# Hi-PACE/hipace

Measured on AMD Instinct MI355X. Metric: transverse slices/s at 1024^2 x 4ppc (explicit solver), higher is better.
Workload: dtype f64

## Files before the change

hipace_amd/_lib.py:

```python
import ctypes as C
import os
import subprocess


def hip_already_started():
    import sys
    if _LIB is not None:
        return True
    t = sys.modules.get("torch")
    try:
        return bool(t is not None and t.cuda.is_initialized())
    except Exception:
        return False


_LIB = None
_HWQ_PRESET = "GPU_MAX_HW_QUEUES" in os.environ
_HIP_STARTED_AT_IMPORT = hip_already_started()
_HERE = os.path.dirname(os.path.abspath(__file__))
CSRC = os.path.join(_HERE, "csrc")
SO = os.environ.get("HPS_LIB") or os.path.join(CSRC, "libhpslice.so")


class Slab(C.Structure):
# ... 74 lines not shown
                ("adaptive_no_predict_step", C.c_int), ("adaptive_no_phase_control", C.c_int), ("adaptive_phase_substeps", C.c_int),
                ("adaptive_density", C.c_double), ("max_time", C.c_double), ("beam_uz_std", C.c_double),
                ("ext_Ez_slope", C.c_double),
                ("beam_do_salame", C.c_int), ("salame_n_iter", C.c_int), ("salame_relative_tolerance", C.c_double),
                ("salame_no_advance", C.c_int), ("salame_Ez_target_slope", C.c_double)]


COMPS = ["N_jx_beam", "N_jy_beam", "chi", "Sy", "Sx", "ExmBy", "EypBx", "Ez", "Bx", "By", "Bz",
         "Psi", "jx_beam", "jy_beam", "jz_beam", "jx", "jy", "rhomjz", "P_jx_beam", "P_jy_beam",
         "Ion_rhomjz", "rho"]
CIDX = {n: i for i, n in enumerate(COMPS)}
COMPS_PC = ["N_jx", "N_jy", "ExmBy", "EypBx", "Ez", "Bx", "By", "Bz", "Psi", "jx", "jy", "jz", "rhomjz",
            "P_Bx", "P_By", "P_jx", "P_jy", "Ion_rhomjz", "It_Bx", "It_By", "PIt_Bx", "PIt_By", "rho"]
CIDX_PC = {n: i for i, n in enumerate(COMPS_PC)}
COMPS_SALAME = ["Ez_target", "Ez_no_salame", "Ez", "jx", "jy", "jz_beam", "Bx", "By", "Sy", "Sx", "Sy_back", "Sx_back"]
ID_VALID = 1 << 63

_SIGS = {
    "hps_last_error": (C.c_char_p, []),
    "hps_version": (C.c_char_p, []),
    "hps_deposit_current": (C.c_int, [Slab, Plasma, Geom, C.c_void_p, C.c_double, C.c_double, C.c_int, C.c_double,
                                      C.c_int, C.c_void_p, C.c_void_p]),
    "hps_explicit_deposit": (C.c_int, [Slab, Plasma, Geom, C.c_void_p, C.c_void_p, C.c_double, C.c_double, C.c_int,
                                       C.c_int, C.c_int, C.c_void_p]),
    "hps_advance_plasma": (C.c_int, [Slab, Plasma, Geom, C.c_void_p, C.c_double, C.c_double, C.c_int, C.c_int,
                                     C.c_int, C.c_int, C.c_void_p]),
    "hps_tiling_create": (C.c_int, [C.c_int, C.c_int, C.c_int, C.c_long, C.POINTER(C.c_void_p)]),
    "hps_reorder_particles": (C.c_int, [C.c_void_p, Plasma, Plasma, Geom, C.c_void_p]),
    "hps_tiling_info": (C.c_int, [C.c_void_p, C.POINTER(C.c_int), C.POINTER(C.c_void_p), C.POINTER(C.c_void_p)]),
    "hps_tiling_destroy": (C.c_int, [C.c_void_p]),
    "hps_deposit_current_tiled": (C.c_int, [Slab, Plasma, Geom, C.c_void_p, C.c_double, C.c_double, C.c_int, C.c_double,
                                            C.c_int, C.c_void_p, C.c_void_p, C.c_void_p, C.c_void_p]),
    "hps_explicit_deposit_tiled": (C.c_int, [Slab, Plasma, Geom, C.c_void_p, C.c_void_p, C.c_double, C.c_double, C.c_int,
                                             C.c_int, C.c_int, C.c_void_p, C.c_void_p, C.c_void_p]),
    "hps_advance_plasma_tiled": (C.c_int, [Slab, Plasma, Geom, C.c_void_p, C.c_double, C.c_double, C.c_int, C.c_int,
                                           C.c_int, C.c_int, C.c_void_p, C.c_void_p, C.c_void_p]),
    "hps_deposit_current_tiled_laser": (C.c_int, [Slab, Plasma, Geom, C.c_void_p, C.c_int, C.c_double, C.c_double, C.c_int,
                                                  C.c_double, C.c_int, C.c_void_p, C.c_void_p, C.c_void_p, C.c_void_p]),
    "hps_explicit_deposit_tiled_laser": (C.c_int, [Slab, Plasma, Geom, C.c_void_p, C.c_int, C.c_void_p, C.c_double, C.c_double,
                                                   C.c_int, C.c_int, C.c_int, C.c_void_p, C.c_void_p, C.c_void_p]),
    "hps_advance_plasma_tiled_laser": (C.c_int, [Slab, Plasma, Geom, C.c_void_p, C.c_int, C.c_double, C.c_double, C.c_int,
                                                 C.c_int, C.c_int, C.c_int, C.c_void_p, C.c_void_p, C.c_void_p]),
    "hps_tiling_set_validity": (C.c_int, [C.c_void_p, C.c_int, C.c_int]),
    "hps_particles_record": (C.c_int, [C.c_int]),
    "hps_particles_recorded": (C.c_int, [C.c_char_p, C.c_long, C.POINTER(C.c_long)]),
    "hps_poisson_create": (C.c_int, [C.c_int, C.c_int, C.c_double, C.c_double, C.POINTER(C.c_void_p)]),
    "hps_poisson_solve": (C.c_int, [C.c_void_p, C.c_void_p, Slab, C.c_int, C.c_void_p]),
    "hps_poisson_solve_batch": (C.c_int, [C.c_void_p, C.c_int, C.c_void_p, Slab, C.c_void_p, C.c_void_p]),
    "hps_poisson_info": (C.c_int, [C.c_void_p, C.POINTER(C.c_int), C.POINTER(C.c_int), C.POINTER(C.c_int)]),
    "hps_poisson_destroy": (C.c_int, [C.c_void_p]),
    "hps_mg_create": (C.c_int, [C.c_int, C.c_int, C.c_double, C.c_double, C.POINTER(C.c_void_p)]),
    "hps_mg_solve1": (C.c_int, [C.c_void_p, Slab, C.c_int, C.c_int, C.c_int, C.c_double, C.c_double, C.c_int,
                                C.POINTER(C.c_int), C.POINTER(C.c_double), C.c_void_p]),
    "hps_mg_solve1_fabs": (C.c_int, [C.c_void_p, Slab, Slab, Slab, C.c_double, C.c_double, C.c_int,
                                     C.POINTER(C.c_int), C.POINTER(C.c_double), C.c_void_p]),
    "hps_mg_info": (C.c_int, [C.c_void_p, C.POINTER(C.c_int), C.POINTER(C.c_int), C.POINTER(C.c_int), C.POINTER(C.c_int),
                              C.POINTER(C.c_long), C.POINTER(C.c_int), C.POINTER(C.c_int), C.POINTER(C.c_int), C.POINTER(C.c_int)]),
    "hps_mg_destroy": (C.c_int, [C.c_void_p]),
    "hps_mg2_create": (C.c_int, [C.c_int, C.c_int, C.c_double, C.c_double, C.POINTER(C.c_void_p)]),
    "hps_mg2_solve2": (C.c_int, [C.c_void_p, C.c_void_p, C.c_void_p, C.c_void_p, C.c_void_p, C.c_double, C.c_double, C.c_int,
                                 C.POINTER(C.c_int), C.POINTER(C.c_double), C.c_void_p]),
    "hps_mg2_info": (C.c_int, [C.c_void_p, C.POINTER(C.c_int), C.POINTER(C.c_int), C.POINTER(C.c_int), C.POINTER(C.c_int)]),
    "hps_mg2_destroy": (C.c_int, [C.c_void_p]),
    "hps_engine_laser_vcycles": (C.c_int, [C.c_void_p, C.POINTER(C.c_long)]),
    "hps_engine_create": (C.c_int, [C.POINTER(Deck), C.c_int, C.POINTER(C.c_void_p)]),
    "hps_engine_destroy": (C.c_int, [C.c_void_p]),
    "hps_engine_begin_step": (C.c_int, [C.c_void_p]),
    "hps_engine_solve_slice": (C.c_int, [C.c_void_p, C.c_int]),
    "hps_engine_solve_slice_begin": (C.c_int, [C.c_void_p, C.c_int]),
    "hps_engine_solve_slice_finish": (C.c_int, [C.c_void_p, C.c_int]),
    "hps_engine_slice_ready": (C.c_int, [C.c_void_p]),
    "hps_engine_run_step": (C.c_int, [C.c_void_p]),
    "hps_engine_sync": (C.c_int, [C.c_void_p]),
    "hps_engine_info": (C.c_int, [C.c_void_p, C.POINTER(C.c_int), C.POINTER(C.c_int), C.POINTER(C.c_long)]),
    "hps_engine_slab": (Slab, [C.c_void_p]),
    "hps_engine_plasma": (Plasma, [C.c_void_p]),
    "hps_engine_stream": (C.c_void_p, [C.c_void_p]),
    "hps_engine_ions": (Plasma, [C.c_void_p]),
    "hps_engine_ion_stats": (C.c_int, [C.c_void_p, C.POINTER(C.c_long), C.POINTER(C.c_long)]),
    "hps_engine_checksums": (C.c_int, [C.c_void_p, C.c_void_p]),
    "hps_beam_sort_by_box": (C.c_int, [C.c_void_p, C.c_long, C.c_double, C.c_double, C.c_int, C.c_void_p, C.c_void_p,
                                       C.c_void_p, C.c_void_p]),
    "hps_engine_stats": (C.c_int, [C.c_void_p, C.POINTER(C.c_long), C.POINTER(C.c_long)]),
    "hps_engine_set_insitu_plasma": (C.c_int, [C.c_void_p, C.c_double]),
    "hps_engine_set_insitu_beam": (C.c_int, [C.c_void_p, C.c_double]),
    "hps_engine_insitu_beam": (C.c_int, [C.c_void_p, C.c_void_p]),
    "hps_engine_insitu_plasma": (C.c_int, [C.c_void_p, C.c_void_p]),
    "hps_engine_set_insitu_fields": (C.c_int, [C.c_void_p, C.c_int]),
    "hps_engine_insitu_fields": (C.c_int, [C.c_void_p, C.c_void_p]),
    "hps_engine_set_field_diagnostic": (C.c_int, [C.c_void_p, C.c_int, C.c_void_p, C.c_void_p]),
    "hps_engine_field_diagnostic": (C.c_int, [C.c_void_p, C.c_void_p]),
    "hps_engine_set_field_diagnostic_box": (C.c_int, [C.c_void_p, C.c_int, C.c_void_p, C.c_void_p, C.c_int, C.c_void_p, C.c_void_p]),
    "hps_engine_field_diagnostic_geometry": (C.c_int, [C.c_void_p, C.c_void_p, C.c_void_p, C.c_void_p]),
    "hps_engine_record_event": (C.c_int, [C.c_void_p, C.c_int, C.POINTER(C.c_void_p)]),
    "hps_engine_wait_event": (C.c_int, [C.c_void_p, C.c_void_p]),
    "hps_stream_pool_shared_pairs": (C.c_int, [C.c_int]),
    "hps_engine_copy_async": (C.c_int, [C.c_void_p, C.c_void_p, C.c_void_p, C.c_long]),
    "hps_engine_set_profiling_stride": (C.c_int, [C.c_void_p, C.c_int]),
    "hps_engine_set_laser_import": (C.c_int, [C.c_void_p, C.c_int, C.c_int]),
    "hps_engine_set_step": (C.c_int, [C.c_void_p, C.c_int]),
    "hps_engine_set_time": (C.c_int, [C.c_void_p, C.c_double, C.c_double]),
    "hps_engine_beam_moments": (C.c_int, [C.c_void_p, C.c_void_p]),
    "hps_adaptive_create": (C.c_int, [C.c_void_p, C.POINTER(C.c_void_p)]),
    "hps_adaptive_set_density_profile": (C.c_int, [C.c_void_p, C.c_int, C.c_void_p, C.c_void_p, C.c_int, C.c_void_p, C.c_void_p]),
    "hps_adaptive_initial_dt": (C.c_int, [C.c_void_p, C.c_double, C.c_double, C.c_int, C.POINTER(C.c_double)]),
    "hps_adaptive_before_step": (C.c_int, [C.c_void_p, C.c_double, C.POINTER(C.c_double)]),
    "hps_adaptive_next_time": (C.c_int, [C.c_void_p, C.POINTER(C.c_double)]),
    "hps_adaptive_after_step": (C.c_int, [C.c_void_p, C.c_void_p, C.c_double, C.c_int, C.POINTER(C.c_double)]),
    "hps_adaptive_destroy": (C.c_int, [C.c_void_p]),
    "hps_engine_export_laser_slice": (C.c_int, [C.c_void_p, C.c_int, C.c_void_p]),
    "hps_engine_import_laser_slice": (C.c_int, [C.c_void_p, C.c_int, C.c_void_p]),
    "hps_engine_import_laser_from": (C.c_int, [C.c_void_p, C.c_int, C.c_void_p]),
    "hps_engine_laser_envelope": (C.c_int, [C.c_void_p, C.c_void_p]),
    "hps_engine_laser_info": (C.c_int, [C.c_void_p, C.POINTER(C.c_int), C.POINTER(C.c_double)]),
    "hps_engine_set_laser_grid": (C.c_int, [C.c_void_p, C.POINTER(C.c_int), C.POINTER(C.c_double), C.POINTER(C.c_double), C.c_int]),
    "hps_engine_laser_grid": (C.c_int, [C.c_void_p, C.POINTER(C.c_int), C.POINTER(C.c_int), C.POINTER(C.c_int), C.POINTER(C.c_int)]),
    "hps_engine_laser_chi": (C.c_int, [C.c_void_p, C.c_void_p]),
    "hps_engine_set_laser_pulses": (C.c_int, [C.c_void_p, C.c_int, C.POINTER(LaserPulse)]),
    "hps_engine_add_laser_samples": (C.c_int, [C.c_void_p, C.c_int, C.c_void_p, C.POINTER(C.c_long), C.POINTER(C.c_double),
                                               C.POINTER(C.c_double), C.c_double]),
    "hps_engine_set_insitu_laser": (C.c_int, [C.c_void_p, C.c_int]),
    "hps_engine_insitu_laser": (C.c_int, [C.c_void_p, C.c_void_p]),
    "hps_laser_interp_aabs": (C.c_int, [Slab, C.c_int, C.c_void_p, C.c_int, C.c_int, C.c_double, C.c_double, C.c_double, C.c_double,
                                        Geom, C.c_int, C.c_void_p]),
    "hps_laser_interp_chi": (C.c_int, [Slab, C.c_int, C.c_void_p, C.c_void_p, C.c_int, C.c_int, C.c_double, C.c_double, C.c_double,
                                       C.c_double, Geom, C.c_int, C.c_int, C.c_void_p]),
    "hps_deposit_current_laser": (C.c_int, [Slab, Plasma, Geom, C.c_void_p, C.c_int, C.c_double, C.c_double, C.c_int, C.c_double,
                                            C.c_int, C.c_void_p, C.c_void_p]),
    "hps_explicit_deposit_laser": (C.c_int, [Slab, Plasma, Geom, C.c_void_p, C.c_int, C.c_void_p, C.c_double, C.c_double, C.c_int,
                                             C.c_int, C.c_int, C.c_void_p]),
    "hps_advance_plasma_laser": (C.c_int, [Slab, Plasma, Geom, C.c_void_p, C.c_int, C.c_double, C.c_double, C.c_int, C.c_int,
                                           C.c_int, C.c_int, C.c_void_p]),
    "hps_engine_pc_stats": (C.c_int, [C.c_void_p, C.POINTER(C.c_long), C.POINTER(C.c_double)]),
    "hps_engine_pc_zero_b_slices": (C.c_int, [C.c_void_p, C.POINTER(C.c_long)]),
    "hps_engine_set_diagnostics": (C.c_int, [C.c_void_p, C.c_int]),
    "hps_engine_set_tiling": (C.c_int, [C.c_void_p, C.c_int, C.c_int]),
    "hps_engine_fallbacks": (C.c_int, [C.c_void_p, C.POINTER(C.c_long)]),
    "hps_engine_set_fusion": (C.c_int, [C.c_void_p, C.c_int]),
    "hps_engine_set_density_profile": (C.c_int, [C.c_void_p, C.c_int, C.c_void_p, C.c_void_p, C.c_int, C.c_void_p, C.c_void_p]),
    "hps_engine_set_plasma_init": (C.c_int, [C.c_void_p, C.POINTER(C.c_int), C.POINTER(C.c_int), C.c_double]),
    "hps_engine_set_fine_patch": (C.c_int, [C.c_void_p, C.c_void_p, C.c_int]),
    "hps_engine_set_plasma_momentum": (C.c_int, [C.c_void_p, C.c_int, C.POINTER(C.c_double), C.POINTER(C.c_double), C.c_ulonglong]),
    "hps_engine_set_plasma_symmetry": (C.c_int, [C.c_void_p, C.c_int, C.c_int]),
    "hps_engine_sorts": (C.c_int, [C.c_void_p, C.POINTER(C.c_long)]),
    "hps_engine_assume_initial_beam_support": (C.c_int, [C.c_void_p]),
    "hps_engine_beam_state": (C.c_int, [C.c_void_p, C.c_void_p, C.c_void_p]),
    "hps_engine_beam_capacity": (C.c_int, [C.c_void_p, C.POINTER(C.c_long)]),
    "hps_engine_set_beam_capacity": (C.c_int, [C.c_void_p, C.c_long]),
    "hps_engine_beam_message_rows": (C.c_int, [C.c_void_p, C.POINTER(C.c_int)]),
    "hps_engine_beam_spin": (C.c_int, [C.c_void_p, C.c_void_p]),
    "hps_engine_set_beam_import": (C.c_int, [C.c_void_p, C.c_int]),
    "hps_engine_export_beam_slice": (C.c_int, [C.c_void_p, C.c_int, C.c_void_p]),
    "hps_engine_import_beam_slice": (C.c_int, [C.c_void_p, C.c_int, C.c_void_p]),
    "hps_engine_set_profiling": (C.c_int, [C.c_void_p, C.c_int]),
    "hps_engine_phase_times": (C.c_int, [C.c_void_p, C.c_void_p, C.c_void_p]),
    "hps_engine_beam_info": (C.c_int, [C.c_void_p, C.POINTER(C.c_long), C.c_void_p]),
    "hps_engine_set_beam_particles": (C.c_int, [C.c_void_p, C.c_long, C.c_void_p, C.POINTER(C.c_long)]),
    "hps_engine_set_beam_storage": (C.c_int, [C.c_void_p, C.c_void_p]),
    "hps_engine_initial_beam": (C.c_int, [C.c_void_p, C.c_void_p]),
    "hps_ring_unique_id": (C.c_int, [C.c_char_p]),
    "hps_ring_init": (C.c_int, [C.c_int, C.c_int, C.c_int, C.c_char_p, C.c_char_p, C.POINTER(C.c_void_p)]),
    "hps_ring_send_slice": (C.c_int, [C.c_void_p, C.c_void_p, C.c_long, C.c_void_p, C.c_int, C.POINTER(C.c_void_p)]),
    "hps_ring_recv_slice": (C.c_int, [C.c_void_p, C.c_void_p, C.c_long, C.c_void_p, C.c_int, C.POINTER(C.c_void_p)]),
    "hps_ring_sendrecv_self": (C.c_int, [C.c_void_p, C.c_void_p, C.c_void_p, C.c_long, C.c_void_p, C.c_int, C.POINTER(C.c_void_p)]),
    "hps_ring_stream_wait": (C.c_int, [C.c_void_p, C.c_int, C.c_void_p]),
    "hps_ring_sync_sends": (C.c_int, [C.c_void_p]),
# ... 89 lines not shown
```

hipace_amd/api.py:

```python
import ctypes as C

import numpy as np
import torch

from . import _lib, decks as _decks, expr as _expr
from ._lib import CIDX, COMPS, ID_VALID, PL_REAL, check


def _stream():
    return C.c_void_p(torch.cuda.current_stream().cuda_stream)


def _iarr(vals):
    return (C.c_int * len(vals))(*[int(v) for v in vals])


class Geometry:

    def __init__(self, nx, ny, lo, hi, dz, bc=1, normalized=True, consts=(1., 1., 1., 1., 1.), ng=None):
        self.nx, self.ny = nx, ny
        g = _lib.Geom()
        g.dx = (hi[0] - lo[0]) / nx
        g.dy = (hi[1] - lo[1]) / ny
        g.dz = dz
# ... 1004 lines not shown
        if event is not None:
            check(_lib.lib().hps_engine_wait_event(self._h, C.c_void_p(event)))

    def copy_async(self, dst, src):
        assert dst.numel() == src.numel()
        check(_lib.lib().hps_engine_copy_async(self._h, C.c_void_p(dst.data_ptr()), C.c_void_p(src.data_ptr()),
                                               dst.numel() * 8))

    def phase_times(self):
        ms = (C.c_double * 8)()
        n = C.c_long()
        check(_lib.lib().hps_engine_phase_times(self._h, ms, C.byref(n)))
        names = ["deposit_current", "poisson", "explicit_deposit", "mg_solve1", "advance_plasma", "other", "sort", "empty_interval"]
        return {k: ms[i] for i, k in enumerate(names)}, n.value

    def checksums(self):
        out = (C.c_double * self.ncomp)()
        check(_lib.lib().hps_engine_checksums(self._h, out))
        names = self.comp_names()
        cs = {names[i]: out[i] for i in range(self.ncomp)}
        if "aabs" in cs:
            tot = C.c_double()
            check(_lib.lib().hps_engine_laser_info(self._h, None, C.byref(tot)))
            cs["laserEnvelope"] = tot.value
        return cs

    @property
    def has_laser(self):
        return bool(self.deck.get("laser_on", 0))

    def laser_message_doubles(self):
        nxl, nyl, _, _ = self.laser_grid()
        return 4 * nxl * nyl

    def set_step(self, step):
        check(_lib.lib().hps_engine_set_step(self._h, int(step)))

    def set_laser_import(self, on, step=0):
        check(_lib.lib().hps_engine_set_laser_import(self._h, int(on), int(step)))

    def export_laser_slice(self, islice, msg):
        check(_lib.lib().hps_engine_export_laser_slice(self._h, islice, C.c_void_p(msg.data_ptr())))

    def import_laser_slice(self, islice, msg):
        check(_lib.lib().hps_engine_import_laser_slice(self._h, islice, C.c_void_p(msg.data_ptr())))

    def import_laser_from(self, islice, src):
        check(_lib.lib().hps_engine_import_laser_from(self._h, islice, src._h))

    def laser_envelope(self):
        nxl, nyl, zlo, zhi = self.laser_grid()
        out = np.empty((zhi - zlo + 1, nyl, nxl), dtype=np.complex128)
        check(_lib.lib().hps_engine_laser_envelope(self._h, out.ctypes.data_as(C.c_void_p)))
        return out

    def comp_names(self):
        if self.deck.get("bxby_solver", 0):
            return list(_lib.COMPS_PC[:22]) + (["rho"] if self.deck.get("deposit_rho", 0) else [])
        return list(COMPS[:21]) + (["rho"] if self.deck.get("deposit_rho", 0) else []) + \
            (["aabs"] if self.deck.get("laser_on", 0) else []) + \
            (["Salame_" + n for n in _lib.COMPS_SALAME] if self.deck.get("beam_do_salame", 0) else [])

    def salame_stats(self):
        nz = self.deck["nz"]
        out = np.zeros((nz, 4), dtype=np.float64)
        check(_lib.lib().hps_engine_salame_stats(self._h, out.ctypes.data_as(C.c_void_p)))
        flags = out[:, 3].astype(np.int64)
        return {"W": out[:, 0].copy(), "W_total": out[:, 1].copy(), "iterations": out[:, 2].astype(np.int64),
                "converged": (flags & 1) != 0, "overloaded": (flags & 2) != 0, "ran": out[:, 2] > 0}

    def pc_stats(self):
        its, err = C.c_long(), C.c_double()
        check(_lib.lib().hps_engine_pc_stats(self._h, C.byref(its), C.byref(err)))
        return its.value, err.value

    def pc_zero_b_slices(self):
        n = C.c_long()
        check(_lib.lib().hps_engine_pc_zero_b_slices(self._h, C.byref(n)))
        return n.value

    def stats(self):
        vc, sl = C.c_long(), C.c_long()
        check(_lib.lib().hps_engine_stats(self._h, C.byref(vc), C.byref(sl)))
        return dict(vcycles=vc.value, slices=sl.value)

    def slab(self):
        self.sync()
        s = _lib.lib().hps_engine_slab(self._h)
        nx, ny, g = s.nx, s.ny, s.ng
        out = np.empty((s.ncomp, ny + 2 * g, nx + 2 * g), dtype=np.float64)
        check(_lib.lib().hps_memcpy_d2h(out.ctypes.data_as(C.c_void_p), C.c_void_p(s.p), out.nbytes))
        return out

    def ions(self):
        self.sync()
        p = _lib.lib().hps_engine_ions(self._h)
        n = p.n
        real = np.empty((11, n), dtype=np.float64)
        idc = np.empty(n, dtype=np.uint64)
        lev = np.empty(n, dtype=np.int32)
        if n:
            for k, name in enumerate(PL_REAL):
                check(_lib.lib().hps_memcpy_d2h(real[k].ctypes.data_as(C.c_void_p), C.c_void_p(getattr(p, name)), real[k].nbytes))
            check(_lib.lib().hps_memcpy_d2h(idc.ctypes.data_as(C.c_void_p), C.c_void_p(p.idcpu), idc.nbytes))
            check(_lib.lib().hps_memcpy_d2h(lev.ctypes.data_as(C.c_void_p), C.c_void_p(p.ion_lev), lev.nbytes))
        key = ((idc >> np.uint64(24)) & np.uint64((1 << 39) - 1)).astype(np.int64) - 1
        return real, ((idc >> np.uint64(63)) & np.uint64(1)).astype(np.int32), lev, key

    def ion_stats(self):
        a, b = C.c_long(), C.c_long()
        check(_lib.lib().hps_engine_ion_stats(self._h, C.byref(a), C.byref(b)))
        return a.value, b.value

    def particles(self):
        self.sync()
        p = _lib.lib().hps_engine_plasma(self._h)
        n = p.n
        real = np.empty((11, n), dtype=np.float64)
        idc = np.empty(n, dtype=np.uint64)
        if n:
            for k, name in enumerate(PL_REAL):
                check(_lib.lib().hps_memcpy_d2h(real[k].ctypes.data_as(C.c_void_p), C.c_void_p(getattr(p, name)), real[k].nbytes))
            check(_lib.lib().hps_memcpy_d2h(idc.ctypes.data_as(C.c_void_p), C.c_void_p(p.idcpu), idc.nbytes))
        return real, ((idc >> np.uint64(63)) & np.uint64(1)).astype(np.int32)
```

hipace_amd/csrc/engine.h:

```cpp
#ifndef HPS_ENGINE_H_
#define HPS_ENGINE_H_

#include "common.h"
#include "expr.h"
#include <algorithm>
#include <array>
#include <vector>
#include "tiling.h"
#include "mg_gate.h"
#include "particle_math.h"
#include "poisson_src.h"
#include "beam_deposit.h"
#include "slab_ops.h"

void mg_rider (void* mg_handle, int** dev_words, const int** host_words);
namespace hps {

constexpr int PC_MAX_SPEC = 64;

int mg_solve1_begin (void* mg_handle, hps_slab s, int sol_comp, int rhs_comp, int acf_comp, double tol_rel, double tol_abs,
                     int max_iters, hipStream_t st);
void mg_solve1_forget_hierarchy (void* mg_handle);
bool poisson_gateable (void* poisson_handle);
void poisson_set_gate (void* poisson_handle, const int* gate);
bool ring_is_ticket (const void* p);
int mg_solve1_prepare (void* mg_handle, hps_slab s, int sol_comp, int rhs_comp, int acf_comp, int max_iters, hipStream_t st);
int mg_solve1_prepare_with (void* mg_handle, hps_slab s, int sol_comp, int rhs_comp, int acf_comp, int max_iters, SlabView f, GradPsiSxSy ga,
                            hipStream_t st, bool* done);
const int* mg_gate_after_enqueued (void* mg_handle);
void mg_defer_post (void* mg_handle);
bool mg_take_deferred_post (void* mg_handle, MgPost* out);
bool mg_solve1_ready (void* mg_handle);
int mg_solve1_finish (void* mg_handle, int* iters_out, double* resnorm_out, int* extra, hipStream_t st);
}

namespace hps {

struct LaserState;

struct DensityProgram { const hps_expr_ins* ins; int n_ins; const double* consts; double z, min_density; };

struct ExprImage {
    ExprImage () = default;
    explicit ExprImage (int header_slots) : h_ins((size_t)header_slots, hps_expr_ins{0, 0}) {}
    int add (const hps_expr& checked);
    hps_expr_ins& slot (int q) { return h_ins[(size_t)q]; }
    int n_ins () const { return (int)h_ins.size(); }
    int upload ();
    const hps_expr_ins* ins () const { return d_ins.get(); }
    const double* consts () const { return d_consts.get(); }
private:
    std::vector<hps_expr_ins> h_ins; std::vector<double> h_consts;
    DevBuf<hps_expr_ins> d_ins; DevBuf<double> d_consts;
};

struct BeamSoA { double *x, *y, *z, *ux, *uy, *uz, *w; int* nsub;
                 double *sx, *sy, *sz; };

struct CollScratch {
    unsigned *cnt = nullptr, *off[2] = {nullptr, nullptr}, *perm[2] = {nullptr, nullptr};
    long cap[2] = {0, 0}; int ncells = 0; void* temp = nullptr; size_t temp_bytes = 0; unsigned long long* stats = nullptr;
    CollScratch () = default; CollScratch (const CollScratch&) = delete; CollScratch& operator= (const CollScratch&) = delete;
    ~CollScratch ();
};

struct Engine {
    hps_deck d{};
    hps_geom gm{};
    int g = 0, ncomp = 0;
    hipStream_t st = nullptr;
    bool st_pooled = false; int st_device = 0;
    hps_slab slab{};
    struct Ions { double* d_adk = nullptr; unsigned long long* d_cnt = nullptr; long long* h_cnt = nullptr; long long* h_cnt_dev = nullptr;
                  long long seq = 0; long n_ionized = 0; bool pending = false; int* d_tile_flag = nullptr;
                  double* d_fbound = nullptr;
                } ion;
    std::vector<double> prof_r, prof_t, prof_f_t; double* d_prof_r = nullptr; double prof_ft = 1.0;
    double hollow_core_radius = 0.0;
    bool fine_patch_set = false; int fine_T = 0; long fine_ncells = 0; int* d_fine_level = nullptr; int* d_fine_cells = nullptr;
    struct Thermal { double u_mean[3] = {0.0, 0.0, 0.0}, u_std[3] = {0.0, 0.0, 0.0}; unsigned long long seed = 0;
                     bool warm () const { for (int q = 0; q < 3; ++q) if (u_mean[q] != 0.0 || u_std[q] != 0.0) return true; return false; }
                   };
    bool do_symmetrize = false, prevent_centered = false;
    bool shifted (const int ppc[2], int dir) const { return prevent_centered && (dir == 0 ? d.nx : d.ny) % 2 == 1 && ppc[dir] % 2 == 1; }
    int set_plasma_momentum (int species, const double* u_mean, const double* u_std, unsigned long long seed);
    int set_plasma_symmetry (int symmetrize, int prevent_centered_particle);
    int alloc_sheets ();
    int set_plasma_init (const int* plasma_fine, const int* ion_fine, double hollow_core);
    int set_fine_patch (const unsigned char* mask_host, int transition_cells);
    bool fuse_push_deposit = false; int ahead_for = -2;
    long fallback_div = 256;
    bool gate_push = true;
    int step_index = -1;
    int next_step = -1;
    bool time_set = false; double next_t = 0.0, next_dt = 0.0, step_dt = 0.0;
    double step_time = 0.0;
    struct BeamExt { bool on = false; ExprImage image; int depth = 0; } bext;
    int set_beam_external_fields (const hps_expr* E3, const hps_expr* B3);
    struct DensityExpr { bool on = false; std::vector<std::vector<hps_expr_ins>> ins; std::vector<std::vector<double>> consts;
                         std::vector<double> z_pos; std::vector<int> off; int depth = 0; double min_density = 0.0; int cur = 0; };
    ExprImage dens_image; double dens_z = 0.0;
    int set_density_expr (int species, int n_progs, const hps_expr* progs, const double* z_pos, double min_density);
    void density_begin_step (double ct);
    DensityProgram density_program (int species) const;
    size_t density_lds (int species) const { const DensityExpr& D = sp[species].dens; return D.on ? expr_lds_bytes(D.depth, 256) : 0; }
    struct Species {
        int index = 0;
        hps_plasma pl{}, pl_alt{}; double *real = nullptr, *real_alt = nullptr; Tiling* tiling = nullptr;
        long cap = 0, n_init = 0;
        int ppc[2] = {0, 0}, fine_ppc[2] = {0, 0}; double density = 0.0, charge = 0.0, mass = 0.0;
        int init_level = 0, can_ionize = 0, keyed = 0;
// ... 34 lines not shown
    double* d_open_mom = nullptr;
    int open_boundary (int nbatch, unsigned no_monopole_mask);
    double* beam_data = nullptr; double* beam_init = nullptr; double* beam_cur = nullptr;
    long nbeam = 0; std::vector<long> beam_off;
    bool moving = false; int steps_begun = 0; int beam_rows = 7;
    BeamSoA bm{}, bm_scr{}; double* bm_store = nullptr; int* bm_nsub = nullptr; int* bm_nsub_scr = nullptr;
    long* d_B = nullptr; int* d_nfront = nullptr; std::vector<long> h_B;
    bool beam_import = false; long* d_Bimp = nullptr; long beam_cap = 0; int* d_beam_overflow = nullptr;
    long beam_bound (int p) const {
        if (p < 0 || p >= d.nz) return 0;
        if (beam_import) return std::max(nbeam, 1L);
        return h_B[p + 1] - h_B[0];
    }
    struct Box { int ilo, ihi, jlo, jhi; };
    Box beam_box{0, -1, 0, -1}, beam_box_init{0, -1, 0, -1}, full_box{0, -1, 0, -1};
    int* d_nqsa = nullptr;
    double* d_checksum = nullptr;
    bool diagnostics = false;
    bool profiling = false; bool prof_light = false; int prof_stride = 1; bool prof_now = false;
    std::vector<hipEvent_t> ev; size_t ev_used = 0;
    std::vector<hipEvent_t> hand_ev;
    void mark ();
    long total_vcycles = 0, slices_done = 0;
    int* d_pc_dist = nullptr;
    double pc_floor = 0.0;
    int* d_pc_go = nullptr; bool pc_speculate = false; int pc_spec_iters = 1, pc_enqueued = 0, pc_islice = -1; double pc_base_seq = 0.0, pc_last_err = 0.0;
    int solve_slice_pc_begin (int islice); int solve_slice_pc_finish (int islice); int pc_enqueue_iteration (int it); int pc_wait_slot (int slot, double seq);
    bool pc = false; double* d_pc = nullptr; double* d_pc_aux = nullptr; double* h_pc = nullptr; double* h_pc_dev = nullptr; double pc_seq = 0.0; long pc_iterations = 0; double pc_err_sum = 0.0; long pc_zero_b_slices = 0;
    double pc_tol = 4e-2, pc_mix = 0.05; int pc_max_iter = 30;
    int c_aabs = -1; double* d_laser_sum = nullptr;
    LaserState* laser = nullptr;
    struct LaserGrid { bool set = false; int nx = 0, ny = 0, zlo = 0, zhi = -1, order = 1;
                       double lo[3] = {0, 0, 0}, hi[3] = {0, 0, 0}, dx = 0.0, dy = 0.0, xoff = 0.0, yoff = 0.0; } lgrid;
    int set_laser_grid (const int* n_cell, const double* patch_lo, const double* patch_hi, int interp_order);
    struct LaserSamples { int geometry = 0; long extent[3] = {0, 0, 0}; double offset[3] = {0, 0, 0}, spacing[3] = {0, 0, 0}, unit = 1.0;
                          std::vector<double> data; };
    bool laser_pulses_set = false; std::vector<hps_laser_pulse> laser_pulses; std::vector<LaserSamples> laser_samples;
    bool insitu_laser = false;
    bool laser_has_slice (int islice) const { return !lgrid.set || (islice >= lgrid.zlo && islice <= lgrid.zhi); }
    hipStream_t st_laser = nullptr; hipEvent_t ev_lfork = nullptr, ev_ldone = nullptr;
    bool laser_async = true, laser_pending = false;
    hipStream_t st_aux = nullptr; hipEvent_t ev_aux[3] = {nullptr, nullptr, nullptr}; bool aux_on = false, aux_pending = false;
    hipStream_t laser_stream () const { return (laser_async && st_laser) ? st_laser : st; }
    int fork_laser ();
    int laser_done ();
    int join_laser ();
    std::vector<int> fd_comps; int fd_c[3] = {1, 1, 1}; double* d_fd = nullptr; int* d_fd_comps = nullptr;
    int fd_n[3] = {0, 0, 0}; double fd_h[3] = {0, 0, 0}, fd_pos0[3] = {0, 0, 0}, fd_lo[3] = {0, 0, 0}, fd_hi[3] = {0, 0, 0}; int fd_slice_dir = -1;
    size_t fd_cells () const { return (size_t)fd_n[0]*fd_n[1]*fd_n[2]; }
    int fill_field_diagnostic (int islice);
    double* d_insitu_bm = nullptr; double insitu_bm_radius = 0.0;
    void insitu_beam (int islice);
    double* d_insitu_pl = nullptr; double insitu_pl_radius = 0.0;
    double* d_insitu = nullptr;

    ~Engine ();
    int create (const hps_deck& deck, int device);
    int init_beam ();
    int install_beam (std::vector<double> (&h)[7]);
    int set_beam_particles (long n, const double* soa_host, long* n_outside);
    int set_beam_fixed_ppc (const hps_expr* density, double min_density, const double* u_std, const int* random_ppc, unsigned long long seed);
    int set_beam_fixed_weight (const hps_beam_fixed_weight* spec, const hps_expr* mean_x, const hps_expr* mean_y, unsigned long long seed,
                               long* n_left_out);
    int set_beam_fixed_weight_pdf (const hps_beam_fixed_weight_pdf* spec, const hps_expr* pdf, const hps_expr* progs, unsigned long long seed,
                                   long* n_left_out, double* uz_moments);
    int install_beam_device (double* blocks_dev, long n, const double box[4]);
    int begin_device_beam (long* n_left_out = nullptr);
    int finish_device_beam (DevBuf<double>& blocks, long n, long* n_left_out = nullptr);
    int drop_device_beam (int e, long* n_left_out);
    void release_beam ();
    void set_beam_box (double xlo, double xhi, double ylo, double yhi);
    int install_moving_beam (const std::vector<double> (*h)[7]);
    int begin_step ();
    int deposit_beam_slice (int islice, int cjx, int cjy, int cjz, const int* go = nullptr);
    void deposit_grid_current (int islice, int cjz);
    int solve_slice (int islice);
    int solve_slice_begin (int islice);
    int solve_slice_finish (int islice);
    int pending_slice = -1; bool pend_fuse = false, pend_gated = false, pend_gated_ion = false;
    bool gate_ion_push = true; IonArgs pend_ia{}; long pend_covered = 0;
    int push_with_ionization (int islice, const int comp[5], const int* go, bool first);
    bool lazy_shift = true, shift_pending = false;
    void flush_shift ();
    bool fuse_sources = true;
    int c_sal = -1; int sal_last_slice = -2; bool sal_overloaded = false; double sal_zeta_initial = 0.0;
    double* d_sal = nullptr; std::vector<double> sal_stats;
    bool salame_now () const { return c_sal >= 0 && step_index == 0; }
    int salame_module (int islice);
    int salame_solve_ez ();
    int run_step ();
    struct Collision { int a, b; double coulomb_log; unsigned long long seed; bool beam = false; };
    std::vector<Collision> coll; CollScratch coll_scratch; bool step_begun = false;
    int collide_slice (int islice);
};

int ion_create (Engine& E);
void ion_destroy (Engine& E);
unsigned event_flags (bool timing);
std::array<double**, 11> soa_arrays (hps_plasma& p);
int alloc_soa (hps_plasma& p, double*& real, long cap, bool alias);
void free_soa (hps_plasma& p, double*& real);
int init_plasma_fine (Engine& E, const Engine::Species& s, double radius_sq);
int init_plasma_warm (Engine& E, const Engine::Species& s, double radius_sq);
int laser_create (Engine& E);
void laser_destroy (Engine& E);
int laser_begin_step (Engine& E);
int laser_update_aabs (Engine& E, int islice, double* sum_abs);
int laser_advance_slice (Engine& E, int islice);
int laser_copy_envelope (Engine& E, double* out_host);
int laser_chi_initial (Engine& E);
int laser_copy_chi (Engine& E, double* out_host);
void laser_sizes (Engine& E, int* nx, int* ny, int* nz);
long laser_mg_vcycles (Engine& E);
int laser_set_import (Engine& E, int on, int step);
int laser_export_slice (Engine& E, int islice, double* msg_dev);
int laser_import_slice (Engine& E, int islice, const double* msg_dev);
int laser_import_from (Engine& E, int islice, Engine& src);
int laser_check_samples (Engine& E, const Engine::LaserSamples& S);
int laser_set_insitu (Engine& E, int on);
int laser_clear_insitu (Engine& E);
int laser_copy_insitu (Engine& E, double* out_host);
int expr_check_named (const char* fn, const char* what, const hps_expr* p, int n_vars, int* depth);
bool expr_is_zero (const hps_expr& p);
int beam_blocks_to_soa (Engine& E, const double* blocks, double* soa, long nb);
int beam_deposit_moving (Engine& E, int p, int cjx, int cjy, int cjz);
int beam_push_moving (Engine& E, int islice);
int beam_push_slice (Engine& E, int islice, int p, long bound);
int beam_moments_reset (Engine& E);
int beam_export_slice (Engine& E, int islice, double* msg_dev, long cap);
int beam_import_slice (Engine& E, int islice, const double* msg_dev, long cap);
int salame_get_w_enqueue (const hps_slab& slab, int cT, int cN, int cE, int cJ, double* scratch, hipStream_t st);
const double* salame_get_w_result (const double* scratch);

}
#endif
```

hipace_amd/csrc/engine.hip:

```cpp
#include "common.h"
#include "engine.h"

#include <cmath>
#include <cstdlib>
#include <cstring>
#include <limits>
#include <atomic>
#include <algorithm>
#include <map>
#include <mutex>
#include <new>

namespace {
std::mutex g_pool_mutex;
std::map<int, std::vector<hipStream_t>> g_stream_pool;
std::map<int, bool> g_pool_made;
}

namespace hps {

int deposit_current_tiled (const hps_slab& slab, const hps_plasma& pl, const hps_geom& g, const int comp[6], double charge,
                           double mass, int order, double max_qsa, int can_ionize, int* n_qsa, Tiling* T, int* n_fallback,
                           hipStream_t st, int aabs_comp = -1, const int* tile_flag = nullptr, TailWork tw = TailWork{},
                           const BeamPairWork* beam = nullptr, const int* go = nullptr, bool valid_by_w = false);
int explicit_deposit_tiled (const hps_slab& slab, const hps_plasma& pl, const hps_geom& g, const int cache[4], const int depos[2],
                            double charge, double mass, int order, int dtype, int can_ionize, Tiling* T, int* n_fallback,
                            hipStream_t st, int aabs_comp = -1, const int* tile_flag = nullptr, TailWork tw = TailWork{}, bool valid_by_w = false);
int advance_plasma_tiled (const hps_slab& slab, const hps_plasma& pl, const hps_geom& g, const int comp[5], double charge,
                          double mass, int order, int temp_slice, int n_subcycles, int can_ionize, Tiling* T,
                          int* n_fallback, hipStream_t st, int aabs_comp = -1, const IonArgs* ion = nullptr, const int* go = nullptr,
                          TailWork tw = TailWork{}, const MgPost* post = nullptr);
int advance_deposit_tiled (const hps_slab& slab, const hps_plasma& pl, const hps_geom& g, const int comp[5], const int dep_comp[6],
                           double charge, double mass, int order, int n_subcycles, double max_qsa, int* n_qsa, Tiling* T,
                           int* n_fallback, hipStream_t st);

static thread_local std::string g_err;
void set_error (const std::string& msg) { g_err = msg; }

struct CompList { int n; int c[12]; };


__global__ __launch_bounds__(256)
void k_zero_comps (double* p, long ns, long plane, int js, CompList full, CompList boxed, CellBox bb, CompList from_ion = CompList{0, {}}, int c_ion = -1)
{
    const long s = (long)blockIdx.x*blockDim.x + threadIdx.x;
    if (s >= plane) return;
    for (int k = 0; k < full.n; ++k) p[full.c[k]*ns + s] = 0.0;
    if (c_ion >= 0) { const double ion = p[c_ion*ns + s]; for (int k = 0; k < from_ion.n; ++k) p[from_ion.c[k]*ns + s] = ion; }
    const int j = (int)(s / js), i = (int)(s - (long)j*js);
    if (i >= bb.ilo && i <= bb.ihi && j >= bb.jlo && j <= bb.jhi)
        for (int k = 0; k < boxed.n; ++k) p[boxed.c[k]*ns + s] = 0.0;
}

__global__ __launch_bounds__(256)
void k_copy_comps (double* p, long ns, long plane, CompList dst, CompList src)
{
    const long s = (long)blockIdx.x*blockDim.x + threadIdx.x;
    if (s >= plane) return;
    double v[12];
    for (int k = 0; k < src.n; ++k) v[k] = p[src.c[k]*ns + s];
    for (int k = 0; k < dst.n; ++k) p[dst.c[k]*ns + s] = v[k];
}

__global__ __launch_bounds__(256)
void k_shift_slices (double* p, long ns, long plane, int js, CellBox bb)
{
    const long s = (long)blockIdx.x*blockDim.x + threadIdx.x;
    if (s >= plane) return;
    const int j = (int)(s / js), i = (int)(s - (long)j*js);
    double njx = 0.0, njy = 0.0;
    if (i >= bb.ilo && i <= bb.ihi && j >= bb.jlo && j <= bb.jhi) {
        const double tjx = p[HPS_C_JXB*ns + s], tjy = p[HPS_C_JYB*ns + s];
        njx = p[HPS_C_N_JXB*ns + s]; njy = p[HPS_C_N_JYB*ns + s];
        p[HPS_C_P_JXB*ns + s] = tjx; p[HPS_C_P_JYB*ns + s] = tjy;
        p[HPS_C_JXB*ns + s] = njx;   p[HPS_C_JYB*ns + s] = njy;
    }
    p[HPS_C_JX*ns + s] = njx; p[HPS_C_JY*ns + s] = njy;
}

__global__ __launch_bounds__(256)
void k_shift_zero (double* p, long ns, long plane, int js, CellBox bb, int c_rho, int c_ion = -1)
{
    const long s = (long)blockIdx.x*blockDim.x + threadIdx.x;
    if (s >= plane) return;
    const int j = (int)(s / js), i = (int)(s - (long)j*js);
    double njx = 0.0, njy = 0.0;
    if (i >= bb.ilo && i <= bb.ihi && j >= bb.jlo && j <= bb.jhi) {
        const double tjx = p[HPS_C_JXB*ns + s], tjy = p[HPS_C_JYB*ns + s];
        njx = p[HPS_C_N_JXB*ns + s]; njy = p[HPS_C_N_JYB*ns + s];
        p[HPS_C_P_JXB*ns + s] = tjx; p[HPS_C_P_JYB*ns + s] = tjy;
        p[HPS_C_JXB*ns + s] = njx;   p[HPS_C_JYB*ns + s] = njy;
        p[HPS_C_N_JXB*ns + s] = 0.0; p[HPS_C_N_JYB*ns + s] = 0.0; p[HPS_C_JZB*ns + s] = 0.0;
    }
    p[HPS_C_JX*ns + s] = njx; p[HPS_C_JY*ns + s] = njy;
    const double ion = c_ion >= 0 ? p[c_ion*ns + s] : 0.0;
    p[HPS_C_CHI*ns + s] = 0.0; p[HPS_C_RHOMJZ*ns + s] = ion;
    if (c_rho >= 0) p[c_rho*ns + s] = ion;
}

__global__ __launch_bounds__(256)
void k_add_ions_psi_rhs (SlabView f, int c_rhomjz, int c_ion, int c_rho, double inv_ep0, double* staging)
{
    const int i = blockIdx.x*blockDim.x + threadIdx.x - f.ng;
    const int j = blockIdx.y - f.ng;
    if (i >= f.nx + f.ng) return;
    const long o = f.off(i, j);
    const double ion = f.p[c_ion*f.ns + o];
    const double r = f.p[c_rhomjz*f.ns + o] + ion;
    f.p[c_rhomjz*f.ns + o] = r;
    if (c_rho >= 0) f.p[c_rho*f.ns + o] += ion;
    if (i >= 0 && i < f.nx && j >= 0 && j < f.ny) staging[(long)j*f.nx + i] = -inv_ep0*r;
}

__global__ __launch_bounds__(256)
void k_rhs_all (SlabView f, int c_rhomjz, int c_ion, int c_rho, int c_jx, int c_jy, double inv_ep0,
                double fez_x, double fez_y, double fbz_y, double fbz_x, double* staging, long plane)
{
    const int i = blockIdx.x*blockDim.x + threadIdx.x - f.ng;
    const int j = blockIdx.y - f.ng;
    if (i >= f.nx + f.ng) return;
    const long o = f.off(i, j);
    double r;
    if (c_ion >= 0) {
        const double ion = f.p[c_ion*f.ns + o];
        r = f.p[c_rhomjz*f.ns + o] + ion;
        f.p[c_rhomjz*f.ns + o] = r;
        if (c_rho >= 0) f.p[c_rho*f.ns + o] += ion;
    } else {
        if (!(i >= 0 && i < f.nx && j >= 0 && j < f.ny)) return;
        r = f.p[c_rhomjz*f.ns + o];
    }
    if (i >= 0 && i < f.nx && j >= 0 && j < f.ny) {
        const long so = (long)j*f.nx + i;
        const double* X = f.p + c_jx*f.ns + o;
        const double* Y = f.p + c_jy*f.ns + o;
        staging[so] = -inv_ep0*r;
        staging[plane + so] = fez_x*(X[1] - X[-1]) + fez_y*(Y[f.js] - Y[-f.js]);
        staging[2*plane + so] = fbz_y*(X[f.js] - X[-f.js]) + fbz_x*(Y[1] - Y[-1]);
    }
}

__global__ __launch_bounds__(256)
void k_rhs_lincomb (SlabView f, int cA, int dirA, double fa, int cB, int dirB, double fb, double* staging)
{
    const int i = blockIdx.x*blockDim.x + threadIdx.x;
    const int j = blockIdx.y;
    if (i >= f.nx) return;
    const long o = f.off(i, j);
    const long sa = dirA == 0 ? 1 : f.js, sb = dirB == 0 ? 1 : f.js;
    const double* A = f.p + cA*f.ns + o;
    const double* B = f.p + cB*f.ns + o;
    staging[(long)j*f.nx + i] = fa*(A[sa] - A[-sa]) + fb*(B[sb] - B[-sb]);
}

__global__ __launch_bounds__(256)
void k_grid_current (SlabView f, int cjz, double xlo, double ylo, double dx, double dy, double mx, double my, double sx, double sy,
                     double amp)
{
    const int i = blockIdx.x*blockDim.x + threadIdx.x;
    const int j = blockIdx.y;
    if (i >= f.nx) return;
    const double delta_x = (xlo + (i + 0.5)*dx - mx) / sx;
    const double delta_y = (ylo + (j + 0.5)*dy - my) / sy;
    f(i, j, cjz) += amp*exp(-0.5*(delta_x*delta_x + delta_y*delta_y));
}

__global__ __launch_bounds__(256)
void k_grad_psi (SlabView f, int cPsi, int cExmBy, int cEypBx, double hdx_inv, double hdy_inv)
{
    const int gg = f.ng - 1;
    const int i = blockIdx.x*blockDim.x + threadIdx.x - gg;
    const int j = blockIdx.y - gg;
    if (i >= f.nx + gg) return;
    const long o = f.off(i, j);
    const double* P = f.p + cPsi*f.ns + o;
    f.p[cExmBy*f.ns + o] = -(P[1] - P[-1])*hdx_inv;
    f.p[cEypBx*f.ns + o] = -(P[f.js] - P[-f.js])*hdy_inv;
}

__global__ __launch_bounds__(256)
// ... 409 lines not shown
        int lo = 0, hi = -1;
        if (std::sscanf(e.substr(pos, end - pos).c_str(), "%d-%d", &lo, &hi) == 2)
            for (int b = std::max(lo, 0); b <= std::min(hi, 255); ++b) mask[b >> 5] |= 1u << (b & 31);
        pos = end + 1;
    }
    return hipExtStreamCreateWithCUMask(s, 8, mask);
}

long Engine::sheet_slots (const Species& s) const
{
    if (!s.present()) return 0;
    const long cells = (long)d.nx*d.ny, nc = (long)s.ppc[0]*s.ppc[1];
    const long copies = do_symmetrize ? 4 : 1;
    if (!(fine_patch_set && s.fine_ppc[0] > 0)) return copies*nc*cells;
    return copies*(nc*cells + ((long)s.fine_ppc[0]*s.fine_ppc[1] - nc)*fine_ncells);
}

std::array<double**, 11> soa_arrays (hps_plasma& p)
{
    return {&p.x, &p.y, &p.w, &p.ux, &p.uy, &p.psi, &p.x_prev, &p.y_prev, &p.ux_half, &p.uy_half, &p.psi_half};
}
int alloc_soa (hps_plasma& p, double*& real, long cap, bool alias)
{
    HPS_HIP_CHECK(hipMalloc(&real, (size_t)cap*11*sizeof(double)));
    const auto arr = soa_arrays(p);
    for (int k = 0; k < 11; ++k) *arr[k] = real + (size_t)k*cap;
    if (alias) { p.x_prev = p.x; p.y_prev = p.y; }
    HPS_HIP_CHECK(hipMalloc(&p.idcpu, (size_t)cap*sizeof(uint64_t)));
    HPS_HIP_CHECK(hipMalloc(&p.ion_lev, (size_t)cap*sizeof(int32_t)));
    return HPS_OK;
}
void free_soa (hps_plasma& p, double*& real)
{
    (void)hipFree(real); (void)hipFree(p.idcpu); (void)hipFree(p.ion_lev);
    real = nullptr; p = hps_plasma{};
}
static hps_plasma tail_of (const hps_plasma& p, long first, long n)
{
    hps_plasma t = p;
    for (double** a : soa_arrays(t)) *a += first;
    t.idcpu += first; t.ion_lev += first; t.n = n;
    return t;
}

int Engine::alloc_sheets ()
{
    for (Species& s : sp) { free_soa(s.pl, s.real); s.n_init = s.cap = sheet_slots(s); }
    if (ions.present()) el.cap = el.n_init + ions.n_init*(long)(d.ion_Z - d.ion_init_level);
    for (Species& s : sp) {
        s.pl.n = s.n_init;
        if (s.cap > 0) { if (int e = alloc_soa(s.pl, s.real, s.cap, s.alias_prev())) return e; }
    }
    return HPS_OK;
}

int Engine::create (const hps_deck& deck, int device)
{
    d = deck;
    HPS_REQUIRE(d.nx >= 4 && d.ny >= 4 && d.nz >= 1, "hps_engine_create: bad grid");
    HPS_REQUIRE(d.order >= 0 && d.order <= 3, "hps_engine_create: depos_order must be 0..3");
    HPS_REQUIRE(d.n_subcycles >= 0, "hps_engine_create: plasma n_subcycles must be >= 1 (0 = default 1)");
    if (d.n_subcycles == 0) d.n_subcycles = 1;
    if (d.field_bc != 0 && d.field_bc != 1) { set_error("hps_engine_create: boundary.field must be 0 (Dirichlet) or 1 (Open)"); return HPS_ERR_UNSUPPORTED; }
    if (d.field_bc == 1) {
        const double radius = std::min(std::min(std::fabs(d.lo[0]), std::fabs(d.hi[0])), std::min(std::fabs(d.lo[1]), std::fabs(d.hi[1])));
        HPS_REQUIRE(radius > 0.0 && d.lo[0] < 0.0 && d.hi[0] > 0.0 && d.lo[1] < 0.0 && d.hi[1] > 0.0, "hps_engine_create: boundary.field = Open needs x = y = 0 inside the box");
        HPS_HIP_CHECK(hipMalloc(&d_open_mom, (size_t)4*256*2*19*sizeof(double)));
    }
    pc = (d.bxby_solver != 0);
    if (const char* v = std::getenv("HPS_GATED_PUSH")) gate_push = std::atoi(v) != 0;
    if (const char* v = std::getenv("HPS_AUX_STREAM")) aux_on = std::atoi(v) != 0;
    if (aux_on) {
        HPS_HIP_CHECK(hipStreamCreateWithFlags(&st_aux, hipStreamNonBlocking));
        for (hipEvent_t& ev : ev_aux) HPS_HIP_CHECK(hipEventCreateWithFlags(&ev, event_flags(false)));
    }
    if (const char* v = std::getenv("HPS_FOLD_TAIL")) fold_tail = std::atoi(v) != 0;
    if (const char* v = std::getenv("HPS_POST_IN_PUSH")) post_in_push = std::atoi(v) != 0;
    if (const char* v = std::getenv("HPS_FOLD_BEAM")) fold_beam = std::atoi(v) != 0;
    if (const char* v = std::getenv("HPS_FOLD_HIERARCHY")) fold_hierarchy = std::atoi(v) != 0;
    if (const char* v = std::getenv("HPS_VALID_BY_W")) valid_by_w = std::atoi(v) != 0;
    if (const char* v = std::getenv("HPS_GATED_ION_PUSH")) gate_ion_push = std::atoi(v) != 0;
    if (const char* v = std::getenv("HPS_LAZY_SHIFT")) lazy_shift = std::atoi(v) != 0;
    if (const char* v = std::getenv("HPS_FUSE_SOURCES")) fuse_sources = std::atoi(v) != 0;
    if (const char* v = std::getenv("HPS_SORT_FALLBACK_DIV")) { const long q = std::atol(v); if (q >= 1) fallback_div = q; }
    HPS_REQUIRE(!(d.beam_spin_tracking && d.dt == 0.0 && !d.dt_adaptive), "hps_engine_create: spin tracking needs a moving beam (hipace.dt != 0)");
    HPS_REQUIRE(!(d.dt_adaptive && d.laser_on), "hps_engine_create: hipace.dt = adaptive cannot be used with a laser (Hipace.cpp:408)");
    if (d.beam_do_salame) {
        if (pc) { set_error("hps_engine_create: beam_do_salame needs the explicit solver (Hipace.cpp:152), not the predictor-corrector"); return HPS_ERR_UNSUPPORTED; }
        if (d.beam_profile == 0 && !(std::isfinite(d.beam_zmin) && std::isfinite(d.beam_zmax))) {
            set_error("hps_engine_create: beam_do_salame with a gaussian beam profile needs finite beam_zmin and beam_zmax (BeamParticleContainer.cpp:149)"); return HPS_ERR_ARG; }
        if (d.ion_on) { set_error("hps_engine_create: beam_do_salame with the ionisable species (ion_on) is not supported"); return HPS_ERR_UNSUPPORTED; }
        if (d.laser_on) { set_error("hps_engine_create: beam_do_salame with a laser is not supported"); return HPS_ERR_UNSUPPORTED; }
        if (d.dt != 0.0 || d.dt_adaptive) { set_error("hps_engine_create: beam_do_salame needs a static beam (hipace.dt = 0)"); return HPS_ERR_UNSUPPORTED; }
        HPS_REQUIRE(d.salame_n_iter >= 0 && d.salame_relative_tolerance >= 0.0, "hps_engine_create: salame_n_iter and salame_relative_tolerance must not be negative");
        if (d.salame_n_iter == 0) d.salame_n_iter = 5;
        if (d.salame_relative_tolerance == 0.0) d.salame_relative_tolerance = 1.0e-4;
    }
    step_dt = d.dt;
    if (d.predcorr_tol > 0.0) pc_tol = d.predcorr_tol;
    if (d.predcorr_max_iter > 0) pc_max_iter = d.predcorr_max_iter;
    if (d.predcorr_mix > 0.0) pc_mix = d.predcorr_mix;
    HPS_HIP_CHECK(hipSetDevice(device));
    HPS_HIP_CHECK(create_engine_stream(&st, device, &st_pooled));
    st_device = device;
    if (const char* v = std::getenv("HPS_LASER_ASYNC")) laser_async = std::atoi(v) != 0;
    if (laser_async && d.laser_on && d.laser_solver >= 1 && d.dt != 0.0) {
        int lo = 0, hi = 0;
        (void)hipDeviceGetStreamPriorityRange(&lo, &hi);
        HPS_HIP_CHECK(hipStreamCreateWithPriority(&st_laser, hipStreamNonBlocking, lo));
        HPS_HIP_CHECK(hipEventCreateWithFlags(&ev_lfork, event_flags(false)));
        HPS_HIP_CHECK(hipEventCreateWithFlags(&ev_ldone, event_flags(false)));
    }
    g = (d.order + 1)/2 + 1;
    ncomp = pc ? (d.deposit_rho ? HPS_PC_RHO + 1 : HPS_PC_RHO) : (d.deposit_rho ? HPS_C_RHO + 1 : HPS_C_RHO);
    if (d.beam_radiation_reaction && !d.si_units && !(d.background_density_SI > 0.0)) {
        set_error("hps_engine_create: radiation reaction in normalised units needs background_density_SI"); return HPS_ERR_ARG; }
    if (d.laser_on) {
        if (pc) { set_error("hps_engine_create: the laser needs the explicit solver"); return HPS_ERR_UNSUPPORTED; }
        HPS_REQUIRE(d.laser_w0 > 0.0 && d.laser_L0 > 0.0 && d.laser_lambda0 > 0.0, "hps_engine_create: laser w0, L0, lambda0 must be positive");
        if (d.laser_solver < 0 || d.laser_solver > 2) { set_error("hps_engine_create: lasers.solver_type must be 0 (static), 1 (fft) or 2 (multigrid)"); return HPS_ERR_UNSUPPORTED; }
        c_aabs = ncomp++;
    }
    gm.dx = (d.hi[0] - d.lo[0])/d.nx; gm.dy = (d.hi[1] - d.lo[1])/d.ny; gm.dz = (d.hi[2] - d.lo[2])/d.nz;
    gm.xoff = 0.5*(d.lo[0] + d.hi[0] - gm.dx*(d.nx - 1));
    gm.yoff = 0.5*(d.lo[1] + d.hi[1] - gm.dy*(d.ny - 1));
    gm.c = gm.ep0 = gm.mu0 = gm.q_e = gm.m_e = 1.0;
    if (d.si_units) {
        gm.c = 299792458.0; gm.ep0 = 8.8541878128e-12; gm.mu0 = 1.25663706212e-06; gm.q_e = 1.602176634e-19; gm.m_e = 9.1093837015e-31;
    }
    gm.plo[0] = d.lo[0]; gm.plo[1] = d.lo[1]; gm.phi[0] = d.hi[0]; gm.phi[1] = d.hi[1];
    gm.bc = d.bc; gm.normalized = d.si_units ? 0 : 1;

    if (d.beam_do_salame) {
        c_sal = ncomp;
        HPS_HIP_CHECK(hipMalloc(&d_sal, (size_t)4*257*sizeof(double)));
        sal_stats.assign((size_t)4*d.nz, 0.0);
    }
    slab.nx = d.nx; slab.ny = d.ny; slab.ng = g; slab.ncomp = ncomp + (c_sal >= 0 ? (int)HPS_SAL_NCOMP : 0);
    slab.jstride = d.nx + 2*g; slab.nstride = slab.jstride*(d.ny + 2*g);
    HPS_HIP_CHECK(hipMalloc(&slab.p, (size_t)slab.nstride*slab.ncomp*sizeof(double)));
    HPS_HIP_CHECK(hipMemset(slab.p, 0, (size_t)slab.nstride*slab.ncomp*sizeof(double)));
    HPS_HIP_CHECK(hipMalloc(&staging, (size_t)3*d.nx*d.ny*sizeof(double)));

    if (d.ion_on) {
        HPS_REQUIRE(d.ion_ppc[0] >= 1 && d.ion_ppc[1] >= 1 && d.ion_density > 0.0 && d.ion_mass > 0.0 && d.ion_charge != 0.0,
                    "hps_engine_create: the ion species needs ppc, density, mass and charge");
        if (int e = ion_create(*this)) return e;
    }
    for (int k = 0; k < 2; ++k) { sp[k].index = k; sp[k].can_ionize = k; sp[k].keyed = k; sp[k].temp_push = pc || (k == 0 && c_sal >= 0); }
    std::copy(d.plasma_ppc, d.plasma_ppc + 2, el.ppc); el.density = d.plasma_density; el.charge = d.plasma_charge; el.mass = d.plasma_mass;
    if (d.ion_on) { std::copy(d.ion_ppc, d.ion_ppc + 2, ions.ppc); ions.density = d.ion_density; ions.charge = d.ion_charge; ions.mass = d.ion_mass; ions.init_level = d.ion_init_level; }
    if (int e = alloc_sheets()) return e;
    HPS_HIP_CHECK(hipMalloc(&d_laser_sum, sizeof(double)));
    HPS_HIP_CHECK(hipMemset(d_laser_sum, 0, sizeof(double)));
    HPS_HIP_CHECK(hipMalloc(&d_nqsa, sizeof(int)));
    HPS_HIP_CHECK(hipMemset(d_nqsa, 0, sizeof(int)));
    HPS_HIP_CHECK(hipMalloc(&d_checksum, HPS_PC_NCOMP_MAX*sizeof(double)));
    HPS_HIP_CHECK(hipMemset(d_checksum, 0, HPS_PC_NCOMP_MAX*sizeof(double)));
    if (int e = hps_poisson_create(d.nx, d.ny, gm.dx, gm.dy, &ps)) return e;
    if (int e = hps_mg_create(d.nx, d.ny, gm.dx, gm.dy, &mg)) return e;
    {   int* dw = nullptr; const int* hw = nullptr;
        mg_rider(mg, &dw, &hw);
        d_nfallback = dw; h_nfallback = hw; }
    if (pc) {
        HPS_HIP_CHECK(hipMalloc(&d_pc, 4*sizeof(double)));
        HPS_HIP_CHECK(hipMemset(d_pc, 0, 4*sizeof(double)));
        HPS_HIP_CHECK(hipMalloc(&d_pc_aux, 4*sizeof(double)));
        HPS_HIP_CHECK(hipMemset(d_pc_aux, 0, 4*sizeof(double)));
        HPS_HIP_CHECK(hipHostMalloc(&h_pc, 8*PC_MAX_SPEC*sizeof(double), hipHostMallocMapped));
        std::memset(h_pc, 0, 8*PC_MAX_SPEC*sizeof(double));
        HPS_HIP_CHECK(hipHostGetDevicePointer((void**)&h_pc_dev, h_pc, 0));
        HPS_HIP_CHECK(hipMalloc(&d_pc_go, (PC_MAX_SPEC + 1)*sizeof(int)));
        HPS_HIP_CHECK(hipMemset(d_pc_go, 0, (PC_MAX_SPEC + 1)*sizeof(int)));
        {   const char* v = std::getenv("HPS_PC_EXACT_ZERO");
            if (!(v && std::atoi(v) == 0)) d_pc_dist = d_pc_go + PC_MAX_SPEC; }
        {   double rel = 0.0;
            if (const char* v = std::getenv("HPS_PC_NOISE_FLOOR")) rel = std::atof(v);
            pc_floor = rel*gm.mu0*gm.c*std::fabs(d.plasma_charge*d.plasma_density)*(double)d.nx*d.ny*(d.nx*gm.dx); }
        {   const char* v = std::getenv("HPS_PC_SPECULATE");
            pc_speculate = !(v && std::atoi(v) == 0) && pc_max_iter <= PC_MAX_SPEC - 2 && poisson_gateable(ps)
                           && d.field_bc == 0; }
        d_nfallback = reinterpret_cast<int*>(d_pc + 2); h_nfallback = reinterpret_cast<const int*>(h_pc + 4);
    }
    if (c_aabs >= 0) { if (int e = laser_create(*this)) return e; }
    return init_beam();
}

int Engine::setup_tiling ()
{
    if (tile_size == 0 || el.cap == 0 || el.tiling) return HPS_OK;
    if (int e = tiling_create(d.nx, d.ny, tile_size, el.cap, &el.tiling)) return e;
    {   const char* v = std::getenv("HPS_VALID_BY_PSI");
        el.tiling->valid_by_psi = (v && std::atoi(v) != 0); }
    if (int e = alloc_soa(el.pl_alt, el.real_alt, el.cap, el.alias_prev())) return e;
    if (ions.present()) {
        int ion_ts = tile_size;
        if (const char* v = std::getenv("HPS_ION_TILE")) { const int t = std::atoi(v); if (t == 16 || t == 32) ion_ts = t; }
        if (int e = tiling_create(d.nx, d.ny, ion_ts, ions.cap, &ions.tiling)) return e;
        if (int e = alloc_soa(ions.pl_alt, ions.real_alt, ions.cap, ions.alias_prev())) return e;
        HPS_HIP_CHECK(hipMalloc(&ion.d_tile_flag, (size_t)ions.tiling->g.ntiles*sizeof(int)));
        {   const char* v = std::getenv("HPS_ION_TILE_SKIP");
            if (!(v && std::atoi(v) == 0)) HPS_HIP_CHECK(hipMalloc(&ion.d_fbound, (size_t)5*ions.tiling->g.ntiles*sizeof(double))); }
    }
    return HPS_OK;
}

int Engine::sort_sheet (Species& s)
{
    s.pl_alt.n = s.pl.n;
    if (int e = tiling_sort(s.tiling, s.pl, s.pl_alt, gm, st)) return e;
    std::swap(s.pl, s.pl_alt);
    std::swap(s.real, s.real_alt);
    return HPS_OK;
}

int Engine::resort ()
{
    if (int e = sort_sheet(el)) return e;
    since_sort = 0; ++n_sorts;
    fb_at_sort = h_nfallback ? *h_nfallback : 0;
    return HPS_OK;
}

int Engine::init_sheet (Species& s)
{
    const long n = s.pl.n;
    if (n == 0) return HPS_OK;
    const double radius_sq = d.plasma_radius > 0.0 ? d.plasma_radius*d.plasma_radius : std::numeric_limits<double>::infinity();
    if (warm_init(s)) return init_plasma_warm(*this, s, radius_sq);
    if (hollow_core_radius > 0.0 || (fine_patch_set && s.fine_ppc[0] > 0) || s.dens.on)
        return init_plasma_fine(*this, s, radius_sq);
    const int nppc = s.ppc[0]*s.ppc[1];
    hipLaunchKernelGGL(k_init_plasma, dim3(ceil_div(n, 256)), dim3(256), 0, st, s.pl, n, d.nx, d.ny, s.ppc[0], s.ppc[1], d.lo[0], d.lo[1],
                       gm.dx, gm.dy, s.density*(d.si_units ? gm.dx*gm.dy*gm.dz/nppc : 1.0/nppc),
                       s.init_level, s.keyed, d_prof_r, (int)prof_r.size(), prof_ft, radius_sq);
    return HPS_OK;
}

int Engine::begin_step ()
{
    HPS_REQUIRE(!(d.dt_adaptive && steps_begun == 0 && d.beam_profile < 0 && !host_beam),
                "hps_engine_begin_step: hipace.dt = adaptive needs a beam (beam_profile = -1 and no hps_engine_set_beam_particles: the sum of weights is 0)");
    HPS_REQUIRE(fine_patch_set == (el.fine_ppc[0] > 0 || ions.fine_ppc[0] > 0),
                "hps_engine_begin_step: both fine_ppc (hps_engine_set_plasma_init) and the fine patch (hps_engine_set_fine_patch) must be given to use the fine plasma patch");
    HPS_REQUIRE(!(laser && laser_pulses_set && laser_pulses.empty() && laser_samples.empty() && !step_begun),
                "hps_engine_begin_step: hps_engine_set_laser_pulses with n = 0 needs at least one hps_engine_add_laser_samples");
    if (laser && !step_begun) { for (const LaserSamples& S : laser_samples) { if (int e = laser_check_samples(*this, S)) return e; } }
    if (int e = setup_tiling()) return e;
    el.keyed = coll.empty() ? 0 : 1;
    step_begun = true;
    if (moving && steps_begun > 0) {
        int ov = 0;
        HPS_HIP_CHECK(hipMemcpyAsync(&ov, d_beam_overflow, sizeof(int), hipMemcpyDeviceToHost, st));
        HPS_HIP_CHECK(hipStreamSynchronize(st));
        HPS_REQUIRE(ov == 0, "moving beam: a slice outgrew the hand-off capacity (twice the fullest injected slice) in the previous step");
    }
    if (moving && beam_import) {
        HPS_HIP_CHECK(hipMemsetAsync(d_B, 0, (size_t)(d.nz + 1)*sizeof(long), st));
        HPS_HIP_CHECK(hipMemsetAsync(d_Bimp, 0, (size_t)(d.nz + 1)*sizeof(long), st));
        HPS_HIP_CHECK(hipMemsetAsync(d_nfront, 0, (size_t)(d.nz + 2)*sizeof(int), st));
        ++steps_begun;
    } else if (moving) {
        if (steps_begun > 0) {
            hipLaunchKernelGGL(k_beam_new_step, dim3(ceil_div(std::max(nbeam, 1L), 256)), dim3(256), 0, st, bm_nsub, nbeam);
            HPS_HIP_CHECK(hipMemsetAsync(d_nfront, 0, (size_t)(d.nz + 2)*sizeof(int), st));
        }
        HPS_HIP_CHECK(hipMemcpyAsync(h_B.data(), d_B, (size_t)(d.nz + 1)*sizeof(long), hipMemcpyDeviceToHost, st));
        HPS_HIP_CHECK(hipStreamSynchronize(st));
        ++steps_begun;
    }
    shift_pending = false;
    HPS_HIP_CHECK(hipMemsetAsync(slab.p, 0, (size_t)slab.nstride*slab.ncomp*sizeof(double), st));
    if (d_pc_dist) HPS_HIP_CHECK(hipMemsetAsync(d_pc_dist, (d.grid_current_on || d.ion_on || d.plasma_no_neutralize || el.thermal.warm() || ions.thermal.warm()) ? 1 : 0, sizeof(int), st));
    HPS_HIP_CHECK(hipMemsetAsync(d_checksum, 0, HPS_PC_NCOMP_MAX*sizeof(double), st));
    HPS_HIP_CHECK(hipMemsetAsync(d_laser_sum, 0, sizeof(double), st));
    if (int e = join_laser()) return e;
    if (laser) { if (int e = laser_begin_step(*this)) return e; }
    if (d_insitu_pl) HPS_HIP_CHECK(hipMemsetAsync(d_insitu_pl, 0, (size_t)15*d.nz*sizeof(double), st));
    if (d_insitu_bm) HPS_HIP_CHECK(hipMemsetAsync(d_insitu_bm, 0, (size_t)23*d.nz*sizeof(double), st));
    if (d_insitu) HPS_HIP_CHECK(hipMemsetAsync(d_insitu, 0, (size_t)10*d.nz*sizeof(double), st));
    if (insitu_laser && laser) { if (int e = laser_clear_insitu(*this)) return e; }
    if (d_fd) HPS_HIP_CHECK(hipMemsetAsync(d_fd, 0, fd_comps.size()*fd_cells()*sizeof(double), st));
    step_index = (next_step >= 0) ? next_step : step_index + 1;
    next_step = -1;
    ahead_for = -2;
    if (salame_now()) { sal_last_slice = -2; sal_overloaded = false; std::fill(sal_stats.begin(), sal_stats.end(), 0.0); }
    if (d_mom) { if (int e = beam_moments_reset(*this)) return e; }
    if (time_set) {
        step_dt = next_dt; step_time = next_t;
        prof_ft = table_value(prof_t.data(), prof_f_t.data(), (int)prof_t.size(), gm.c*next_t);
        density_begin_step(gm.c*next_t);
        time_set = false;
    } else {
        step_dt = d.dt; step_time = d.dt*step_index;
        prof_ft = table_value(prof_t.data(), prof_f_t.data(), (int)prof_t.size(), gm.c*d.dt*step_index);
        density_begin_step(gm.c*d.dt*step_index);
    }
    if (laser && lgrid.set) { if (int e = laser_chi_initial(*this)) return e; }
    if (int e = ionize_collect()) return e;
    el.pl.n = el.n_init;
    if (int e = init_sheet(el)) return e;
    if (el.tiling) { if (int e = resort()) return e; }
    if (el.pl.n > 0 && !d.plasma_no_neutralize) {
        const int comp[6] = {-1, -1, -1, -1, -1, pc ? (int)HPS_PC_ION_RHOMJZ : (int)HPS_C_ION_RHOMJZ};
        if (el.tiling) {
            if (int e = deposit_current_tiled(slab, el.pl, gm, comp, -el.charge, el.mass, d.order, d.max_qsa, 0, d_nqsa, el.tiling, d_nfallback, st)) return e;
        } else {
            if (int e = hps_deposit_current(slab, el.pl, gm, comp, -el.charge, el.mass, d.order, d.max_qsa, 0, d_nqsa, st)) return e;
        }
    }
    if (ions.present()) {
        if (int e = init_sheet(ions)) return e;
        if (ions.tiling) {
            if (int e = sort_sheet(ions)) return e;
            HPS_HIP_CHECK(hipMemsetAsync(ion.d_tile_flag, ions.init_level > 0 ? 0x01 : 0, (size_t)ions.tiling->g.ntiles*sizeof(int), st));
        }
        const unsigned long long c0[4] = {(unsigned long long)el.n_init, 0ULL, 0ULL, (unsigned long long)ion.n_ionized};
        HPS_HIP_CHECK(hipMemcpyAsync(ion.d_cnt, c0, sizeof(c0), hipMemcpyHostToDevice, st));
        HPS_HIP_CHECK(hipStreamSynchronize(st));
    }
    HPS_HIP_CHECK(hipGetLastError());
    return HPS_OK;
}

void Engine::deposit_grid_current (int islice, int cjz)
{
    if (!d.grid_current_on) return;
    const double delta_z = (d.lo[2] + islice*gm.dz - d.grid_current_mean[2]) / d.grid_current_std[2];
    hipLaunchKernelGGL(k_grid_current, dim3(ceil_div(d.nx, 256), d.ny), dim3(256), 0, st, SlabView(slab), cjz, d.lo[0], d.lo[1], gm.dx,
                       gm.dy, d.grid_current_mean[0], d.grid_current_mean[1], d.grid_current_std[0], d.grid_current_std[1],
                       d.grid_current_peak*std::exp(-0.5*(delta_z*delta_z)));
}

int Engine::deposit_beam_slice (int islice, int cjx, int cjy, int cjz, const int* go)
{
    if (nbeam == 0 || islice < 0 || islice >= d.nz) return HPS_OK;
    if (moving) return beam_deposit_moving(*this, d.nz - 1 - islice, cjx, cjy, cjz);
    const long first0 = beam_off[d.nz - 1 - islice], count = beam_off[d.nz - islice] - first0;
    if (count <= 0) return HPS_OK;
    double* blk = beam_cur + 7*first0;
    const BeamView beam{blk, blk + count, blk + 2*count, blk + 3*count, blk + 4*count, blk + 5*count, blk + 6*count};
    const long first = 0;
    const double q_invvol = d.beam_charge*(d.si_units ? 1.0/(gm.dx*gm.dy*gm.dz) : 1.0);
    const double csq_inv = 1.0/(gm.c*gm.c);
    const dim3 grid(ceil_div(count, 256)), block(256);
    SlabView f(slab);
    switch (d.order) {
        case 0: hipLaunchKernelGGL(k_beam_deposit<0>, grid, block, 0, st, f, beam, first, count, cjx, cjy, cjz, q_invvol, csq_inv, 1.0/gm.dx, 1.0/gm.dy, gm.xoff, gm.yoff, go, d_pc_dist); break;
        case 1: hipLaunchKernelGGL(k_beam_deposit<1>, grid, block, 0, st, f, beam, first, count, cjx, cjy, cjz, q_invvol, csq_inv, 1.0/gm.dx, 1.0/gm.dy, gm.xoff, gm.yoff, go, d_pc_dist); break;
        case 2: hipLaunchKernelGGL(k_beam_deposit<2>, grid, block, 0, st, f, beam, first, count, cjx, cjy, cjz, q_invvol, csq_inv, 1.0/gm.dx, 1.0/gm.dy, gm.xoff, gm.yoff, go, d_pc_dist); break;
        default: hipLaunchKernelGGL(k_beam_deposit<3>, grid, block, 0, st, f, beam, first, count, cjx, cjy, cjz, q_invvol, csq_inv, 1.0/gm.dx, 1.0/gm.dy, gm.xoff, gm.yoff, go, d_pc_dist); break;
    }
    return HPS_OK;
}
// ... 566 lines not shown
        e = hps_poisson_solve_batch(ps, 2, staging, slab, comps, st);
        poisson_set_gate(ps, nullptr);
        if (e) return e; }
    pc_seq += 1.0;
    hipLaunchKernelGGL(k_rel_b_error, dim3(128), b256, 0, st, f, HPS_PC_BX, HPS_PC_IT_BX, d_pc, (volatile double*)h_pc_dev, pc_seq,
                       go, pc_tol, it, pc_max_iter, pc_floor);
    hipLaunchKernelGGL(k_pc_mix, gplane, b256, 0, st, slab.p, slab.nstride, plane, d_pc, d_pc_aux, it, pc_mix, (const int*)go, (const int*)d_pc_dist);
    pc_enqueued = it;
    return HPS_OK;
}

int Engine::pc_wait_slot (int slot, double seq)
{
    volatile double* hp = h_pc + 8*slot;
    auto there = [&] () { return hp[1] == seq && hp[3] == seq && hp[5] == seq; };
    long spins = 0;
    while (!there()) {
        if ((++spins & 0xfffff) == 0 && hipStreamQuery(st) != hipErrorNotReady) {
            if (there()) break;
            HPS_HIP_CHECK(hipStreamSynchronize(st));
            if (!there()) { set_error("predictor-corrector: the error read-back never arrived"); return HPS_ERR_HIP; }
        }
    }
    __atomic_thread_fence(__ATOMIC_ACQUIRE);
    return HPS_OK;
}

int Engine::solve_slice_pc_finish (int islice)
{
    SlabView f(slab);
    const long plane = slab.nstride;
    const dim3 b256(256);
    const dim3 gplane(ceil_div(plane, 256));
    const int comp_push[5] = {HPS_PC_PSI, HPS_PC_EZ, HPS_PC_BX, HPS_PC_BY, HPS_PC_BZ};
    int e;
    double err = pc_last_err;
    if (pc_speculate && el.tiling && !moving && !ions.present()) {
        int it = 0;
        err = 1.0;
        while (err > pc_tol && it < pc_max_iter) {
            ++it; ++pc_iterations;
            if (it > pc_enqueued) { if ((e = pc_enqueue_iteration(it))) return e; }
            if ((e = pc_wait_slot(it, pc_base_seq + it))) return e;
            const volatile double* hp = h_pc + 8*it;
            err = hp[0] > 0.0 ? hp[2]/hp[0] : 0.0;
            if (!(hp[0] > 0.0) && it == 1) ++pc_zero_b_slices;
        }
        pc_spec_iters = it;
        pc_seq = pc_base_seq + std::max(it, pc_enqueued);
    }
    pc_err_sum += err;
    mark();
    if (diagnostics)
        hipLaunchKernelGGL(k_checksum, dim3(64, ncomp), b256, 0, st, f, ncomp, d_checksum);
    if ((e = fill_field_diagnostic(islice))) return e;
    mark();
    if (ions.present()) {
        if (ions.tiling) {
            if ((e = ion_field_bounds())) return e;
            const IonArgs ia = ion_args(islice);
            if ((e = advance_plasma_tiled(slab, ions.pl, gm, comp_push, ions.charge, ions.mass, d.order, 0, d.n_subcycles, 1, ions.tiling, d_nfallback, st, -1, &ia))) return e;
        } else {
            if ((e = ionize_slice(islice))) return e;
            if ((e = species_advance(ions, comp_push, 0))) return e;
        }
        if ((e = ionize_collect())) return e;
    }
    if ((e = species_advance(el, comp_push, 0))) return e;
    insitu_beam(islice);
    if (moving && nbeam > 0) { if ((e = beam_push_moving(*this, islice))) return e; }
    if (!coll.empty()) { if ((e = collide_slice(islice))) return e; }
    mark();
    {   CompList dst{6, {HPS_PC_PIT_BX, HPS_PC_PIT_BY, HPS_PC_P_BX, HPS_PC_P_BY, HPS_PC_P_JX, HPS_PC_P_JY}};
        CompList src{6, {HPS_PC_P_BX, HPS_PC_P_BY, HPS_PC_BX, HPS_PC_BY, HPS_PC_JX, HPS_PC_JY}};
        hipLaunchKernelGGL(k_copy_comps, gplane, b256, 0, st, slab.p, slab.nstride, plane, dst, src); }
    mark();
    HPS_HIP_CHECK(hipGetLastError());
    ++slices_done;
    return HPS_OK;
}

void Engine::flush_shift ()
{
    if (!shift_pending) return;
    shift_pending = false;
    const CellBox bb{beam_box.ilo, beam_box.ihi, beam_box.jlo, beam_box.jhi};
    hipLaunchKernelGGL(k_shift_slices, dim3(ceil_div(slab.nstride, 256)), dim3(256), 0, st, slab.p, slab.nstride, slab.nstride, (int)slab.jstride, bb);
}

int Engine::solve_slice (int islice)
{
    if (int e = solve_slice_begin(islice)) return e;
    return solve_slice_finish(islice);
}

int Engine::solve_slice_begin (int islice)
{
    HPS_REQUIRE(pending_slice == -1, "hps_engine_solve_slice_begin: the previous slice has not been finished");
    if (pc) { if (int e = solve_slice_pc_begin(islice)) return e; pending_slice = islice; return HPS_OK; }
    SlabView f(slab);
    const long plane = slab.nstride;
    const dim3 b256(256);
    const dim3 gplane(ceil_div(plane, 256));
    const dim3 gvalid(ceil_div(d.nx, 256), d.ny);
    int e;

    prof_now = profiling && (slices_done % prof_stride == 0);
    mg_solve1_forget_hierarchy(mg);
    if ((e = join_laser())) return e;
    mark();
    if (d_insitu_pl && el.pl.n > 0)
        hipLaunchKernelGGL(k_insitu_plasma, dim3(256), b256, 0, st, el.pl, 1.0/gm.c, insitu_pl_radius*insitu_pl_radius, d_insitu_pl, d.nz, islice);
    const CellBox bb{beam_box.ilo, beam_box.ihi, beam_box.jlo, beam_box.jhi};
    const bool ahead = (ahead_for == islice);
    ahead_for = -2;
    bool zeroed = false;
    if (shift_pending) {
        shift_pending = false;
        if (!ahead) { hipLaunchKernelGGL(k_shift_zero, gplane, b256, 0, st, slab.p, slab.nstride, plane, (int)slab.jstride, bb, d.deposit_rho ? (int)HPS_C_RHO : -1, (int)HPS_C_ION_RHOMJZ); zeroed = true; }
        else hipLaunchKernelGGL(k_shift_slices, gplane, b256, 0, st, slab.p, slab.nstride, plane, (int)slab.jstride, bb);
    }
    if (!ahead && !zeroed)
    {   CompList z{0, {}}, zb{0, {}};
        for (int c : {HPS_C_CHI, HPS_C_RHOMJZ}) z.c[z.n++] = c;
        if (d.deposit_rho) z.c[z.n++] = HPS_C_RHO;
        for (int c : {HPS_C_JZB, HPS_C_N_JXB, HPS_C_N_JYB}) zb.c[zb.n++] = c;
        CompList fi{0, {}};
        fi.c[fi.n++] = HPS_C_RHOMJZ; if (d.deposit_rho) fi.c[fi.n++] = HPS_C_RHO;
        hipLaunchKernelGGL(k_zero_comps, gplane, b256, 0, st, slab.p, slab.nstride, plane, (int)slab.jstride, z, zb, bb, fi, (int)HPS_C_ION_RHOMJZ); }
    if (c_aabs >= 0) {
        if ((e = laser_update_aabs(*this, islice, diagnostics ? d_laser_sum : nullptr))) return e;
    }
    const bool sal = salame_now();
    const bool aux = aux_on && st_aux && !pc && !ahead && !prof_now && !sal;
    if (aux) { HPS_HIP_CHECK(hipEventRecord(ev_aux[0], st)); HPS_HIP_CHECK(hipStreamWaitEvent(st_aux, ev_aux[0], 0)); }

    mark();
    if (el.tiling && (since_sort >= sort_period || (since_sort >= 2 && *h_nfallback - fb_at_sort > el.pl.n/fallback_div) ||
                      (since_sort >= 1 && el.pl.n - el.tiling->sorted_n > std::max(el.pl.n/32, 16384L)))) { if ((e = resort())) return e; }
    ++since_sort;
    mark();
    const bool pair = !moving && nbeam > 0 && !sal;
    BeamPairWork bw;
    if (pair) {
        const long fA = beam_off[d.nz - 1 - islice], cA = beam_off[d.nz - islice] - fA;
        const long fB = islice >= 1 ? beam_off[d.nz - islice] : 0, cB = islice >= 1 ? beam_off[d.nz - islice + 1] - fB : 0;
        double* pa = beam_cur + 7*fA; double* pb = beam_cur + 7*fB;
        bw.a = BeamView{pa, pa + cA, pa + 2*cA, pa + 3*cA, pa + 4*cA, pa + 5*cA, pa + 6*cA};
        bw.b = BeamView{pb, pb + cB, pb + 2*cB, pb + 3*cB, pb + 4*cB, pb + 5*cB, pb + 6*cB};
        bw.ca = cA; bw.cb = cB; bw.nba = (int)ceil_div(cA, 256); bw.nwg = bw.nba + (int)ceil_div(cB, 256);
        bw.cjz = HPS_C_JZB; bw.cjxn = HPS_C_N_JXB; bw.cjyn = HPS_C_N_JYB;
        bw.q_invvol = d.beam_charge*(d.si_units ? 1.0/(gm.dx*gm.dy*gm.dz) : 1.0); bw.csq_inv = 1.0/(gm.c*gm.c);
    }
    const bool beam_folded = pair && fold_beam && bw.nwg > 0 && !ahead && el.pl.n > 0 && el.tiling && el.tiling->sorted_n > 0;
    if (!ahead)
    {   const int comp[6] = {HPS_C_JX, HPS_C_JY, -1, d.deposit_rho ? HPS_C_RHO : -1, HPS_C_CHI, HPS_C_RHOMJZ};
        if ((e = species_deposit(el, comp, beam_folded ? &bw : nullptr))) return e;
        if ((e = species_deposit(ions, comp))) return e; }
    mark();
    if (pair) {
        if (!beam_folded && bw.nwg > 0) {
            hipStream_t sb = (aux && !d.grid_current_on) ? st_aux : st;
#define HPS_PAIR(O) hipLaunchKernelGGL(k_beam_deposit_pair<O>, dim3(bw.nwg), b256, 0, sb, f, bw, 1.0/gm.dx, 1.0/gm.dy, gm.xoff, gm.yoff)
            switch (d.order) { case 0: HPS_PAIR(0); break; case 1: HPS_PAIR(1); break; case 2: HPS_PAIR(2); break; default: HPS_PAIR(3); break; }
#undef HPS_PAIR
        }
    } else if ((e = deposit_beam_slice(islice, -1, -1, HPS_C_JZB))) return e;
    deposit_grid_current(islice, HPS_C_JZB);
    if (aux) {
        HPS_HIP_CHECK(hipEventRecord(ev_aux[1], st)); HPS_HIP_CHECK(hipStreamWaitEvent(st_aux, ev_aux[1], 0));
        if ((e = mg_solve1_prepare(mg, slab, HPS_C_BX, HPS_C_SY, HPS_C_CHI, 200, st_aux))) return e;
        HPS_HIP_CHECK(hipEventRecord(ev_aux[2], st_aux));
        aux_pending = true;
    }

    {   const double fa = 1.0/(gm.ep0*gm.c);
        const double fez_x = fa*0.5*(1.0/gm.dx), fez_y = fa*0.5*(1.0/gm.dy), fbz_y = gm.mu0*0.5*(1.0/gm.dy), fbz_x = -gm.mu0*0.5*(1.0/gm.dx);
        const int comps[3] = {HPS_C_PSI, HPS_C_EZ, HPS_C_BZ};
        if (fuse_sources && poisson_sources_fusable(ps) && d.field_bc == 0) {
            const long js = slab.jstride;
            const double* R = slab.p + (long)HPS_C_RHOMJZ*slab.nstride + g + (long)g*js;
            const double* X = slab.p + (long)HPS_C_JX*slab.nstride + g + (long)g*js;
            const double* Y = slab.p + (long)HPS_C_JY*slab.nstride + g + (long)g*js;
            const PoissonSrc spec[3] = {
                {1, {R, nullptr}, {nullptr, nullptr}, {-1.0/gm.ep0, 0.0}},
                {2, {X + 1, Y + js}, {X - 1, Y - js}, {fez_x, fez_y}},
                {2, {X + js, Y + 1}, {X - js, Y - 1}, {fbz_y, fbz_x}}};
            if ((e = poisson_solve_batch_src(ps, 3, spec, js, slab, comps, st))) return e;
        } else {
            hipLaunchKernelGGL(k_rhs_all, dim3(ceil_div(slab.jstride, 256), d.ny + 2*g), b256, 0, st, f, HPS_C_RHOMJZ,
                               -1 , d.deposit_rho ? HPS_C_RHO : -1, HPS_C_JX, HPS_C_JY, 1.0/gm.ep0,
                               fez_x, fez_y, fbz_y, fbz_x, staging, (long)d.nx*d.ny);
            if ((e = open_boundary(3, 0x6u))) return e;
            if ((e = hps_poisson_solve_batch(ps, 3, staging, slab, comps, st))) return e;
        } }
    const bool laser_now = c_aabs >= 0 && d.laser_solver >= 1 && d.dt != 0.0 && laser_has_slice(islice);
    const bool laser_split = laser_now && laser_stream() != st;
    if (laser_now && !laser_split) { if ((e = laser_advance_slice(*this, islice))) return e; }
    if (laser_split) { if ((e = fork_laser())) return e; }
    if (laser_split && d.laser_solver == 1) { if ((e = laser_advance_slice(*this, islice)) || (e = laser_done())) return e; }
    if (aux_pending) { HPS_HIP_CHECK(hipStreamWaitEvent(st, ev_aux[2], 0)); aux_pending = false; }
    if (pair || nbeam == 0) {
        const GradPsiSxSy ga{HPS_C_PSI, HPS_C_EXMBY, HPS_C_EYPBX, 0.5*(1.0/gm.dx), 0.5*(1.0/gm.dy), HPS_C_SX, HPS_C_SY, HPS_C_JZB, HPS_C_N_JXB, HPS_C_N_JYB,
                             HPS_C_P_JXB, HPS_C_P_JYB, gm.mu0, 2.0*gm.dx, 2.0*gm.dy, 2.0*gm.dz, bb};
        bool with_hierarchy = false;
        if (fold_hierarchy && !pc && !aux) {
            if ((e = mg_solve1_prepare_with(mg, slab, HPS_C_BX, HPS_C_SY, HPS_C_CHI, 200, f, ga, st, &with_hierarchy))) return e;
        }
        if (!with_hierarchy)
            hipLaunchKernelGGL(k_gradpsi_sxsy, dim3(ceil_div(slab.jstride, 256), d.ny + 2*g), b256, 0, st, f, ga);
        mark();
    } else {
        hipLaunchKernelGGL(k_grad_psi, dim3(ceil_div(d.nx + 2*(g - 1), 256), d.ny + 2*(g - 1)), b256, 0, st, f, HPS_C_PSI,
                           HPS_C_EXMBY, HPS_C_EYPBX, 0.5*(1.0/gm.dx), 0.5*(1.0/gm.dy));
        mark();
        if (!sal) { if ((e = deposit_beam_slice(islice - 1, HPS_C_N_JXB, HPS_C_N_JYB, -1))) return e; }
        hipLaunchKernelGGL(k_sxsy_beam, dim3(ceil_div(slab.jstride, 256), d.ny + 2*g), b256, 0, st, f, HPS_C_SX, HPS_C_SY, HPS_C_JZB, HPS_C_N_JXB, HPS_C_N_JYB,
                           HPS_C_P_JXB, HPS_C_P_JYB, gm.mu0, 2.0*gm.dx, 2.0*gm.dy, 2.0*gm.dz, bb);
    }
    mark();
    {   const int cache[4] = {HPS_C_BZ, HPS_C_EZ, HPS_C_EXMBY, HPS_C_EYPBX};
        const int depos[2] = {HPS_C_SY, HPS_C_SX};
        for (const Species& s : sp) { if ((e = species_explicit(s, cache, depos))) return e; } }

    mark();
    const bool fuse = fuse_push_deposit && coll.empty() && el.tiling && islice > 0 && !moving && c_aabs < 0 && !ions.present() && el.pl.n > 0 && el.tiling->sorted_n == el.pl.n && !sal;
    const bool gated = gate_push && el.tiling && !fuse && !ions.present() && el.pl.n > 0 && el.tiling->sorted_n == el.pl.n && !diagnostics && !d_fd && !d_insitu && !sal;
    const bool gated_ion = gate_push && gate_ion_push && el.tiling && !fuse && ions.present() && ions.tiling && el.pl.n > 0 && el.tiling->sorted_n > 0 && fold_tail
                           && !diagnostics && !d_fd && !d_insitu && !sal;
    const int comp_push[5] = {HPS_C_PSI, HPS_C_EZ, HPS_C_BX, HPS_C_BY, HPS_C_BZ};
    {
        if (gated && post_in_push) mg_defer_post(mg);
        if ((e = mg_solve1_begin(mg, slab, HPS_C_BX, HPS_C_SY, HPS_C_CHI, d.mg_tol_rel, d.mg_tol_abs, 200, st))) return e;
        if (gated_ion) {
            mark();
            mark();
            if ((e = push_with_ionization(islice, comp_push, mg_gate_after_enqueued(mg), true))) return e;
        }
        if (gated) {
            mark();
            mark();
            MgPost mp{};
            const bool posting = mg_take_deferred_post(mg, &mp);
            if ((e = advance_plasma_tiled(slab, el.pl, gm, comp_push, el.charge, el.mass, d.order, 0, d.n_subcycles, 0, el.tiling, d_nfallback, st, c_aabs, nullptr,
                                          posting ? nullptr : mg_gate_after_enqueued(mg), TailWork{}, posting ? &mp : nullptr))) return e;
        }
        if (laser_split && d.laser_solver == 2) { if ((e = laser_advance_slice(*this, islice)) || (e = laser_done())) return e; }
        pending_slice = islice; pend_fuse = fuse; pend_gated = gated; pend_gated_ion = gated_ion;
        HPS_HIP_CHECK(hipGetLastError());
        return HPS_OK;
    }
}

int Engine::push_with_ionization (int islice, const int comp[5], const int* go, bool first)
{
    int e;
    if ((e = ion_field_bounds())) return e;
    if (first) pend_ia = ion_args(islice);
    if ((e = advance_plasma_tiled(slab, ions.pl, gm, comp, ions.charge, ions.mass, d.order, 0, d.n_subcycles, 1, ions.tiling, d_nfallback, st, c_aabs, &pend_ia, go))) return e;
    TailWork tw = fold_tail_of(el, 256, &pend_covered);
    if (tw.nwg) tw.live_n = ion.d_cnt;
    return advance_plasma_tiled(slab, el.pl, gm, comp, el.charge, el.mass, d.order, 0, d.n_subcycles, 0, el.tiling, d_nfallback, st, c_aabs, nullptr, go, tw);
}

int Engine::solve_slice_finish (int islice)
{
    HPS_REQUIRE(pending_slice == islice, "hps_engine_solve_slice_finish: not the slice that hps_engine_solve_slice_begin started");
    pending_slice = -1;
    if (pc) return solve_slice_pc_finish(islice);
    SlabView f(slab);
    const long plane = slab.nstride;
    const dim3 b256(256);
    const dim3 gplane(ceil_div(plane, 256));
    const CellBox bb{beam_box.ilo, beam_box.ihi, beam_box.jlo, beam_box.jhi};
    const bool fuse = pend_fuse, gated = pend_gated, gated_ion = pend_gated_ion;
    const int comp_push[5] = {HPS_C_PSI, HPS_C_EZ, HPS_C_BX, HPS_C_BY, HPS_C_BZ};
    int e;
    {   int iters = 0, extra = 0;
        if ((e = mg_solve1_finish(mg, &iters, nullptr, &extra, st))) return e;
        total_vcycles += iters;
        if (gated && extra) { if ((e = species_advance(el, comp_push, 0))) return e; }
        if (gated_ion) {
            if (extra) { if ((e = push_with_ionization(islice, comp_push, nullptr, false))) return e; }
            if ((e = ionize_collect())) return e;
            if (el.pl.n > pend_covered) { if ((e = hps_advance_plasma_laser(slab, tail_of(el.pl, pend_covered, el.pl.n - pend_covered), gm, comp_push, c_aabs, el.charge, el.mass, d.order, 0, d.n_subcycles, 0, st))) return e; }
        } }

    if (salame_now() && !moving && nbeam > 0 && beam_off[d.nz - islice] - beam_off[d.nz - 1 - islice] > 0) {
        if ((e = salame_module(islice))) return e;
    }

    if (!gated && !gated_ion) {
    mark();
    if (diagnostics)
        hipLaunchKernelGGL(k_checksum, dim3(64, ncomp), b256, 0, st, f, ncomp, d_checksum);
    if ((e = fill_field_diagnostic(islice))) return e;
    if (d_insitu)
        hipLaunchKernelGGL(k_insitu_fields, dim3(64), b256, 0, st, f, gm.c, gm.dx*gm.dy*gm.dz, d_insitu, d.nz, islice);

    mark();
    {   const int* comp = comp_push;
        bool body_done = false; long body_covered = 0;
        if (ions.present()) {
            if (ions.tiling) {
                if ((e = ion_field_bounds())) return e;
                const IonArgs ia = ion_args(islice);
                if ((e = advance_plasma_tiled(slab, ions.pl, gm, comp, ions.charge, ions.mass, d.order, 0, d.n_subcycles, 1, ions.tiling, d_nfallback, st, c_aabs, &ia))) return e;
            } else {
                if ((e = ionize_slice(islice))) return e;
                if ((e = species_advance(ions, comp, 0))) return e;
            }
            if (el.tiling && el.tiling->sorted_n > 0 && !fuse) {
                TailWork tw = fold_tail_of(el, 256, &body_covered);
                if (tw.nwg) tw.live_n = ion.d_cnt;
                if ((e = advance_plasma_tiled(slab, el.pl, gm, comp, el.charge, el.mass, d.order, 0, d.n_subcycles, 0, el.tiling, d_nfallback, st, c_aabs, nullptr, nullptr, tw))) return e;
                body_done = true;
            }
            if ((e = ionize_collect())) return e;
        }
        if (fuse) {
            hipLaunchKernelGGL(k_shift_zero, gplane, b256, 0, st, slab.p, slab.nstride, plane, (int)slab.jstride, bb, d.deposit_rho ? (int)HPS_C_RHO : -1, (int)HPS_C_ION_RHOMJZ);
            const int dep[6] = {HPS_C_JX, HPS_C_JY, -1, d.deposit_rho ? HPS_C_RHO : -1, HPS_C_CHI, HPS_C_RHOMJZ};
            if ((e = advance_deposit_tiled(slab, el.pl, gm, comp, dep, el.charge, el.mass, d.order, d.n_subcycles, d.max_qsa, d_nqsa, el.tiling, d_nfallback, st))) return e;
            ahead_for = islice - 1;
        } else if (body_done) {
            if (el.pl.n > body_covered) { if ((e = hps_advance_plasma_laser(slab, tail_of(el.pl, body_covered, el.pl.n - body_covered), gm, comp, c_aabs, el.charge, el.mass, d.order, 0, d.n_subcycles, 0, st))) return e; }
        } else {
            if ((e = species_advance(el, comp, 0))) return e;
        } }
    }

    insitu_beam(islice);
    if (moving && nbeam > 0) { if ((e = beam_push_moving(*this, islice))) return e; }
    if (!coll.empty()) { if ((e = collide_slice(islice))) return e; }
    mark();
    if (ahead_for != islice - 1) {
        if (lazy_shift && islice > 0 && !salame_now()) shift_pending = true;
        else hipLaunchKernelGGL(k_shift_slices, gplane, b256, 0, st, slab.p, slab.nstride, plane, (int)slab.jstride, bb);
    }
    mark();
    HPS_HIP_CHECK(hipGetLastError());
    ++slices_done;
    return HPS_OK;
}


int Engine::salame_solve_ez ()
{
    const double fa = 1.0/(gm.ep0*gm.c);
    hipLaunchKernelGGL(k_rhs_lincomb, dim3(ceil_div(d.nx, 256), d.ny), dim3(256), 0, st, SlabView(slab), c_sal + HPS_SAL_JX, 0,
                       fa*0.5*(1.0/gm.dx), c_sal + HPS_SAL_JY, 1, fa*0.5*(1.0/gm.dy), staging);
    if (int e = open_boundary(1, 0x1u)) return e;
    return hps_poisson_solve(ps, staging, slab, c_sal + HPS_SAL_EZ, st);
}

int Engine::salame_module (int islice)
{
    SlabView f(slab);
    const long plane = slab.nstride;
    const dim3 b256(256), gplane(ceil_div(plane, 256)), gvalid(ceil_div(d.nx, 256), d.ny);
    const CellBox bb{beam_box.ilo, beam_box.ihi, beam_box.jlo, beam_box.jhi}, none{0, -1, 0, -1};
    const int S = c_sal;
    const int comp_push[5] = {HPS_C_PSI, HPS_C_EZ, HPS_C_BX, HPS_C_BY, HPS_C_BZ};
    const int dep_jxjy[6] = {S + HPS_SAL_JX, S + HPS_SAL_JY, -1, -1, -1, -1};
    auto zero = [&] (std::initializer_list<int> cs) {
        CompList z{0, {}}; for (int c : cs) z.c[z.n++] = c;
        hipLaunchKernelGGL(k_zero_comps, gplane, b256, 0, st, slab.p, slab.nstride, plane, (int)slab.jstride, z, CompList{0, {}}, none);
    };
    auto copy = [&] (std::initializer_list<int> dst, std::initializer_list<int> src) {
        CompList a{0, {}}, b{0, {}}; for (int c : dst) a.c[a.n++] = c; for (int c : src) b.c[b.n++] = c;
        hipLaunchKernelGGL(k_copy_comps, gplane, b256, 0, st, slab.p, slab.nstride, plane, a, b);
    };
    auto solve_bxby = [&] (int cB, int cS) -> int {
        int iters = 0;
        if (int e = hps_mg_solve1(mg, slab, cB, cS, HPS_C_CHI, d.mg_tol_rel, d.mg_tol_abs, 200, &iters, nullptr, st)) return e;
        total_vcycles += iters;
        return HPS_OK;
    };
    int e;

    if (islice + 1 != sal_last_slice) {
        copy({S + HPS_SAL_EZ_TARGET}, {HPS_C_EZ});
        sal_overloaded = false;
        sal_zeta_initial = islice*gm.dz + d.lo[2] + 0.5*gm.dz;
    }
    sal_last_slice = islice;

    zero({HPS_C_SY, HPS_C_SX});
    {   const int cache[4] = {HPS_C_BZ, HPS_C_EZ, HPS_C_EXMBY, HPS_C_EYPBX};
        const int depos[2] = {HPS_C_SY, HPS_C_SX};
        if ((e = species_explicit(el, cache, depos))) return e; }
    copy({S + HPS_SAL_SY_BACK, S + HPS_SAL_SX_BACK}, {HPS_C_SY, HPS_C_SX});

    const long first0 = beam_off[d.nz - 1 - islice], count = beam_off[d.nz - islice] - first0;
    double W = 1.0, W_total = 0.0;
    int iter = 0, used = 0; bool converged = false, undetermined = false;
    for (; iter < d.salame_n_iter; ++iter) {
        if ((e = species_advance(el, comp_push, 1))) return e;
        copy({S + HPS_SAL_JX, S + HPS_SAL_JY}, {HPS_C_N_JXB, HPS_C_N_JYB});
        if ((e = species_deposit(el, dep_jxjy))) return e;
        zero({S + HPS_SAL_EZ, S + HPS_SAL_JZB, S + HPS_SAL_SY, S + HPS_SAL_SX, S + HPS_SAL_BX, S + HPS_SAL_BY});
        if ((e = salame_solve_ez())) return e;
        copy({S + HPS_SAL_EZ_NO_SALAME}, {S + HPS_SAL_EZ});

        if ((e = deposit_beam_slice(islice, -1, -1, S + HPS_SAL_JZB))) return e;
        if ((e = hps_salame_sxsy_from_jz(slab, gm, S + HPS_SAL_JZB, S + HPS_SAL_SY, S + HPS_SAL_SX, st))) return e;
        if ((e = solve_bxby(S + HPS_SAL_BX, S + HPS_SAL_SY))) return e;
        zero({S + HPS_SAL_EZ, S + HPS_SAL_JX, S + HPS_SAL_JY});
        if (!d.salame_no_advance) {
            if (el.pl.n > 0) { if ((e = hps_salame_only_advance(slab, el.pl, gm, S + HPS_SAL_BX, S + HPS_SAL_BY, el.charge, el.mass, d.order, 0, st))) return e; }
            if ((e = species_deposit(el, dep_jxjy))) return e;
        } else {
            if ((e = hps_salame_jxjy_from_bxby(slab, gm, S + HPS_SAL_BX, S + HPS_SAL_BY, HPS_C_CHI, S + HPS_SAL_JX, S + HPS_SAL_JY, st))) return e;
        }
        if ((e = salame_solve_ez())) return e;

        zero({S + HPS_SAL_JZB});
        if ((e = deposit_beam_slice(islice, -1, -1, S + HPS_SAL_JZB))) return e;
        double s4[4];
        if ((e = salame_get_w_enqueue(slab, S + HPS_SAL_EZ_TARGET, S + HPS_SAL_EZ_NO_SALAME, S + HPS_SAL_EZ, S + HPS_SAL_JZB, d_sal, st))) return e;
        HPS_HIP_CHECK(hipMemcpyAsync(s4, salame_get_w_result(d_sal), sizeof(s4), hipMemcpyDeviceToHost, st));
// ... 16 lines not shown

        {   CompList zb{0, {}}; zb.c[zb.n++] = HPS_C_JZB;
            hipLaunchKernelGGL(k_zero_comps, gplane, b256, 0, st, slab.p, slab.nstride, plane, (int)slab.jstride, CompList{0, {}}, zb, bb); }
        if ((e = deposit_beam_slice(islice, -1, -1, HPS_C_JZB))) return e;
        deposit_grid_current(islice, HPS_C_JZB);
        hipLaunchKernelGGL(k_sxsy_beam, dim3(ceil_div(slab.jstride, 256), d.ny + 2*g), b256, 0, st, f, HPS_C_SX, HPS_C_SY, HPS_C_JZB, HPS_C_N_JXB, HPS_C_N_JYB,
                           HPS_C_P_JXB, HPS_C_P_JYB, gm.mu0, 2.0*gm.dx, 2.0*gm.dy, 2.0*gm.dz, bb, S + HPS_SAL_SX_BACK, S + HPS_SAL_SY_BACK);
        if ((e = solve_bxby(HPS_C_BX, HPS_C_SY))) return e;
        if (last) break;
    }
    double* o = sal_stats.data() + (size_t)4*islice;
    o[0] = W; o[1] = W_total; o[2] = (double)used; o[3] = (converged ? 1.0 : 0.0) + (sal_overloaded ? 2.0 : 0.0);
    HPS_HIP_CHECK(hipGetLastError());
    return HPS_OK;
}

int Engine::run_step ()
{
    if (int e = begin_step()) return e;
    for (int isl = d.nz - 1; isl >= 0; --isl)
        if (int e = solve_slice(isl)) return e;
    return HPS_OK;
}

}

using namespace hps;

extern "C" const char* hps_last_error (void) { return g_err.c_str(); }
extern "C" const char* hps_version (void) { return "hpslice 0.1 (gfx950)"; }

extern "C" int hps_engine_create (const hps_deck* deck, int device, void** handle)
{
    HPS_REQUIRE(deck && handle, "hps_engine_create: null argument");
    Engine* E = new Engine;
    if (int e = E->create(*deck, device)) { delete E; return e; }
    *handle = E;
    return HPS_OK;
}
extern "C" int hps_engine_destroy (void* h) { delete static_cast<Engine*>(h); return HPS_OK; }
extern "C" int hps_engine_begin_step (void* h) { return static_cast<Engine*>(h)->begin_step(); }
extern "C" int hps_engine_solve_slice (void* h, int islice) { return static_cast<Engine*>(h)->solve_slice(islice); }
extern "C" int hps_engine_solve_slice_begin (void* h, int islice) { return static_cast<Engine*>(h)->solve_slice_begin(islice); }
extern "C" int hps_engine_slice_ready (void* h)
{
    Engine* E = static_cast<Engine*>(h);
    if (E->pc) {
        if (!(E->pc_speculate && E->el.tiling && !E->moving && !E->ions.present()) || E->pc_islice < 0 || E->pc_enqueued <= 0) return 1;
        for (int it = 1; it <= E->pc_enqueued; ++it) {
            const volatile double* hp = E->h_pc + 8*it;
            const double seq = E->pc_base_seq + it;
            if (!(hp[1] == seq && hp[3] == seq && hp[5] == seq)) return 0;
            const double err = hp[0] > 0.0 ? hp[2]/hp[0] : 0.0;
            if (!(err > E->pc_tol) || it >= E->pc_max_iter) return 1;
        }
        return 1;
    }
    if (E->pending_slice < 0) return 1;
    return mg_solve1_ready(E->mg) ? 1 : 0;
}
extern "C" int hps_engine_solve_slice_finish (void* h, int islice) { return static_cast<Engine*>(h)->solve_slice_finish(islice); }
extern "C" int hps_engine_run_step (void* h) { return static_cast<Engine*>(h)->run_step(); }
extern "C" int hps_engine_sync (void* h)
{
    Engine* E = static_cast<Engine*>(h);
    E->flush_shift();
    if (int e = E->join_laser()) return e;
    HPS_HIP_CHECK(hipStreamSynchronize(E->st));
    if (E->moving && E->d_beam_overflow) {
        int ov = 0;
        HPS_HIP_CHECK(hipMemcpy(&ov, E->d_beam_overflow, sizeof(int), hipMemcpyDeviceToHost));
        HPS_REQUIRE(ov == 0, "moving beam: a slice outgrew the hand-off capacity (twice the fullest injected slice): particles were lost");
    }
    return HPS_OK;
}
extern "C" int hps_engine_info (void* h, int* ncomp, int* ng, long* np)
{
    Engine* E = static_cast<Engine*>(h);
    if (ncomp) *ncomp = E->ncomp;
    if (ng) *ng = E->g;
    if (np) *np = E->el.pl.n;
    return HPS_OK;
}
extern "C" hps_slab hps_engine_slab (void* h) { Engine* E = static_cast<Engine*>(h); E->flush_shift(); return E->slab; }
extern "C" hps_plasma hps_engine_plasma (void* h) { return static_cast<Engine*>(h)->el.pl; }
extern "C" int hps_engine_tiling (void* h, void** tiling)
{
    HPS_REQUIRE(h && tiling, "hps_engine_tiling: null argument");
    *tiling = static_cast<Engine*>(h)->el.tiling;
    return HPS_OK;
}
extern "C" hps_plasma hps_engine_ions (void* h)
{
    Engine* E = static_cast<Engine*>(h);
    (void)hipStreamSynchronize(E->st);
    return E->ions.pl;
}
extern "C" int hps_engine_ion_stats (void* h, long* n_ionized, long* n_product)
{
    Engine* E = static_cast<Engine*>(h);
    HPS_HIP_CHECK(hipStreamSynchronize(E->st));
    if (int e = E->ionize_collect()) return e;
    if (n_ionized) *n_ionized = E->ion.n_ionized;
    if (n_product) *n_product = E->el.pl.n;
    return HPS_OK;
}
extern "C" hps_stream hps_engine_stream (void* h) { return static_cast<Engine*>(h)->st; }
extern "C" int hps_engine_checksums (void* h, double* out)
{
    Engine* E = static_cast<Engine*>(h);
    HPS_HIP_CHECK(hipStreamSynchronize(E->st));
    HPS_HIP_CHECK(hipMemcpy(out, E->d_checksum, E->ncomp*sizeof(double), hipMemcpyDeviceToHost));
    return HPS_OK;
}
extern "C" int hps_engine_stats (void* h, long* vc, long* sl)
{
    Engine* E = static_cast<Engine*>(h);
    if (vc) *vc = E->total_vcycles;
    if (sl) *sl = E->slices_done;
    return HPS_OK;
}
extern "C" int hps_engine_set_insitu_plasma (void* h, double radius)
{
    Engine* E = static_cast<Engine*>(h);
    HPS_HIP_CHECK(hipStreamSynchronize(E->st));
    (void)hipFree(E->d_insitu_pl); E->d_insitu_pl = nullptr; E->insitu_pl_radius = radius;
    if (!(radius > 0.0)) return HPS_OK;
    HPS_HIP_CHECK(hipMalloc(&E->d_insitu_pl, (size_t)15*E->d.nz*sizeof(double)));
    HPS_HIP_CHECK(hipMemset(E->d_insitu_pl, 0, (size_t)15*E->d.nz*sizeof(double)));
    return HPS_OK;
}
extern "C" int hps_engine_set_insitu_beam (void* h, double radius)
{
    Engine* E = static_cast<Engine*>(h);
    HPS_HIP_CHECK(hipStreamSynchronize(E->st));
    (void)hipFree(E->d_insitu_bm); E->d_insitu_bm = nullptr; E->insitu_bm_radius = radius;
    if (!(radius > 0.0)) return HPS_OK;
    HPS_HIP_CHECK(hipMalloc(&E->d_insitu_bm, (size_t)23*E->d.nz*sizeof(double)));
    HPS_HIP_CHECK(hipMemset(E->d_insitu_bm, 0, (size_t)23*E->d.nz*sizeof(double)));
    return HPS_OK;
}
extern "C" int hps_engine_insitu_beam (void* h, double* out)
{
    Engine* E = static_cast<Engine*>(h);
    HPS_REQUIRE(E->d_insitu_bm && out, "hps_engine_insitu_beam: not switched on");
    HPS_HIP_CHECK(hipStreamSynchronize(E->st));
    const int nz = E->d.nz;
    HPS_HIP_CHECK(hipMemcpy(out, E->d_insitu_bm, (size_t)23*nz*sizeof(double), hipMemcpyDeviceToHost));
    for (int k = 0; k < nz; ++k) {
        const double sw = out[k], inv = sw <= 0.0 ? 0.0 : 1.0/sw;
        for (int q = 1; q <= 21; ++q) out[(size_t)q*nz + k] *= inv;
    }
    return HPS_OK;
}
extern "C" int hps_engine_insitu_plasma (void* h, double* out)
{
    Engine* E = static_cast<Engine*>(h);
    HPS_REQUIRE(E->d_insitu_pl && out, "hps_engine_insitu_plasma: not switched on");
    HPS_HIP_CHECK(hipStreamSynchronize(E->st));
    const int nz = E->d.nz;
    HPS_HIP_CHECK(hipMemcpy(out, E->d_insitu_pl, (size_t)15*nz*sizeof(double), hipMemcpyDeviceToHost));
    for (int k = 0; k < nz; ++k) {
        const double sw = out[k], inv = sw <= 0.0 ? 0.0 : 1.0/sw;
        for (int q = 1; q <= 12; ++q) out[(size_t)q*nz + k] *= inv;
    }
    return HPS_OK;
}
// ... 549 lines not shown
```

hipace_amd/csrc/multigrid.hip:

```cpp
#include "common.h"
#include <type_traits>
#include "mg_gate.h"
#include "slab_ops.h"

#include <vector>
#include <algorithm>
#include <cmath>
#include <cstring>

namespace hps {

struct FView {
    double* p; long js, ns; int oi, oj;
    __device__ __forceinline__ double& operator() (int i, int j, int n) const {
        const unsigned o = (unsigned)((i + oi) + (j + oj)*(int)js + n*(int)ns)*8u;
        return *reinterpret_cast<double*>(reinterpret_cast<char*>(p) + o);
    }
};

struct LevBox { int lox, loy, hix, hiy;
                int vlx, vly, vhx, vhy; };

enum { SRC_ZERO = 0, SRC_DIRECT = 1, SRC_PROLONG = 2 };

// ... 838 lines not shown
    if (!last) {
        double q0[4];
        blk_residual(B, i, j, cc_box(nx, ny), a, fx, fy, q0);
        if (B.act) {
            const int pn = d.nx[l+1] + 2, psn = pn*(d.ny[l+1] + 2);
            base[d.off[l+1] + psn + ((j >> 1) + 1)*pn + (i >> 1) + 1] = 0.25*(q0[0] + q0[1] + q0[2] + q0[3]);
        }
        lvl_sync<WAVE>();
    }
}

template <bool WAVE>
__device__ __forceinline__ void low_up_s (lds_double* base, const Low2& d, int l, int t, double fx, double fy)
{
    const int nx = d.nx[l], ny = d.ny[l];
    Blk B; int i, j;
    blk_geometry(B, base + d.off[l], nx, ny, t, fx, fy, i, j);
    const int ps = B.pitch*(ny + 2);
    const lds_double* r = B.c0 + ps;
    const lds_double* cf = base + d.coff[l] + (B.c0 - (base + d.off[l]));
    const int ok[4] = {0, 1, B.pitch, B.pitch + 1};
    const int pn = d.nx[l+1] + 2;
    const lds_double* kc = base + d.off[l+1] + ((j >> 1) + 1)*pn + (i >> 1) + 1;
    const double k0 = B.act ? kc[0] : 0.0;
#pragma unroll
    for (int k = 0; k < 4; ++k) {
        const int o = B.ok[k] ? ok[k] : 0;
        B.r0[k] = r[o]; B.ci[k] = cf[ps + o];
        const double c0 = B.c0[o];
        B.v0[k] = B.ok[k] ? c0 + k0 : 0.0;
        if (B.ok[k]) B.c0[o] = B.v0[k];
    }
    lvl_sync<WAVE>();
    blk_sweep<0, WAVE>(B); blk_sweep<1, WAVE>(B); blk_sweep<0, WAVE>(B); blk_sweep<1, WAVE>(B);
}

__device__ __forceinline__ void tiny_down_s (lds_double* base, const Low2& d, int l, int t, double fx, double fy)
{
    const int nx = d.nx[l], ny = d.ny[l], pitch = nx + 2, ps = pitch*(ny + 2);
    const int i = t & 7, j = t >> 3;
    const bool ok = (i < nx) && (j < ny);
    const int o = ok ? (j + 1)*pitch + i + 1 : pitch + 1;
    lds_double* c0 = base + d.off[l] + o;
    const lds_double* cf = base + d.coff[l] + o;
    const double r0 = c0[ps], a = cf[0], ci = cf[ps];
    const double fxm = wall_mult<true>(i, 0, nx - 1, fx), fym = wall_mult<true>(j, 0, ny - 1, fy);
    if (ok && (((i + j) & 1) == 0)) c0[0] = r0*ci;
    lvl_sync<true>();
    for (int s = 1; s < 4; ++s) {
        if (ok && (((i + j + s) & 1) == 0)) c0[0] = (r0 - offdiag_m((const lds_double*)c0, pitch, fxm, fym))*ci;
        lvl_sync<true>();
    }
    const LevBox b = cc_box(nx, ny);
    const double u0 = residual_at<false>((const lds_double*)c0, pitch, i, j, b, r0, a, fx, fy);
    const double q0 = ok ? u0 : 0.0;
    const double b0 = __shfl_down(q0, 1), g0 = __shfl_down(q0, 8), e0 = __shfl_down(q0, 9);
    if (ok && !(i & 1) && !(j & 1)) {
        const int pn = d.nx[l+1] + 2, psn = pn*(d.ny[l+1] + 2);
        base[d.off[l+1] + psn + ((j >> 1) + 1)*pn + (i >> 1) + 1] = 0.25*(q0 + b0 + g0 + e0);
    }
    lvl_sync<true>();
}

__device__ __forceinline__ void tiny_up_s (lds_double* base, const Low2& d, int l, int t, double fx, double fy)
{
    const int nx = d.nx[l], ny = d.ny[l], pitch = nx + 2, ps = pitch*(ny + 2);
    const int i = t & 7, j = t >> 3;
    const bool ok = (i < nx) && (j < ny);
    const int o = ok ? (j + 1)*pitch + i + 1 : pitch + 1;
    lds_double* c0 = base + d.off[l] + o;
    const double r0 = c0[ps], ci = base[d.coff[l] + ps + o];
    const double fxm = wall_mult<true>(i, 0, nx - 1, fx), fym = wall_mult<true>(j, 0, ny - 1, fy);
    if (ok) {
        const int pn = d.nx[l+1] + 2;
        c0[0] = c0[0] + base[d.off[l+1] + ((j >> 1) + 1)*pn + (i >> 1) + 1];
    }
    lvl_sync<true>();
    for (int s = 0; s < 4; ++s) {
        if (ok && (((i + j + s) & 1) == 0)) c0[0] = (r0 - offdiag_m((const lds_double*)c0, pitch, fxm, fym))*ci;
        lvl_sync<true>();
    }
}

__global__ __launch_bounds__(1024)
void k_lower_v3 (const Low2* __restrict__ dp, const double* __restrict__ acf_g, const double* __restrict__ cinv_g,
                 const double* __restrict__ res_g, double* __restrict__ cor_g, double* __restrict__ coef_g, int nxA, int nyA, int ctot,
                 double facx0, double facy0, int nsweeps_bottom, StopRule sr)
{
    extern __shared__ __attribute__((aligned(16))) double lds_raw[];
    lds_double* base = (lds_double*)lds_raw;
    const int t = threadIdx.x;
    const Low2& d = *dp;
    const int nl = d.nl;
    const int cellsA = nxA*nyA;
    res_g += (long)blockIdx.x*cellsA; cor_g += (long)blockIdx.x*cellsA;
    const LevBox bA = cc_box(nxA, nyA);
    Blk A; int iA, jA;
    blk_geometry(A, base, nxA, nyA, t, facx0, facy0, iA, jA);
    double aA[4], rA[4];
#pragma unroll
    for (int k = 0; k < 4; ++k) {
        const int i = iA + (k & 1), j = jA + (k >> 1);
        const int g = min(i, nxA - 1) + min(j, nyA - 1)*nxA;
        const double v0 = res_g[g], v2 = acf_g[g], v3 = cinv_g[g];
        rA[k] = A.ok[k] ? v0 : 0.0; aA[k] = A.ok[k] ? v2 : 0.0; A.ci[k] = A.ok[k] ? v3 : 0.0;
        A.r0[k] = rA[k];
    }
    const bool derive = (sr.k <= 0);
    constexpr int NIMG = 4;
    double img[NIMG];
#pragma unroll
    for (int m = 0; m < NIMG; ++m) { const int q = min(t + 1024*m, ctot - 1); img[m] = derive ? 0.0 : coef_g[q]; }
    const bool active = vcycle_active(sr);
#pragma unroll
    for (int k = 0; k < 4; ++k) { HPS_KEEP(rA[k]); HPS_KEEP(aA[k]); HPS_KEEP(A.ci[k]); }
#pragma unroll
    for (int m = 0; m < NIMG; ++m) HPS_KEEP(img[m]);
    if (!active) return;
    MG_STAMP(8);
    for (int l = 0; l < nl; ++l) {
        const int n1 = (d.nx[l] + 2)*(d.ny[l] + 2);
        lds_double* c = base + d.off[l];
        for (int s = t; s < n1; s += 1024) c[s] = 0.0;
    }
    if (!derive) {
#pragma unroll
        for (int m = 0; m < NIMG; ++m) if (t + 1024*m < ctot) base[d.cbase + t + 1024*m] = img[m];
        for (int q = t + 1024*NIMG; q < ctot; q += 1024) base[d.cbase + q] = coef_g[q];
    }
    __syncthreads();
    if (derive) {
        if (nl > 1 && A.act) {
            const int p1 = d.nx[1] + 2;
            base[d.coff[1] + ((jA >> 1) + 1)*p1 + (iA >> 1) + 1] = 0.25*(aA[0] + aA[1] + aA[2] + aA[3]);
        }
        __syncthreads();
        for (int l = 1; l < nl; ++l) {
            const double fx = lvl_fac(facx0, l), fy = lvl_fac(facy0, l);
            const int nx = d.nx[l], ny = d.ny[l];
            Blk B; int i, j;
            blk_geometry(B, base + d.coff[l], nx, ny, t, fx, fy, i, j);
            const int ps = B.pitch*(ny + 2);
            lds_double* acf = B.c0;
            const int ok[4] = {0, 1, B.pitch, B.pitch + 1};
            if (B.act) {
                double a[4];
#pragma unroll
                for (int k = 0; k < 4; ++k) a[k] = B.ok[k] ? acf[ok[k]] : 0.0;
                if (l + 1 < nl) {
                    const int pn = d.nx[l+1] + 2;
                    base[d.coff[l+1] + ((j >> 1) + 1)*pn + (i >> 1) + 1] = 0.25*(a[0] + a[1] + a[2] + a[3]);
                }
#pragma unroll
                for (int k = 0; k < 4; ++k)
                    if (B.ok[k]) acf[ps + ok[k]] = 1.0/diag_c0<true>(i + (k & 1), j + (k >> 1), cc_box(nx, ny), a[k], fx, fy);
            }
            __syncthreads();
        }
        if (blockIdx.x == 0) for (int q = t; q < ctot; q += 1024) coef_g[q] = base[d.cbase + q];
    }
    MG_STAMP(9);
    const bool bottomA = (nl == 1);
    blk_down_sweeps<false>(A, bottomA ? nsweeps_bottom : 4);
    if (!bottomA) {
        double q0[4];
        blk_residual(A, iA, jA, bA, aA, facx0, facy0, q0);
        if (A.act) {
            const int p1 = d.nx[1] + 2, ps1 = p1*(d.ny[1] + 2);
            base[d.off[1] + ps1 + ((jA >> 1) + 1)*p1 + (iA >> 1) + 1] = 0.25*(q0[0] + q0[1] + q0[2] + q0[3]);
        }
        __syncthreads();
// ... 156 lines not shown
            if (i >= 1 && i <= o.vhx[l] && j >= 1 && j <= o.vhy[l]) {
                const double* f = cur + (2*lj)*w + 2*li;
                v = (1./16.)*(f[0] + 2.*f[1] + f[2]
                            + 2.*f[w] + 4.*f[w + 1] + 2.*f[w + 2]
                            + f[2*w] + 2.*f[2*w + 1] + f[2*w + 2]);
                if (i >= ox && j >= oy) out(i, j, 0) = v;
            }
            if (l < np) nxt[e] = v;
        }
        __syncthreads();
        cur = nxt; w = wl;
    }
}
static size_t nodal_pyramid_lds (int np)
{
    size_t n = 0;
    for (int l = 0; l < np; ++l) { const int s = np - l; const size_t w = (size_t)NPYR_NB*(1 << s) + (1 << s) - 1; n += w*w; }
    return n*sizeof(double);
}

__global__ void k_level_cinv (const double* __restrict__ acf, double* __restrict__ cinv, int nx, int ny, double fx, double fy)
{
    const int i = blockIdx.x*blockDim.x + threadIdx.x, j = blockIdx.y;
    if (i < nx && j < ny) cinv[i + (long)j*nx] = 1.0/diag_c0<true>(i, j, cc_box(nx, ny), acf[i + (long)j*nx], fx, fy);
}

__global__ void k_copy2 (LevBox b, FView dst, FView src)
{
    const int i = b.vlx + blockIdx.x*blockDim.x + threadIdx.x;
    const int j = b.vly + blockIdx.y;
    if (i > b.vhx || j > b.vhy) return;
    dst(i, j, 0) = src(i, j, 0); dst(i, j, 1) = src(i, j, 1);
}

template <bool CC>
__global__ __launch_bounds__(256)
void k_bottom_sweep (LevBox b, FView cor, FView rhs, FView acf, double facx, double facy, int is, StopRule sr)
{
    if (!vcycle_active(sr)) return;
    const int i = b.vlx + blockIdx.x*blockDim.x + threadIdx.x;
    const int j = b.vly + blockIdx.y;
    if (i > b.vhx || j > b.vhy) return;
    if (is < 0) { cor(i, j, 0) = 0.0; cor(i, j, 1) = 0.0; return; }
    if ((i + j + is) & 1) return;
    const double ci = 1.0/diag_c0<CC>(i, j, b, acf(i, j, 0), facx, facy);
    for (int n = 0; n < 2; ++n) {
        const double w = (i > b.lox) ? cor(i-1, j, n) : 0.0, e = (i < b.hix) ? cor(i+1, j, n) : 0.0;
        const double s = (j > b.loy) ? cor(i, j-1, n) : 0.0, no = (j < b.hiy) ? cor(i, j+1, n) : 0.0;
        double lx = facx*(w + e), ly = facy*(s + no);
        if (CC) {
            lx = (i == b.lox) ? facx*(4./3.)*e : ((i == b.hix) ? facx*(4./3.)*w : lx);
            ly = (j == b.loy) ? facy*(4./3.)*no : ((j == b.hiy) ? facy*(4./3.)*s : ly);
        }
        cor(i, j, n) = (rhs(i, j, n) - (lx + ly))*ci;
    }
}

struct MGLevelDev { LevBox b; long cells; double *acf, *res, *cor, *rescor; };

constexpr long LOWV_MAX_CELLS = 34*34;
constexpr long SMALL_TILE_CELLS = 300L*300L;

constexpr int MG_GO_WORD = 8;
struct SolveRun { int enq, nspec, nzeroed, max_iters; double tol_rel, tol_abs; bool cc; };

struct Multigrid {
    bool cc; int nx, ny; double dx, dy;
    bool hierarchy_ready = false;
    bool nodal_pull1 = false;
    std::vector<MGLevelDev> L;
    int lowv_begin = 1;
    LowLev* d_low = nullptr; size_t low_lds = 0;
    bool bottom = false;
    unsigned long long *d_buf = nullptr, *h_buf = nullptr;
    unsigned long long* h_buf_dev = nullptr;
    long dbg_trips = 0, dbg_solves = 0, dbg_hist[8] = {0,0,0,0,0,0,0,0};
    unsigned long long* h_seq = nullptr; unsigned long long* h_seq_dev = nullptr; unsigned long long seq = 0;
    unsigned long long* d_norms = nullptr;
    unsigned long long* h_norms = nullptr;
    int last_iters = 1;
    SolveRun run{};
    bool defer_post = false; bool deferred_valid = false; MgPost deferred{};
    bool use_low3 = false; Low2 low3{}; Low2* d_low3 = nullptr; size_t low3_lds = 0;
    double* cinvA = nullptr;
    double* coef_img = nullptr;
    double* tmp0 = nullptr;
    bool cor_in_tmp = false;
    FView sol, rhs, acf0;

    ~Multigrid () {
        for (auto& l : L) { (void)hipFree(l.acf); (void)hipFree(l.res); (void)hipFree(l.cor); (void)hipFree(l.rescor); }
        if (getenv("HPS_MG_DEBUG")) fprintf(stderr, "mg: solves %ld trips %ld hist %ld %ld %ld %ld %ld %ld\n", dbg_solves, dbg_trips, dbg_hist[0], dbg_hist[1], dbg_hist[2], dbg_hist[3], dbg_hist[4], dbg_hist[5]);
        (void)hipFree(d_buf); (void)hipFree(d_low); (void)hipFree(tmp0); (void)hipFree(d_low3); (void)hipFree(cinvA); (void)hipFree(coef_img);
        if (h_buf) (void)hipHostFree(h_buf);
    }
    FView lv (int il, double* p) const {
        const MGLevelDev& l = L[il];
        const long nxb = l.b.hix - l.b.lox + 1;
        return FView{p, nxb, l.cells, -l.b.lox, -l.b.loy};
    }
    int nlev () const { return (int)L.size(); }
    bool pulls (int il) const {
        return !cc && ((il >= 2 && ((il < lowv_begin && L[il].cells <= SMALL_TILE_CELLS) ||
                                    (il == lowv_begin && !use_low3 && !bottom))) ||
                       (il == 1 && nodal_pull1));
    }
};

static size_t device_max_lds ()
{
    static const size_t lim = [] {
        int dev = 0, a = 0, b = 0;
        if (hipGetDevice(&dev) != hipSuccess) return (size_t)0;
        if (hipDeviceGetAttribute(&a, hipDeviceAttributeMaxSharedMemoryPerBlock, dev) != hipSuccess) a = 0;
        if (hipDeviceGetAttribute(&b, hipDeviceAttributeSharedMemPerBlockOptin, dev) != hipSuccess) b = 0;
        return (size_t)std::max(a, b);
    }();
    return lim;
}

int mg_create (int nx, int ny, double dx, double dy, Multigrid** out)
{
    if (nx % 2 != ny % 2) { set_error("hps_mg_create: nx and ny must have the same parity"); return HPS_ERR_ARG; }
    HPS_REQUIRE((long)(nx + 16)*(ny + 16) < (1L << 27), "hps_mg_create: the kernels address a two-component plane pair by 32-bit byte offsets (at most 2^27 cells per plane)");
    Multigrid* M = new Multigrid;
    M->cc = (nx % 2 == 0); M->nx = nx; M->ny = ny; M->dx = dx; M->dy = dy;
    int hx = M->cc ? nx - 1 : nx + 1, hy = M->cc ? ny - 1 : ny + 1;
    for (int il = 0; il < 31; ++il) {
        MGLevelDev l{};
        l.b.lox = 0; l.b.loy = 0; l.b.hix = hx; l.b.hiy = hy;
        if (M->cc) { l.b.vlx = 0; l.b.vly = 0; l.b.vhx = hx; l.b.vhy = hy; }
        else       { l.b.vlx = 1; l.b.vly = 1; l.b.vhx = hx - 1; l.b.vhy = hy - 1; }
        l.cells = (long)(hx + 1)*(hy + 1);
        HPS_HIP_CHECK(hipMalloc(&l.acf, l.cells*sizeof(double)));
        HPS_HIP_CHECK(hipMalloc(&l.res, 2*l.cells*sizeof(double)));
        HPS_HIP_CHECK(hipMalloc(&l.cor, 2*l.cells*sizeof(double)));
        HPS_HIP_CHECK(hipMalloc(&l.rescor, 2*l.cells*sizeof(double)));
        HPS_HIP_CHECK(hipMemset(l.acf, 0, l.cells*sizeof(double)));
        HPS_HIP_CHECK(hipMemset(l.res, 0, 2*l.cells*sizeof(double)));
        HPS_HIP_CHECK(hipMemset(l.cor, 0, 2*l.cells*sizeof(double)));
        HPS_HIP_CHECK(hipMemset(l.rescor, 0, 2*l.cells*sizeof(double)));
        M->L.push_back(l);
        bool ok;
        const int nxl = hx + 1, nyl = hy + 1;
        if (M->cc) { ok = nxl >= 4 && nyl >= 4 && nxl % 2 == 0 && nyl % 2 == 0; if (ok) { hx = nxl/2 - 1; hy = nyl/2 - 1; } }
        else       { ok = nxl >= 8 && nyl >= 8 && hx % 2 == 0 && hy % 2 == 0;   if (ok) { hx /= 2; hy /= 2; } }
        if (!ok) break;
    }
    if (M->nlev() < 2) { delete M; set_error("hps_mg_create: grid too small to coarsen"); return HPS_ERR_ARG; }
    if (!M->cc)
        HPS_HIP_CHECK(hipFuncSetAttribute((const void*)k_nodal_acf_pyramid<5>, hipFuncAttributeMaxDynamicSharedMemorySize, (int)nodal_pyramid_lds(NPYR_MAX)));
    const int nl = M->nlev();
    M->lowv_begin = nl - 1;
    for (int il = nl - 1; il >= 1; --il) if (M->L[il].cells <= LOWV_MAX_CELLS) M->lowv_begin = il;
    if (M->cc) {
        for (int il = 1; il < nl; ++il) {
            const LevBox& b = M->L[il].b;
            const bool fits = (b.hix + 1 <= 64) && (b.hiy + 1 <= 64) && (nl - il <= LOW2_MAXLEV)
                           && (il + 1 >= nl || (M->L[il+1].b.hix + 1 <= 32 && M->L[il+1].b.hiy + 1 <= 32));
            if (!fits) continue;
            M->use_low3 = true; M->lowv_begin = il;
            Low2& e = M->low3;
            e.nl = nl - il;
            int off3 = 0;
            for (int k = 0; k < e.nl; ++k) {
                const LevBox& bk = M->L[il + k].b;
                e.nx[k] = bk.hix + 1; e.ny[k] = bk.hiy + 1; e.off[k] = off3;
                off3 += (k == 0 ? 1 : 2)*(e.nx[k] + 2)*(e.ny[k] + 2);
            }
            e.cbase = off3; e.coff[0] = off3;
            for (int k = 1; k < e.nl; ++k) { e.coff[k] = off3; off3 += 2*(e.nx[k] + 2)*(e.ny[k] + 2); }
            e.ctot = std::max(off3 - e.cbase, 1);
            e.total = off3;
            HPS_HIP_CHECK(hipMalloc(&M->coef_img, (size_t)e.ctot*sizeof(double)));
            HPS_HIP_CHECK(hipMemset(M->coef_img, 0, (size_t)e.ctot*sizeof(double)));
            M->low3_lds = (size_t)off3*sizeof(double);
            if (M->low3_lds > 64*1024)
                HPS_HIP_CHECK(hipFuncSetAttribute((const void*)k_lower_v3, hipFuncAttributeMaxDynamicSharedMemorySize, (int)M->low3_lds));
            HPS_HIP_CHECK(hipMalloc(&M->d_low3, sizeof(Low2)));
            HPS_HIP_CHECK(hipMemcpy(M->d_low3, &e, sizeof(Low2), hipMemcpyHostToDevice));
            HPS_HIP_CHECK(hipMalloc(&M->cinvA, (size_t)e.nx[0]*e.ny[0]*sizeof(double)));
            break;
        }
    }
    if (!M->use_low3) {
        long cells = 0;
        for (int il = M->lowv_begin; il < nl; ++il) cells += M->L[il].cells;
        M->low_lds = (size_t)(8*cells)*sizeof(double);
        hipFuncAttributes fa{};
        HPS_HIP_CHECK(hipFuncGetAttributes(&fa, M->cc ? (const void*)k_lower_v<true> : (const void*)k_lower_v<false>));
        if (M->low_lds + fa.sharedSizeBytes > device_max_lds()) { M->bottom = true; M->lowv_begin = nl - 1; M->low_lds = 0; }
    }
    M->nodal_pull1 = !M->cc && M->lowv_begin > 1;
    if (!M->use_low3 && !M->bottom) {
        std::vector<LowLev> low;
        int off = 0;
        for (int il = M->lowv_begin; il < nl; ++il) {
            const MGLevelDev& l = M->L[il];
            low.push_back(LowLev{l.b, l.b.hix - l.b.lox + 1, (int)l.cells, off});
            off += 8*(int)l.cells;
        }
        if (M->low_lds > 64*1024) {
            HPS_HIP_CHECK(hipFuncSetAttribute((const void*)k_lower_v<true>, hipFuncAttributeMaxDynamicSharedMemorySize, (int)M->low_lds));
            HPS_HIP_CHECK(hipFuncSetAttribute((const void*)k_lower_v<false>, hipFuncAttributeMaxDynamicSharedMemorySize, (int)M->low_lds));
        }
        HPS_HIP_CHECK(hipMalloc(&M->d_low, low.size()*sizeof(LowLev)));
        HPS_HIP_CHECK(hipMemcpy(M->d_low, low.data(), low.size()*sizeof(LowLev), hipMemcpyHostToDevice));
    }
    HPS_HIP_CHECK(hipMalloc(&M->d_buf, (3 + MG_MAX_VCYCLES)*MG_NSUB*sizeof(unsigned long long)));
    HPS_HIP_CHECK(hipHostMalloc(&M->h_buf, ((3 + MG_MAX_VCYCLES)*MG_NSUB + 8)*sizeof(unsigned long long), hipHostMallocMapped));
    HPS_HIP_CHECK(hipHostGetDevicePointer((void**)&M->h_buf_dev, M->h_buf, 0));
    M->h_seq = M->h_buf + (3 + MG_MAX_VCYCLES)*MG_NSUB; M->h_seq_dev = M->h_buf_dev + (3 + MG_MAX_VCYCLES)*MG_NSUB;
    *M->h_seq = 0ULL;
    HPS_HIP_CHECK(hipMemset(M->d_buf, 0, (3 + MG_MAX_VCYCLES)*MG_NSUB*sizeof(unsigned long long)));
    memset(M->h_buf, 0, (3 + MG_MAX_VCYCLES)*MG_NSUB*sizeof(unsigned long long));
    M->d_norms = M->d_buf + MG_NSUB; M->h_norms = M->h_buf + MG_NSUB;
    HPS_HIP_CHECK(hipMalloc(&M->tmp0, 2*M->L[0].cells*sizeof(double)));
    HPS_HIP_CHECK(hipMemset(M->tmp0, 0, 2*M->L[0].cells*sizeof(double)));
    *out = M;
    return HPS_OK;
}

template <class TS, bool CC, int SRC, bool DO_RES, int NSW = 4, bool RPULL = false>
static void launch_smooth_ts (Multigrid* M, int il, FView phi_out, FView phi_out2, FView rhs, FView acf, FView phi_in, FView crse,
                              FView res_out, FView cres_out, unsigned long long* resnorm, unsigned long long* rhsnorm,
                              const StopRule& sr, hipStream_t st)
{
    const LevBox& b = M->L[il].b;
    constexpr int E = DO_RES ? NSW : NSW - 1;
    constexpr int FX = TS::TX - 2*E, FY = TS::TY - 2*E;
    const int ntx = ceil_div(b.vhx - b.vlx + 1, FX), nty = ceil_div(b.vhy - b.vly + 1, FY);
    const double fac = (double)(1 << il);
    const double ldx = M->dx*fac, ldy = M->dy*fac;
    const double facx = 1.0/(ldx*ldx), facy = 1.0/(ldy*ldy);
    constexpr bool FUSE = CC && DO_RES;
    hipLaunchKernelGGL((k_smooth<TS, CC, SRC, DO_RES, FUSE, NSW, RPULL>), dim3(ntx*nty), dim3(TS::NT), 0, st, b, phi_out, phi_out2, rhs, acf,
                       phi_in, crse, res_out, cres_out, facx, facy, ntx, resnorm, rhsnorm, sr);
}

template <bool CC, int SRC, bool DO_RES>
static void launch_smooth (Multigrid* M, int il, FView phi_out, FView phi_out2, FView rhs, FView acf, FView phi_in, FView crse,
                           FView res_out, FView cres_out, unsigned long long* resnorm, unsigned long long* rhsnorm,
                           const StopRule& sr, hipStream_t st)
{
    if (M->L[il].cells <= SMALL_TILE_CELLS)
        launch_smooth_ts<TileSmall, CC, SRC, DO_RES>(M, il, phi_out, phi_out2, rhs, acf, phi_in, crse, res_out, cres_out, resnorm, rhsnorm, sr, st);
    else
        launch_smooth_ts<TileBig, CC, SRC, DO_RES>(M, il, phi_out, phi_out2, rhs, acf, phi_in, crse, res_out, cres_out, resnorm, rhsnorm, sr, st);
}

template <bool CC>
static void restrict_residual_if_nodal (Multigrid* M, int il, const StopRule& sr, hipStream_t st)
{
    if (CC) return;
    const LevBox& cb = M->L[il+1].b;
    hipLaunchKernelGGL(k_restrict<CC>, dim3(ceil_div(cb.vhx - cb.vlx + 1, 64), cb.vhy - cb.vly + 1), dim3(64), 0, st,
                       cb, M->lv(il+1, M->L[il+1].res), M->lv(il, M->L[il].rescor), 2, sr);
}

template <bool CC>
static void vcycle (Multigrid* M, int k, double tol_rel, double tol_abs, hipStream_t st)
{
    const int nl = M->nlev();
    const int lb = M->lowv_begin;
    const FView none{};
    const StopRule sr{M->d_norms, k, tol_rel, tol_abs};
    for (int il = 1; il < lb; ++il) {
        if (!M->pulls(il))
            launch_smooth<CC, SRC_ZERO, true>(M, il, M->lv(il, M->L[il].cor), none, M->lv(il, M->L[il].res), M->lv(il, M->L[il].acf), none,
                                              none, M->lv(il, M->L[il].rescor), M->lv(il+1, M->L[il+1].res), nullptr, nullptr, sr, st);
        else if constexpr (!CC) {
            if (M->L[il].cells > SMALL_TILE_CELLS)
                launch_smooth_ts<TileMid, CC, SRC_ZERO, true, 4, true>(M, il, M->lv(il, M->L[il].cor), none, M->lv(il, M->L[il].res), M->lv(il, M->L[il].acf), none,
                                                                       M->lv(il-1, M->L[il-1].rescor), M->lv(il, M->L[il].rescor), M->lv(il+1, M->L[il+1].res), nullptr, nullptr, sr, st);
            else
                launch_smooth_ts<TileSmall, CC, SRC_ZERO, true, 4, true>(M, il, M->lv(il, M->L[il].cor), none, M->lv(il, M->L[il].res), M->lv(il, M->L[il].acf), none,
                                                                         M->lv(il-1, M->L[il-1].rescor), M->lv(il, M->L[il].rescor), M->lv(il+1, M->L[il+1].res), nullptr, nullptr, sr, st);
        }
        if (!M->pulls(il + 1)) restrict_residual_if_nodal<CC>(M, il, sr, st);
    }
    {
        const double fac = (double)(1 << lb);
        const double ldx = M->dx*fac, ldy = M->dy*fac;
        const LevBox& bb = M->L[nl-1].b;
        const int nsweeps = std::max(16, (std::max(bb.hix - bb.lox + 1, bb.hiy - bb.loy + 1) + 1)/2*2);
        if (M->bottom) {
            const FView cor = M->lv(lb, M->L[lb].cor), rhs = M->lv(lb, M->L[lb].res), acf = M->lv(lb, M->L[lb].acf);
            const dim3 grid(ceil_div(bb.vhx - bb.vlx + 1, 64), bb.vhy - bb.vly + 1);
            for (int is = -1; is < nsweeps; ++is)
                hipLaunchKernelGGL(k_bottom_sweep<CC>, grid, dim3(64), 0, st, bb, cor, rhs, acf, 1.0/(ldx*ldx), 1.0/(ldy*ldy), is, sr);
        } else if (M->use_low3)
            hipLaunchKernelGGL(k_lower_v3, dim3(2), dim3(1024), M->low3_lds, st, M->d_low3, M->L[lb].acf, M->cinvA, M->L[lb].res, M->L[lb].cor,
                               M->coef_img, M->low3.nx[0], M->low3.ny[0], M->low3.ctot, 1.0/(ldx*ldx), 1.0/(ldy*ldy), nsweeps, sr);
        else
            hipLaunchKernelGGL(k_lower_v<CC>, dim3(CC ? 1 : 2), dim3(1024), M->low_lds, st, M->d_low, nl - lb, M->L[lb].acf, M->L[lb].res,
                               M->L[lb].cor, 1.0/(ldx*ldx), 1.0/(ldy*ldy), nsweeps, sr, M->pulls(lb) ? M->lv(lb-1, M->L[lb-1].rescor) : FView{});
    }
    for (int il = lb - 1; il >= 1; --il) {
        double* crse = (il + 1 == lb) ? M->L[il+1].cor : M->L[il+1].rescor;
        launch_smooth<CC, SRC_PROLONG, false>(M, il, M->lv(il, M->L[il].rescor), none, M->lv(il, M->L[il].res), M->lv(il, M->L[il].acf),
                                              M->lv(il, M->L[il].cor), M->lv(il+1, crse), none, none, nullptr, nullptr, sr, st);
    }
    {
        double* crse = (1 == lb) ? M->L[1].cor : M->L[1].rescor;
        double* in = M->cor_in_tmp ? M->tmp0 : M->L[0].cor;
        double* out = M->cor_in_tmp ? M->L[0].cor : M->tmp0;
        launch_smooth_ts<typename HugeTileOf<CC>::type, CC, SRC_PROLONG, true, 8>(M, 0, M->lv(0, out), M->sol, M->rhs, M->acf0, M->lv(0, in), M->lv(1, crse),
                                                             M->lv(0, M->L[0].rescor), M->lv(1, M->L[1].res), M->d_norms + (2 + k)*MG_NSUB,
                                                             nullptr, sr, st);
        M->cor_in_tmp = !M->cor_in_tmp;
    }
    if (!M->nodal_pull1) restrict_residual_if_nodal<CC>(M, 0, sr, st);
}

__global__ __launch_bounds__(256)
void k_post_norms (const unsigned long long* __restrict__ src, volatile unsigned long long* dst, int nwords,
                   volatile unsigned long long* seq_slot, unsigned long long seq, int* go_word, StopRule after)
{
    {   const bool act = vcycle_active(after);
        if (threadIdx.x == 0) *go_word = act ? 0 : 1; }
    for (int w = threadIdx.x; w < nwords; w += blockDim.x) dst[w] = src[w];
    HPS_HOST_STORES_ACKNOWLEDGED();
    __syncthreads();
    if (threadIdx.x == 0) { *seq_slot = seq; }
}

template <bool CC>
static void enqueue_cycles (Multigrid* M, hipStream_t st)
{
    SolveRun& r = M->run;
    for (int v = 0; v < r.nspec && r.enq < r.max_iters; ++v, ++r.enq) {
        if (r.enq >= r.nzeroed) {
            const int more = std::min(r.max_iters - r.nzeroed, 64);
            (void)hipMemsetAsync(M->d_norms + (2 + r.nzeroed)*MG_NSUB, 0, more*MG_NSUB*sizeof(unsigned long long), st);
            r.nzeroed += more;
        }
        vcycle<CC>(M, r.enq, r.tol_rel, r.tol_abs, st);
    }
    ++M->seq; ++M->dbg_trips;
    if (M->defer_post) {
        M->defer_post = false; M->deferred_valid = true;
        M->deferred = MgPost{M->d_buf, (volatile unsigned long long*)M->h_buf_dev, (3 + r.enq)*MG_NSUB, (volatile unsigned long long*)M->h_seq_dev, M->seq,
                             StopRule{M->d_norms, r.enq, r.tol_rel, r.tol_abs}};
        return;
    }
    hipLaunchKernelGGL(k_post_norms, dim3(1), dim3(256), 0, st, M->d_buf, (volatile unsigned long long*)M->h_buf_dev,
                       (3 + r.enq)*MG_NSUB, (volatile unsigned long long*)M->h_seq_dev, M->seq,
                       reinterpret_cast<int*>(M->d_buf) + MG_GO_WORD, StopRule{M->d_norms, r.enq, r.tol_rel, r.tol_abs});
}

struct GuestPass { bool on = false; SlabView f{hps_slab{}}; GradPsiSxSy ga{}; };

template <bool CC>
static int solve1_hierarchy (Multigrid* M, int max_iters, hipStream_t st, const GuestPass* guest = nullptr)
{
    const int lb = M->lowv_begin;
    max_iters = std::min(max_iters, MG_MAX_VCYCLES);
    const StopRule always{nullptr, -1, 0.0, 0.0};
    int nspec = std::min(std::max(M->last_iters, 1), std::max(max_iters, 1));
    int nzeroed = std::min(max_iters, nspec + 8);
    const int nzero_words = (2 + nzeroed)*MG_NSUB;
    int first = 1;
    if (CC) {
        PyrOut po{};
        const int np = std::min(lb, 5);
        for (int il = 1; il <= np; ++il) { po.p[il-1] = M->L[il].acf; po.nx[il-1] = M->L[il].b.hix + 1; po.ny[il-1] = M->L[il].b.hiy + 1; }
        const double lfac = (double)(1 << lb), lfx = 1.0/(M->dx*lfac*M->dx*lfac), lfy = 1.0/(M->dy*lfac*M->dy*lfac);
        if (M->use_low3 && lb <= np) { po.cinv = M->cinvA; po.cinv_l = lb - 1; po.cfx = lfx; po.cfy = lfy; }
        if (guest) {
            const int gx = ceil_div(M->nx, 32), gy = ceil_div(M->ny, 32);
            const SlabView& f = guest->f;
            const int nbx = ceil_div(f.js, 256), rows = f.ny + 2*f.ng;
            hipLaunchKernelGGL(k_hierarchy_gradpsi, dim3(gx*gy + nbx*rows), dim3(256), 0, st, M->acf0, M->nx, M->ny, po, np, M->d_norms, nzero_words,
                               gx, gy, f, guest->ga, nbx);
        } else
        hipLaunchKernelGGL(k_acf_pyramid, dim3(ceil_div(M->nx, 32), ceil_div(M->ny, 32)), dim3(256), 0, st, M->acf0, M->nx, M->ny, po, np,
                           M->d_norms, nzero_words);
// ... 67 lines not shown
        {   volatile unsigned long long* hs = M->h_seq;
            long spins = 0;
            while (*hs != M->seq) {
                if ((++spins & 0xfffff) == 0 && hipStreamQuery(st) != hipErrorNotReady) {
                    if (*hs == M->seq) break;
                    HPS_HIP_CHECK(hipStreamSynchronize(st));
                    if (*hs != M->seq) { set_error("hps_mg_solve1: the norm read-back never arrived"); return HPS_ERR_HIP; }
                }
            }
            __atomic_thread_fence(__ATOMIC_ACQUIRE); }
        const double res0 = slot_value(0), rhs0 = slot_value(1);
        const double max_norm = (rhs0 >= res0) ? rhs0 : res0;
        const double target = std::max(r.tol_abs, std::max(r.tol_rel, 1.e-16)*max_norm);
        last_norm = res0; iters = 0;
        converged = (res0 <= target); diverged = false;
        for (int k = 0; k < r.enq && !converged && !diverged; ++k) {
            last_norm = slot_value(2 + k); ++iters;
            if (last_norm <= target) converged = true;
            else if (!(last_norm <= 1.e20*max_norm)) diverged = true;
        }
        if (first_trip) {
            const double prev = (r.enq == 0) ? res0 : slot_value(2 + r.enq - 1);
            const bool gate_active = prev > target && prev <= 1.e20*max_norm;
            if (gate_active != !(converged || diverged)) { set_error("hps_mg_solve1: host and device stopping rules disagree"); return HPS_ERR_HIP; }
            if (extra) *extra = gate_active ? 1 : 0;
            first_trip = false;
        }
        if (converged || diverged) break;
        if (r.enq >= r.max_iters) { set_error("hps_mg_solve1: not converged after max_iters V-cycles"); status = HPS_ERR_MG_MAXITER; break; }
        r.nspec = 1;
        enqueue_cycles<CC>(M, st);
    }
    if (diverged) { set_error("hps_mg_solve1: diverging"); status = HPS_ERR_MG_DIVERGED; }
    M->last_iters = std::max(1, iters); ++M->dbg_solves; ++M->dbg_hist[std::min(iters, 7)];
    if (iters == 0) {
        const LevBox& b0 = M->L[0].b;
        hipLaunchKernelGGL(k_copy2, dim3(ceil_div(b0.vhx - b0.vlx + 1, 64), b0.vhy - b0.vly + 1), dim3(64), 0, st,
                           b0, M->sol, M->lv(0, M->L[0].cor));
    }
    HPS_HIP_CHECK(hipGetLastError());
    if (iters_out) *iters_out = iters;
    if (resnorm_out) *resnorm_out = last_norm;
    return status;
}

static void set_views (Multigrid* M, const hps_slab& s, int sol_comp, int rhs_comp, int acf_comp)
{
    const int sh = M->cc ? 0 : 1;
    const int o = s.ng - sh;
    M->sol  = FView{s.p + (long)sol_comp*s.nstride, s.jstride, s.nstride, o, o};
    M->rhs  = FView{s.p + (long)rhs_comp*s.nstride, s.jstride, s.nstride, o, o};
    M->acf0 = FView{s.p + (long)acf_comp*s.nstride, s.jstride, s.nstride, o, o};
}

int mg_solve1_begin (void* handle, hps_slab s, int sol_comp, int rhs_comp, int acf_comp, double tol_rel, double tol_abs,
                     int max_iters, hipStream_t st)
{
    Multigrid* M = static_cast<Multigrid*>(handle);
    HPS_REQUIRE(s.nstride < (1L << 27) && s.ng <= 8, "mg_solve1_begin: planes of at most 2^27 doubles and at most 8 guard cells (32-bit byte offsets in the kernels)");
    set_views(M, s, sol_comp, rhs_comp, acf_comp);
    return M->cc ? solve1_begin<true>(M, tol_rel, tol_abs, max_iters, st) : solve1_begin<false>(M, tol_rel, tol_abs, max_iters, st);
}
int mg_solve1_prepare (void* handle, hps_slab s, int sol_comp, int rhs_comp, int acf_comp, int max_iters, hipStream_t st)
{
    Multigrid* M = static_cast<Multigrid*>(handle);
    set_views(M, s, sol_comp, rhs_comp, acf_comp);
    if (int e = M->cc ? solve1_hierarchy<true>(M, max_iters, st) : solve1_hierarchy<false>(M, max_iters, st)) return e;
    M->hierarchy_ready = true;
    return HPS_OK;
}
int mg_solve1_prepare_with (void* handle, hps_slab s, int sol_comp, int rhs_comp, int acf_comp, int max_iters, SlabView f, GradPsiSxSy ga,
                            hipStream_t st, bool* done)
{
    Multigrid* M = static_cast<Multigrid*>(handle);
    *done = false;
    if (!M->cc) return HPS_OK;
    set_views(M, s, sol_comp, rhs_comp, acf_comp);
    GuestPass g; g.on = true; g.f = f; g.ga = ga;
    if (int e = solve1_hierarchy<true>(M, max_iters, st, &g)) return e;
    M->hierarchy_ready = true;
    *done = true;
    return HPS_OK;
}
void mg_solve1_forget_hierarchy (void* handle) { if (handle) static_cast<Multigrid*>(handle)->hierarchy_ready = false; }
void mg_defer_post (void* handle) { Multigrid* M = static_cast<Multigrid*>(handle); M->defer_post = true; M->deferred_valid = false; }
bool mg_take_deferred_post (void* handle, MgPost* out)
{
    Multigrid* M = static_cast<Multigrid*>(handle);
    M->defer_post = false;
    if (!M->deferred_valid) return false;
    M->deferred_valid = false; *out = M->deferred;
    return true;
}
const int* mg_gate_after_enqueued (void* handle)
{
    return reinterpret_cast<const int*>(static_cast<Multigrid*>(handle)->d_buf) + MG_GO_WORD;
}
bool mg_solve1_ready (void* handle)
{
    Multigrid* M = static_cast<Multigrid*>(handle);
    return *(volatile unsigned long long*)M->h_seq == M->seq;
}
int mg_solve1_finish (void* handle, int* iters_out, double* resnorm_out, int* extra, hipStream_t st)
{
    Multigrid* M = static_cast<Multigrid*>(handle);
    return M->cc ? solve1_finish<true>(M, iters_out, resnorm_out, extra, st) : solve1_finish<false>(M, iters_out, resnorm_out, extra, st);
}

int mg_solve1 (Multigrid* M, hps_slab s, int sol_comp, int rhs_comp, int acf_comp, double tol_rel, double tol_abs,
               int max_iters, int* iters_out, double* resnorm_out, hipStream_t st)
{
    if (int e = mg_solve1_begin(M, s, sol_comp, rhs_comp, acf_comp, tol_rel, tol_abs, max_iters, st)) return e;
    return mg_solve1_finish(M, iters_out, resnorm_out, nullptr, st);
}

}

using namespace hps;

extern "C" int hps_mg_create (int nx, int ny, double dx, double dy, void** handle)
{
    HPS_REQUIRE(nx >= 2 && ny >= 2 && handle, "hps_mg_create: bad size");
    Multigrid* M = nullptr;
    if (int e = mg_create(nx, ny, dx, dy, &M)) return e;
    *handle = M;
    return HPS_OK;
}

extern "C" int hps_mg_info (void* handle, int* cc, int* nlev, int* lowv_begin, int* lowv_kind, long* lowv_lds, int* tiles,
                            int* nodal_pull1, int* pyr_levels, int* pyr_restricts)
{
    HPS_REQUIRE(handle, "hps_mg_info: null handle");
    const Multigrid* M = static_cast<const Multigrid*>(handle);
    const int lb = M->lowv_begin;
    if (cc) *cc = M->cc;
    if (nlev) *nlev = M->nlev();
    if (lowv_begin) *lowv_begin = lb;
    if (lowv_kind) *lowv_kind = M->bottom ? HPS_MG_LOWV_BOTTOM : M->use_low3 ? HPS_MG_LOWV_V3 : M->cc ? HPS_MG_LOWV_CC : HPS_MG_LOWV_NODAL;
    if (lowv_lds) *lowv_lds = (long)(M->use_low3 ? M->low3_lds : M->low_lds);
    if (tiles) {
        for (int il = 0; il < HPS_MG_MAXLEV; ++il) {
            int t = -1;
            if (il < lb) {
                const bool small = M->L[il].cells <= SMALL_TILE_CELLS;
                t = M->pulls(il) ? (small ? HPS_MG_TILE_SMALL_PULL : HPS_MG_TILE_MID_PULL) : (small ? HPS_MG_TILE_SMALL : HPS_MG_TILE_BIG);
            }
            tiles[il] = t;
        }
    }
    if (nodal_pull1) *nodal_pull1 = M->nodal_pull1;
    if (pyr_levels) *pyr_levels = std::min(lb, M->cc ? 5 : NPYR_MAX);
    if (pyr_restricts) *pyr_restricts = lb - std::min(lb, M->cc ? 5 : NPYR_MAX);
    return HPS_OK;
}

extern "C" int hps_mg_solve1 (void* handle, hps_slab slab, int sol_comp, int rhs_comp, int acoef_comp, double tol_rel,
                              double tol_abs, int max_iters, int* iters_host, double* resnorm_host, hps_stream stream)
{
    HPS_REQUIRE(handle && slab.p, "hps_mg_solve1: null argument");
    Multigrid* M = static_cast<Multigrid*>(handle);
    HPS_REQUIRE(slab.nx == M->nx && slab.ny == M->ny, "hps_mg_solve1: slab size does not match the solver");
    HPS_REQUIRE(sol_comp >= 0 && sol_comp + 1 < slab.ncomp && rhs_comp >= 0 && rhs_comp + 1 < slab.ncomp &&
                acoef_comp >= 0 && acoef_comp < slab.ncomp, "hps_mg_solve1: bad component");
    HPS_REQUIRE(M->cc || slab.ng >= 1, "hps_mg_solve1: node-centred solve needs >= 1 guard cell");
    HPS_REQUIRE(slab.nstride < (1L << 27) && slab.ng <= 8, "hps_mg_solve1: planes of at most 2^27 doubles and at most 8 guard cells (32-bit byte offsets in the kernels)");
    return mg_solve1(M, slab, sol_comp, rhs_comp, acoef_comp, tol_rel, tol_abs, max_iters, iters_host, resnorm_host,
                     (hipStream_t)stream);
}

extern "C" int hps_mg_solve1_fabs (void* handle, hps_slab sol2, hps_slab rhs2, hps_slab acoef1, double tol_rel, double tol_abs,
                                   int max_iters, int* iters_host, double* resnorm_host, hps_stream stream)
{
    HPS_REQUIRE(handle && sol2.p && rhs2.p && acoef1.p, "hps_mg_solve1_fabs: null argument");
    Multigrid* M = static_cast<Multigrid*>(handle);
// ... 46 lines not shown
```

hipace_amd/csrc/slab_ops.h:

```cpp
#ifndef HPS_SLAB_OPS_H_
#define HPS_SLAB_OPS_H_

#include "common.h"

namespace hps {

struct CellBox { int ilo, ihi, jlo, jhi; };

struct GradPsiSxSy { int cPsi, cExmBy, cEypBx; double hdx_inv, hdy_inv; int cSx, cSy, cJzb, cNx, cNy, cPx, cPy;
                     double mu0, dx2, dy2, dz2; CellBox bb; };

__device__ __forceinline__ void gradpsi_sxsy_cell (const SlabView& f, const GradPsiSxSy& a, int i, int j)
{
    if (i >= f.nx + f.ng) return;
    const long o = f.off(i, j);
    const int gg = f.ng - 1;
    if (i >= -gg && i < f.nx + gg && j >= -gg && j < f.ny + gg) {
        const double* P = f.p + a.cPsi*f.ns + o;
        f.p[a.cExmBy*f.ns + o] = -(P[1] - P[-1])*a.hdx_inv;
        f.p[a.cEypBx*f.ns + o] = -(P[f.js] - P[-f.js])*a.hdy_inv;
    }
    const int ia = i + f.ng, ja = j + f.ng;
    if (i < 0 || i >= f.nx || j < 0 || j >= f.ny || ia < a.bb.ilo || ia > a.bb.ihi || ja < a.bb.jlo || ja > a.bb.jhi) {
        f.p[a.cSy*f.ns + o] = 0.0; f.p[a.cSx*f.ns + o] = 0.0; return;
    }
    const double* J = f.p + a.cJzb*f.ns + o;
    const double dx_jzb = (J[1] - J[-1])/a.dx2;
    const double dy_jzb = (J[f.js] - J[-f.js])/a.dy2;
    const double dz_jxb = (f.p[a.cPx*f.ns + o] - f.p[a.cNx*f.ns + o])/a.dz2;
    const double dz_jyb = (f.p[a.cPy*f.ns + o] - f.p[a.cNy*f.ns + o])/a.dz2;
    f.p[a.cSy*f.ns + o] =  a.mu0*(-dy_jzb + dz_jyb);
    f.p[a.cSx*f.ns + o] = -a.mu0*(-dx_jzb + dz_jxb);
}

}
#endif
```

include/hpslice.h:

```cpp
#ifndef HPSLICE_H_
#define HPSLICE_H_

#include <stdint.h>

#ifdef __cplusplus
extern "C" {
#endif

typedef void* hps_stream;

enum { HPS_OK = 0, HPS_ERR_ARG = 1, HPS_ERR_HIP = 2, HPS_ERR_FFT = 3, HPS_ERR_MG_DIVERGED = 4,
       HPS_ERR_MG_MAXITER = 5, HPS_ERR_COMM = 6, HPS_ERR_UNSUPPORTED = 7 };

enum { HPS_BC_REFLECTING = 0, HPS_BC_PERIODIC = 1, HPS_BC_ABSORBING = 2 };

typedef struct {
    double* p;
    int nx, ny, ng, ncomp;
    long jstride, nstride;
} hps_slab;

typedef struct {
    double *x, *y, *w, *ux, *uy, *psi, *x_prev, *y_prev, *ux_half, *uy_half, *psi_half;
    uint64_t* idcpu;
// ... 94 lines not shown
int hps_mg_solve1_fabs (void* handle, hps_slab sol2, hps_slab rhs2, hps_slab acoef1, double tol_rel, double tol_abs,
                        int max_iters, int* iters_host, double* resnorm_host, hps_stream stream);
enum { HPS_MG_LOWV_V3 = 0, HPS_MG_LOWV_CC = 1, HPS_MG_LOWV_NODAL = 2, HPS_MG_LOWV_BOTTOM = 3 };
enum { HPS_MG_TILE_SMALL = 0, HPS_MG_TILE_BIG = 1, HPS_MG_TILE_SMALL_PULL = 2, HPS_MG_TILE_MID_PULL = 3 };
enum { HPS_MG_MAXLEV = 31 };
int hps_mg_info (void* handle, int* cc, int* nlev, int* lowv_begin, int* lowv_kind, long* lowv_lds, int* tiles,
                 int* nodal_pull1, int* pyr_levels, int* pyr_restricts);
int hps_mg_destroy (void* handle);

int hps_mg2_create (int nx, int ny, double dx, double dy, void** handle);
int hps_mg2_solve2 (void* handle, double* sol2_dev, const double* rhs2_dev, const double* acoef_real_dev,
                    const double* acoef_imag_dev, double tol_rel, double tol_abs, int max_iters, int* iters_host,
                    double* resnorm_host, hps_stream stream);
enum { HPS_MG2_BOTTOM_LOWER_V = 0, HPS_MG2_BOTTOM_SINGLE_BLOCK = 1, HPS_MG2_BOTTOM_PER_SWEEP = 2 };
enum { HPS_MG2_TILE_SINGLE_BLOCK = 0, HPS_MG2_TILE_SMALL = 1, HPS_MG2_TILE_BIG = 2 };
int hps_mg2_info (void* handle, int* nlev, int* low_top, int* bottom, int* tiles);
int hps_mg2_destroy (void* handle);


#define HPS_MAX_ION_LEVELS 56
typedef struct {
    int nx, ny, nz; double lo[3], hi[3];
    int order; int deriv_type;
    int plasma_ppc[2]; double plasma_density; double plasma_radius;
    double plasma_charge, plasma_mass; double max_qsa; int n_subcycles;
    int beam_profile;
    double beam_zmin, beam_zmax, beam_radius, beam_density;
    double beam_umean[3], beam_pos_mean[3], beam_pos_std[3]; int beam_ppc[3]; double beam_charge;
    int bc; double mg_tol_rel, mg_tol_abs; int deposit_rho; int n_steps;
    double dt; int beam_n_subcycles; double beam_mass; double ext_E_slope[2];
    int bxby_solver; double predcorr_tol; int predcorr_max_iter; double predcorr_mix; int field_bc;
    int laser_on; double laser_a0, laser_w0, laser_L0, laser_lambda0, laser_pos[3];
    double laser_zfoc; int laser_solver; int laser_use_phase;
    int si_units;
    int grid_current_on; double grid_current_peak, grid_current_mean[3], grid_current_std[3];
    double laser_mg_tol_rel, laser_mg_tol_abs;
    int beam_radiation_reaction; double background_density_SI; int beam_no_z_push;
    int plasma_no_neutralize;
    int ion_on; int ion_ppc[2]; double ion_density, ion_mass, ion_charge; int ion_init_level, ion_Z;
    double ion_energies[HPS_MAX_ION_LEVELS]; unsigned long long ion_seed;
    int beam_spin_tracking; double beam_initial_spin[3]; double beam_spin_anom;
    int dt_adaptive; double nt_per_betatron, dt_max, adaptive_threshold_uz, adaptive_phase_tolerance;
    int adaptive_no_predict_step, adaptive_no_phase_control, adaptive_phase_substeps;
    double adaptive_density, max_time, beam_uz_std;
    double ext_Ez_slope;
    int beam_do_salame; int salame_n_iter; double salame_relative_tolerance; int salame_no_advance;
    double salame_Ez_target_slope;
} hps_deck;

enum { HPS_SAL_EZ_TARGET = 0, HPS_SAL_EZ_NO_SALAME, HPS_SAL_EZ, HPS_SAL_JX, HPS_SAL_JY, HPS_SAL_JZB, HPS_SAL_BX, HPS_SAL_BY,
       HPS_SAL_SY, HPS_SAL_SX, HPS_SAL_SY_BACK, HPS_SAL_SX_BACK, HPS_SAL_NCOMP };

enum { HPS_C_N_JXB = 0, HPS_C_N_JYB, HPS_C_CHI, HPS_C_SY, HPS_C_SX, HPS_C_EXMBY, HPS_C_EYPBX,
       HPS_C_EZ, HPS_C_BX, HPS_C_BY, HPS_C_BZ, HPS_C_PSI, HPS_C_JXB, HPS_C_JYB, HPS_C_JZB,
       HPS_C_JX, HPS_C_JY, HPS_C_RHOMJZ, HPS_C_P_JXB, HPS_C_P_JYB, HPS_C_ION_RHOMJZ, HPS_C_RHO,
       HPS_NCOMP_MAX };

enum { HPS_PC_N_JX = 0, HPS_PC_N_JY, HPS_PC_EXMBY, HPS_PC_EYPBX, HPS_PC_EZ, HPS_PC_BX, HPS_PC_BY, HPS_PC_BZ,
       HPS_PC_PSI, HPS_PC_JX, HPS_PC_JY, HPS_PC_JZ, HPS_PC_RHOMJZ, HPS_PC_P_BX, HPS_PC_P_BY, HPS_PC_P_JX,
       HPS_PC_P_JY, HPS_PC_ION_RHOMJZ, HPS_PC_IT_BX, HPS_PC_IT_BY, HPS_PC_PIT_BX, HPS_PC_PIT_BY, HPS_PC_RHO,
       HPS_PC_NCOMP_MAX };

int hps_engine_create (const hps_deck* deck, int device, void** handle);
int hps_engine_destroy (void* handle);
int hps_engine_begin_step (void* handle);
int hps_engine_set_step (void* handle, int step);
int hps_engine_set_time (void* handle, double t, double dt);
int hps_engine_beam_moments (void* handle, double* out4_host);
int hps_engine_solve_slice (void* handle, int islice);
int hps_engine_solve_slice_begin (void* handle, int islice);
int hps_engine_solve_slice_finish (void* handle, int islice);
int hps_engine_slice_ready (void* handle);
int hps_engine_run_step (void* handle);
int hps_engine_sync (void* handle);
int hps_engine_info (void* handle, int* ncomp, int* nguards, long* nparticles);
hps_slab hps_engine_slab (void* handle);
hps_plasma hps_engine_plasma (void* handle);
int hps_engine_tiling (void* handle, void** tiling);
hps_plasma hps_engine_ions (void* handle);
int hps_engine_ion_stats (void* handle, long* n_ionized_host, long* n_product_host);
hps_stream hps_engine_stream (void* handle);
int hps_engine_checksums (void* handle, double* out_host);
int hps_engine_stats (void* handle, long* total_vcycles, long* slices_done);
int hps_engine_pc_stats (void* handle, long* iterations, double* error_sum);
int hps_engine_pc_zero_b_slices (void* handle, long* slices);
int hps_engine_laser_info (void* handle, int* aabs_comp, double* envelope_abs_sum_host);
int hps_engine_laser_envelope (void* handle, double* out_host);
int hps_engine_set_laser_import (void* handle, int on, int step);
int hps_engine_export_laser_slice (void* handle, int islice, double* msg_dev);
int hps_engine_import_laser_slice (void* handle, int islice, const double* msg_dev);
int hps_engine_import_laser_from (void* handle, int islice, void* src_engine);
int hps_engine_set_laser_grid (void* handle, const int* n_cell , const double* patch_lo ,
                               const double* patch_hi , int interp_order);
int hps_engine_laser_grid (void* handle, int* nxl, int* nyl, int* zeta_lo, int* zeta_hi);
int hps_engine_laser_chi (void* handle, double* out_host);
int hps_laser_interp_aabs (hps_slab slab, int c_aabs, const double* a_plane, int nxl, int nyl, double dxl, double dyl,
                           double xoffl, double yoffl, hps_geom geom, int order, void* stream);
int hps_laser_interp_chi (hps_slab slab, int c_chi, const double* chi_initial, double* chi_out, int nxl, int nyl, double dxl,
                          double dyl, double xoffl, double yoffl, hps_geom geom, int shrink, int order, void* stream);
typedef struct { double a0, w0, L0, pos[3], zfoc, cep, propagation_angle_yz, pft_yz; } hps_laser_pulse;
int hps_engine_set_laser_pulses (void* handle, int n, const hps_laser_pulse* pulses);
int hps_engine_add_laser_samples (void* handle, int geometry, const double* data_host, const long extent[3],
                                  const double offset[3], const double spacing[3], double unit);
int hps_engine_set_insitu_laser (void* handle, int on);
int hps_engine_insitu_laser (void* handle, double* out_host );
int hps_engine_set_diagnostics (void* handle, int on);
int hps_engine_set_field_diagnostic (void* handle, int ncomps, const int* comps, const int coarsening[3]);
int hps_engine_field_diagnostic (void* handle, double* out_host);
int hps_engine_set_field_diagnostic_box (void* handle, int ncomps, const int* comps, const int coarsening[3], int slice_dir,
                                         const double* patch_lo , const double* patch_hi );
int hps_engine_field_diagnostic_geometry (void* handle, int* n3, double* lo3, double* hi3);

int hps_engine_set_insitu_fields (void* handle, int on);
int hps_engine_insitu_fields (void* handle, double* out_host );

int hps_engine_set_insitu_plasma (void* handle, double radius);
int hps_engine_laser_vcycles (void* handle, long* vcycles);
int hps_engine_set_insitu_beam (void* handle, double radius);
int hps_engine_insitu_beam (void* handle, double* out_host );
int hps_engine_insitu_plasma (void* handle, double* out_host );

int hps_engine_set_tiling (void* handle, int tile_size, int sort_period);
int hps_engine_fallbacks (void* handle, long* n_fallback_host);
int hps_engine_set_density_profile (void* handle, int nr, const double* r_host, const double* fr_host, int nt,
                                    const double* ct_host, const double* ft_host);
int hps_engine_set_plasma_init (void* handle, const int* plasma_fine_ppc, const int* ion_fine_ppc, double hollow_core_radius);
int hps_engine_set_fine_patch (void* handle, const unsigned char* mask_host, int transition_cells);
int hps_engine_set_plasma_momentum (void* handle, int species, const double u_mean[3], const double u_std[3], unsigned long long seed);
int hps_engine_set_plasma_symmetry (void* handle, int do_symmetrize, int prevent_centered_particle);
int hps_engine_set_fusion (void* handle, int on);
int hps_engine_sorts (void* handle, long* n_sorts_host);
int hps_engine_set_profiling (void* handle, int on);
int hps_engine_set_profiling_stride (void* handle, int stride);
int hps_engine_phase_times (void* handle, double* ms_host, long* nslices_host);

int hps_engine_beam_info (void* handle, long* nbeam_host, long* offsets_host );
int hps_engine_set_beam_particles (void* handle, long n, const double* soa_host, long* n_outside);
int hps_engine_set_beam_storage (void* handle, double* storage_dev );
int hps_engine_initial_beam (void* handle, double* dst_dev);
int hps_engine_beam_state (void* handle, long* boundaries_host, double* soa_host);
int hps_engine_beam_capacity (void* handle, long* cap_host);
int hps_engine_set_beam_capacity (void* handle, long cap);
int hps_engine_beam_message_rows (void* handle, int* rows_host);
int hps_engine_beam_spin (void* handle, double* soa_host);
int hps_engine_set_beam_import (void* handle, int on);
int hps_engine_export_beam_slice (void* handle, int islice, double* msg_dev);
int hps_engine_import_beam_slice (void* handle, int islice, const double* msg_dev);
int hps_engine_assume_initial_beam_support (void* handle);

int hps_engine_record_event (void* handle, int slot, void** event_out);
int hps_stream_pool_shared_pairs (int device);
int hps_engine_wait_event (void* handle, void* event);
int hps_engine_copy_async (void* handle, void* dst_dev, const void* src_dev, long bytes);

int hps_open_boundary (double* staging_dev, int nbatch, int nx, int ny, const double lo[2], const double hi[2],
                       unsigned no_monopole_mask, void* stream);

int hps_engine_salame_stats (void* handle, double* out_host );
int hps_salame_only_advance (hps_slab slab, hps_plasma plasma, hps_geom geom, int bx_comp, int by_comp, double charge,
                             double mass, int depos_order, int can_ionize, hps_stream stream);
int hps_salame_jxjy_from_bxby (hps_slab slab, hps_geom geom, int bx_comp, int by_comp, int chi_comp, int jx_comp, int jy_comp,
                               hps_stream stream);
int hps_salame_sxsy_from_jz (hps_slab slab, hps_geom geom, int jz_comp, int sy_comp, int sx_comp, hps_stream stream);
int hps_salame_get_w (hps_slab slab, int ez_target_comp, int ez_no_salame_comp, int ez_comp, int jz_comp, double* scratch_dev,
                      double* out4_host, hps_stream stream);
int hps_salame_scale_beam_slice (double* w_dev, long n, double W, hps_stream stream);
// ... 108 lines not shown
```

Measured before the change: 1705.

## Ride next-slice shift/zero-init on idle CUs of the multigrid coarse-level kernel

```diff
diff --git a/hipace_amd/_lib.py b/hipace_amd/_lib.py
--- a/hipace_amd/_lib.py
+++ b/hipace_amd/_lib.py
@@ -180,6 +180,7 @@
     "hps_beam_sort_by_box": (C.c_int, [C.c_void_p, C.c_long, C.c_double, C.c_double, C.c_int, C.c_void_p, C.c_void_p,
                                        C.c_void_p, C.c_void_p]),
     "hps_engine_stats": (C.c_int, [C.c_void_p, C.POINTER(C.c_long), C.POINTER(C.c_long)]),
+    "hps_engine_early_init_slices": (C.c_int, [C.c_void_p, C.POINTER(C.c_long)]),
     "hps_engine_set_insitu_plasma": (C.c_int, [C.c_void_p, C.c_double]),
     "hps_engine_set_insitu_beam": (C.c_int, [C.c_void_p, C.c_double]),
     "hps_engine_insitu_beam": (C.c_int, [C.c_void_p, C.c_void_p]),
diff --git a/hipace_amd/api.py b/hipace_amd/api.py
--- a/hipace_amd/api.py
+++ b/hipace_amd/api.py
@@ -1110,7 +1110,9 @@
     def stats(self):
         vc, sl = C.c_long(), C.c_long()
         check(_lib.lib().hps_engine_stats(self._h, C.byref(vc), C.byref(sl)))
-        return dict(vcycles=vc.value, slices=sl.value)
+        ei = C.c_long()
+        check(_lib.lib().hps_engine_early_init_slices(self._h, C.byref(ei)))
+        return dict(vcycles=vc.value, slices=sl.value, early_init=ei.value)
 
     def slab(self):
         self.sync()
diff --git a/hipace_amd/csrc/engine.h b/hipace_amd/csrc/engine.h
--- a/hipace_amd/csrc/engine.h
+++ b/hipace_amd/csrc/engine.h
@@ -27,6 +27,7 @@
 int mg_solve1_prepare (void* mg_handle, hps_slab s, int sol_comp, int rhs_comp, int acf_comp, int max_iters, hipStream_t st);
 int mg_solve1_prepare_with (void* mg_handle, hps_slab s, int sol_comp, int rhs_comp, int acf_comp, int max_iters, SlabView f, GradPsiSxSy ga,
                             hipStream_t st, bool* done);
+bool mg_ride_shift_init (void* mg_handle, const ShiftInit& pass);
 const int* mg_gate_after_enqueued (void* mg_handle);
 void mg_defer_post (void* mg_handle);
 bool mg_take_deferred_post (void* mg_handle, MgPost* out);
@@ -227,6 +228,10 @@
     int push_with_ionization (int islice, const int comp[5], const int* go, bool first);
     bool lazy_shift = true, shift_pending = false;
     void flush_shift ();
+    bool early_init = true; int n_alt = 0; InitSet set_canon{}, set_alt{};
+    bool alt_live = false, init_done = false, pend_rode = false; long slices_rode = 0;
+    const InitSet& live () const { return alt_live ? set_alt : set_canon; }
+    const InitSet& other () const { return alt_live ? set_canon : set_alt; }
     bool fuse_sources = true;
     int c_sal = -1; int sal_last_slice = -2; bool sal_overloaded = false; double sal_zeta_initial = 0.0;
     double* d_sal = nullptr; std::vector<double> sal_stats;
diff --git a/hipace_amd/csrc/engine.hip b/hipace_amd/csrc/engine.hip
--- a/hipace_amd/csrc/engine.hip
+++ b/hipace_amd/csrc/engine.hip
@@ -63,7 +63,7 @@
 }
 
 __global__ __launch_bounds__(256)
-void k_shift_slices (double* p, long ns, long plane, int js, CellBox bb)
+void k_shift_slices (double* p, long ns, long plane, int js, CellBox bb, int c_njxb, int c_njyb)
 {
     const long s = (long)blockIdx.x*blockDim.x + threadIdx.x;
     if (s >= plane) return;
@@ -71,7 +71,7 @@
     double njx = 0.0, njy = 0.0;
     if (i >= bb.ilo && i <= bb.ihi && j >= bb.jlo && j <= bb.jhi) {
         const double tjx = p[HPS_C_JXB*ns + s], tjy = p[HPS_C_JYB*ns + s];
-        njx = p[HPS_C_N_JXB*ns + s]; njy = p[HPS_C_N_JYB*ns + s];
+        njx = p[c_njxb*ns + s]; njy = p[c_njyb*ns + s];
         p[HPS_C_P_JXB*ns + s] = tjx; p[HPS_C_P_JYB*ns + s] = tjy;
         p[HPS_C_JXB*ns + s] = njx;   p[HPS_C_JYB*ns + s] = njy;
     }
@@ -79,23 +79,11 @@
 }
 
 __global__ __launch_bounds__(256)
-void k_shift_zero (double* p, long ns, long plane, int js, CellBox bb, int c_rho, int c_ion = -1)
+void k_shift_zero (ShiftInit a)
 {
     const long s = (long)blockIdx.x*blockDim.x + threadIdx.x;
-    if (s >= plane) return;
-    const int j = (int)(s / js), i = (int)(s - (long)j*js);
-    double njx = 0.0, njy = 0.0;
-    if (i >= bb.ilo && i <= bb.ihi && j >= bb.jlo && j <= bb.jhi) {
-        const double tjx = p[HPS_C_JXB*ns + s], tjy = p[HPS_C_JYB*ns + s];
-        njx = p[HPS_C_N_JXB*ns + s]; njy = p[HPS_C_N_JYB*ns + s];
-        p[HPS_C_P_JXB*ns + s] = tjx; p[HPS_C_P_JYB*ns + s] = tjy;
-        p[HPS_C_JXB*ns + s] = njx;   p[HPS_C_JYB*ns + s] = njy;
-        p[HPS_C_N_JXB*ns + s] = 0.0; p[HPS_C_N_JYB*ns + s] = 0.0; p[HPS_C_JZB*ns + s] = 0.0;
-    }
-    p[HPS_C_JX*ns + s] = njx; p[HPS_C_JY*ns + s] = njy;
-    const double ion = c_ion >= 0 ? p[c_ion*ns + s] : 0.0;
-    p[HPS_C_CHI*ns + s] = 0.0; p[HPS_C_RHOMJZ*ns + s] = ion;
-    if (c_rho >= 0) p[c_rho*ns + s] = ion;
+    if (s >= a.plane) return;
+    shift_init_cell(a, s);
 }
 
 __global__ __launch_bounds__(256)
@@ -671,6 +659,7 @@
     if (const char* v = std::getenv("HPS_GATED_ION_PUSH")) gate_ion_push = std::atoi(v) != 0;
     if (const char* v = std::getenv("HPS_LAZY_SHIFT")) lazy_shift = std::atoi(v) != 0;
     if (const char* v = std::getenv("HPS_FUSE_SOURCES")) fuse_sources = std::atoi(v) != 0;
+    if (const char* v = std::getenv("HPS_EARLY_INIT")) early_init = std::atoi(v) != 0;
     if (const char* v = std::getenv("HPS_SORT_FALLBACK_DIV")) { const long q = std::atol(v); if (q >= 1) fallback_div = q; }
     HPS_REQUIRE(!(d.beam_spin_tracking && d.dt == 0.0 && !d.dt_adaptive), "hps_engine_create: spin tracking needs a moving beam (hipace.dt != 0)");
     HPS_REQUIRE(!(d.dt_adaptive && d.laser_on), "hps_engine_create: hipace.dt = adaptive cannot be used with a laser (Hipace.cpp:408)");
@@ -726,6 +715,13 @@
         sal_stats.assign((size_t)4*d.nz, 0.0);
     }
     slab.nx = d.nx; slab.ny = d.ny; slab.ng = g; slab.ncomp = ncomp + (c_sal >= 0 ? (int)HPS_SAL_NCOMP : 0);
+    set_canon = set_alt = InitSet{HPS_C_CHI, HPS_C_RHOMJZ, d.deposit_rho ? (int)HPS_C_RHO : -1, HPS_C_JZB, HPS_C_N_JXB, HPS_C_N_JYB};
+    if (early_init && !pc && !d.laser_on && !d.ion_on && d.dt == 0.0 && !d.dt_adaptive && d.nx % 2 == 0 && d.ny % 2 == 0) {
+        int c = slab.ncomp;
+        set_alt.chi = c++; set_alt.rhomjz = c++; if (d.deposit_rho) set_alt.rho = c++;
+        set_alt.jzb = c++; set_alt.njxb = c++; set_alt.njyb = c++;
+        n_alt = c - slab.ncomp; slab.ncomp = c;
+    }
     slab.jstride = d.nx + 2*g; slab.nstride = slab.jstride*(d.ny + 2*g);
     HPS_HIP_CHECK(hipMalloc(&slab.p, (size_t)slab.nstride*slab.ncomp*sizeof(double)));
     HPS_HIP_CHECK(hipMemset(slab.p, 0, (size_t)slab.nstride*slab.ncomp*sizeof(double)));
@@ -859,6 +855,7 @@
         ++steps_begun;
     }
     shift_pending = false;
+    alt_live = false; init_done = false; pend_rode = false;
     HPS_HIP_CHECK(hipMemsetAsync(slab.p, 0, (size_t)slab.nstride*slab.ncomp*sizeof(double), st));
     if (d_pc_dist) HPS_HIP_CHECK(hipMemsetAsync(d_pc_dist, (d.grid_current_on || d.ion_on || d.plasma_no_neutralize || el.thermal.warm() || ions.thermal.warm()) ? 1 : 0, sizeof(int), st));
     HPS_HIP_CHECK(hipMemsetAsync(d_checksum, 0, HPS_PC_NCOMP_MAX*sizeof(double), st));
@@ -1591,10 +1588,23 @@
 
 void Engine::flush_shift ()
 {
-    if (!shift_pending) return;
-    shift_pending = false;
-    const CellBox bb{beam_box.ilo, beam_box.ihi, beam_box.jlo, beam_box.jhi};
-    hipLaunchKernelGGL(k_shift_slices, dim3(ceil_div(slab.nstride, 256)), dim3(256), 0, st, slab.p, slab.nstride, slab.nstride, (int)slab.jstride, bb);
+    const dim3 gplane(ceil_div(slab.nstride, 256)), b256(256);
+    if (shift_pending) {
+        shift_pending = false;
+        const CellBox bb{beam_box.ilo, beam_box.ihi, beam_box.jlo, beam_box.jhi};
+        hipLaunchKernelGGL(k_shift_slices, gplane, b256, 0, st, slab.p, slab.nstride, slab.nstride, (int)slab.jstride, bb, live().njxb, live().njyb);
+    }
+    if (alt_live != init_done) {
+        CompList a{0, {}}, b{0, {}};
+        for (int k = 0; k < 2; ++k) {
+            const InitSet& x = k ? set_alt : set_canon; CompList& l = k ? b : a;
+            for (int c : {x.chi, x.rhomjz, x.rho, x.jzb, x.njxb, x.njyb}) if (c >= 0) l.c[l.n++] = c;
+        }
+        CompList dst = a, src = b;
+        for (int k = 0; k < b.n; ++k) { dst.c[dst.n++] = b.c[k]; src.c[src.n++] = a.c[k]; }
+        hipLaunchKernelGGL(k_copy_comps, gplane, b256, 0, st, slab.p, slab.nstride, slab.nstride, dst, src);
+        alt_live = !alt_live;
+    }
 }
 
 int Engine::solve_slice (int islice)
@@ -1623,19 +1633,27 @@
     const CellBox bb{beam_box.ilo, beam_box.ihi, beam_box.jlo, beam_box.jhi};
     const bool ahead = (ahead_for == islice);
     ahead_for = -2;
-    bool zeroed = false;
+    const bool plain = n_alt > 0 && !moving && coll.empty() && c_aabs < 0 && !ions.present() && !salame_now() && !fuse_push_deposit && !ahead
+                       && lazy_shift && !aux_on && !diagnostics && !d_fd && !d_insitu;
+    if (!plain && (alt_live || init_done)) {
+        flush_shift();
+        alt_live = false; init_done = false;
+    }
+    const InitSet L = live();
+    bool zeroed = init_done;
+    init_done = false;
     if (shift_pending) {
         shift_pending = false;
-        if (!ahead) { hipLaunchKernelGGL(k_shift_zero, gplane, b256, 0, st, slab.p, slab.nstride, plane, (int)slab.jstride, bb, d.deposit_rho ? (int)HPS_C_RHO : -1, (int)HPS_C_ION_RHOMJZ); zeroed = true; }
-        else hipLaunchKernelGGL(k_shift_slices, gplane, b256, 0, st, slab.p, slab.nstride, plane, (int)slab.jstride, bb);
+        if (!ahead) { hipLaunchKernelGGL(k_shift_zero, gplane, b256, 0, st, ShiftInit{slab.p, slab.nstride, plane, (int)slab.jstride, bb, L, L, (int)HPS_C_ION_RHOMJZ}); zeroed = true; }
+        else hipLaunchKernelGGL(k_shift_slices, gplane, b256, 0, st, slab.p, slab.nstride, plane, (int)slab.jstride, bb, L.njxb, L.njyb);
     }
     if (!ahead && !zeroed)
     {   CompList z{0, {}}, zb{0, {}};
-        for (int c : {HPS_C_CHI, HPS_C_RHOMJZ}) z.c[z.n++] = c;
-        if (d.deposit_rho) z.c[z.n++] = HPS_C_RHO;
-        for (int c : {HPS_C_JZB, HPS_C_N_JXB, HPS_C_N_JYB}) zb.c[zb.n++] = c;
+        for (int c : {L.chi, L.rhomjz}) z.c[z.n++] = c;
+        if (d.deposit_rho) z.c[z.n++] = L.rho;
+        for (int c : {L.jzb, L.njxb, L.njyb}) zb.c[zb.n++] = c;
         CompList fi{0, {}};
-        fi.c[fi.n++] = HPS_C_RHOMJZ; if (d.deposit_rho) fi.c[fi.n++] = HPS_C_RHO;
+        fi.c[fi.n++] = L.rhomjz; if (d.deposit_rho) fi.c[fi.n++] = L.rho;
         hipLaunchKernelGGL(k_zero_comps, gplane, b256, 0, st, slab.p, slab.nstride, plane, (int)slab.jstride, z, zb, bb, fi, (int)HPS_C_ION_RHOMJZ); }
     if (c_aabs >= 0) {
         if ((e = laser_update_aabs(*this, islice, diagnostics ? d_laser_sum : nullptr))) return e;
@@ -1658,12 +1676,12 @@
         bw.a = BeamView{pa, pa + cA, pa + 2*cA, pa + 3*cA, pa + 4*cA, pa + 5*cA, pa + 6*cA};
         bw.b = BeamView{pb, pb + cB, pb + 2*cB, pb + 3*cB, pb + 4*cB, pb + 5*cB, pb + 6*cB};
         bw.ca = cA; bw.cb = cB; bw.nba = (int)ceil_div(cA, 256); bw.nwg = bw.nba + (int)ceil_div(cB, 256);
-        bw.cjz = HPS_C_JZB; bw.cjxn = HPS_C_N_JXB; bw.cjyn = HPS_C_N_JYB;
+        bw.cjz = L.jzb; bw.cjxn = L.njxb; bw.cjyn = L.njyb;
         bw.q_invvol = d.beam_charge*(d.si_units ? 1.0/(gm.dx*gm.dy*gm.dz) : 1.0); bw.csq_inv = 1.0/(gm.c*gm.c);
     }
     const bool beam_folded = pair && fold_beam && bw.nwg > 0 && !ahead && el.pl.n > 0 && el.tiling && el.tiling->sorted_n > 0;
     if (!ahead)
-    {   const int comp[6] = {HPS_C_JX, HPS_C_JY, -1, d.deposit_rho ? HPS_C_RHO : -1, HPS_C_CHI, HPS_C_RHOMJZ};
+    {   const int comp[6] = {HPS_C_JX, HPS_C_JY, -1, L.rho, L.chi, L.rhomjz};
         if ((e = species_deposit(el, comp, beam_folded ? &bw : nullptr))) return e;
         if ((e = species_deposit(ions, comp))) return e; }
     mark();
@@ -1674,11 +1692,11 @@
             switch (d.order) { case 0: HPS_PAIR(0); break; case 1: HPS_PAIR(1); break; case 2: HPS_PAIR(2); break; default: HPS_PAIR(3); break; }
 #undef HPS_PAIR
         }
-    } else if ((e = deposit_beam_slice(islice, -1, -1, HPS_C_JZB))) return e;
-    deposit_grid_current(islice, HPS_C_JZB);
+    } else if ((e = deposit_beam_slice(islice, -1, -1, L.jzb))) return e;
+    deposit_grid_current(islice, L.jzb);
     if (aux) {
         HPS_HIP_CHECK(hipEventRecord(ev_aux[1], st)); HPS_HIP_CHECK(hipStreamWaitEvent(st_aux, ev_aux[1], 0));
-        if ((e = mg_solve1_prepare(mg, slab, HPS_C_BX, HPS_C_SY, HPS_C_CHI, 200, st_aux))) return e;
+        if ((e = mg_solve1_prepare(mg, slab, HPS_C_BX, HPS_C_SY, L.chi, 200, st_aux))) return e;
         HPS_HIP_CHECK(hipEventRecord(ev_aux[2], st_aux));
         aux_pending = true;
     }
@@ -1688,7 +1706,7 @@
         const int comps[3] = {HPS_C_PSI, HPS_C_EZ, HPS_C_BZ};
         if (fuse_sources && poisson_sources_fusable(ps) && d.field_bc == 0) {
             const long js = slab.jstride;
-            const double* R = slab.p + (long)HPS_C_RHOMJZ*slab.nstride + g + (long)g*js;
+            const double* R = slab.p + (long)L.rhomjz*slab.nstride + g + (long)g*js;
             const double* X = slab.p + (long)HPS_C_JX*slab.nstride + g + (long)g*js;
             const double* Y = slab.p + (long)HPS_C_JY*slab.nstride + g + (long)g*js;
             const PoissonSrc spec[3] = {
@@ -1697,8 +1715,8 @@
                 {2, {X + js, Y + 1}, {X - js, Y - 1}, {fbz_y, fbz_x}}};
             if ((e = poisson_solve_batch_src(ps, 3, spec, js, slab, comps, st))) return e;
         } else {
-            hipLaunchKernelGGL(k_rhs_all, dim3(ceil_div(slab.jstride, 256), d.ny + 2*g), b256, 0, st, f, HPS_C_RHOMJZ,
-                               -1 , d.deposit_rho ? HPS_C_RHO : -1, HPS_C_JX, HPS_C_JY, 1.0/gm.ep0,
+            hipLaunchKernelGGL(k_rhs_all, dim3(ceil_div(slab.jstride, 256), d.ny + 2*g), b256, 0, st, f, L.rhomjz,
+                               -1 , L.rho, HPS_C_JX, HPS_C_JY, 1.0/gm.ep0,
                                fez_x, fez_y, fbz_y, fbz_x, staging, (long)d.nx*d.ny);
             if ((e = open_boundary(3, 0x6u))) return e;
             if ((e = hps_poisson_solve_batch(ps, 3, staging, slab, comps, st))) return e;
@@ -1710,11 +1728,11 @@
     if (laser_split && d.laser_solver == 1) { if ((e = laser_advance_slice(*this, islice)) || (e = laser_done())) return e; }
     if (aux_pending) { HPS_HIP_CHECK(hipStreamWaitEvent(st, ev_aux[2], 0)); aux_pending = false; }
     if (pair || nbeam == 0) {
-        const GradPsiSxSy ga{HPS_C_PSI, HPS_C_EXMBY, HPS_C_EYPBX, 0.5*(1.0/gm.dx), 0.5*(1.0/gm.dy), HPS_C_SX, HPS_C_SY, HPS_C_JZB, HPS_C_N_JXB, HPS_C_N_JYB,
+        const GradPsiSxSy ga{HPS_C_PSI, HPS_C_EXMBY, HPS_C_EYPBX, 0.5*(1.0/gm.dx), 0.5*(1.0/gm.dy), HPS_C_SX, HPS_C_SY, L.jzb, L.njxb, L.njyb,
                              HPS_C_P_JXB, HPS_C_P_JYB, gm.mu0, 2.0*gm.dx, 2.0*gm.dy, 2.0*gm.dz, bb};
         bool with_hierarchy = false;
         if (fold_hierarchy && !pc && !aux) {
-            if ((e = mg_solve1_prepare_with(mg, slab, HPS_C_BX, HPS_C_SY, HPS_C_CHI, 200, f, ga, st, &with_hierarchy))) return e;
+            if ((e = mg_solve1_prepare_with(mg, slab, HPS_C_BX, HPS_C_SY, L.chi, 200, f, ga, st, &with_hierarchy))) return e;
         }
         if (!with_hierarchy)
             hipLaunchKernelGGL(k_gradpsi_sxsy, dim3(ceil_div(slab.jstride, 256), d.ny + 2*g), b256, 0, st, f, ga);
@@ -1723,8 +1741,8 @@
         hipLaunchKernelGGL(k_grad_psi, dim3(ceil_div(d.nx + 2*(g - 1), 256), d.ny + 2*(g - 1)), b256, 0, st, f, HPS_C_PSI,
                            HPS_C_EXMBY, HPS_C_EYPBX, 0.5*(1.0/gm.dx), 0.5*(1.0/gm.dy));
         mark();
-        if (!sal) { if ((e = deposit_beam_slice(islice - 1, HPS_C_N_JXB, HPS_C_N_JYB, -1))) return e; }
-        hipLaunchKernelGGL(k_sxsy_beam, dim3(ceil_div(slab.jstride, 256), d.ny + 2*g), b256, 0, st, f, HPS_C_SX, HPS_C_SY, HPS_C_JZB, HPS_C_N_JXB, HPS_C_N_JYB,
+        if (!sal) { if ((e = deposit_beam_slice(islice - 1, L.njxb, L.njyb, -1))) return e; }
+        hipLaunchKernelGGL(k_sxsy_beam, dim3(ceil_div(slab.jstride, 256), d.ny + 2*g), b256, 0, st, f, HPS_C_SX, HPS_C_SY, L.jzb, L.njxb, L.njyb,
                            HPS_C_P_JXB, HPS_C_P_JYB, gm.mu0, 2.0*gm.dx, 2.0*gm.dy, 2.0*gm.dz, bb);
     }
     mark();
@@ -1740,7 +1758,9 @@
     const int comp_push[5] = {HPS_C_PSI, HPS_C_EZ, HPS_C_BX, HPS_C_BY, HPS_C_BZ};
     {
         if (gated && post_in_push) mg_defer_post(mg);
-        if ((e = mg_solve1_begin(mg, slab, HPS_C_BX, HPS_C_SY, HPS_C_CHI, d.mg_tol_rel, d.mg_tol_abs, 200, st))) return e;
+        pend_rode = plain && gated && islice > 0
+                    && mg_ride_shift_init(mg, ShiftInit{slab.p, slab.nstride, plane, (int)slab.jstride, bb, L, other(), (int)HPS_C_ION_RHOMJZ});
+        if ((e = mg_solve1_begin(mg, slab, HPS_C_BX, HPS_C_SY, L.chi, d.mg_tol_rel, d.mg_tol_abs, 200, st))) return e;
         if (gated_ion) {
             mark();
             mark();
@@ -1828,7 +1848,7 @@
             if ((e = ionize_collect())) return e;
         }
         if (fuse) {
-            hipLaunchKernelGGL(k_shift_zero, gplane, b256, 0, st, slab.p, slab.nstride, plane, (int)slab.jstride, bb, d.deposit_rho ? (int)HPS_C_RHO : -1, (int)HPS_C_ION_RHOMJZ);
+            hipLaunchKernelGGL(k_shift_zero, gplane, b256, 0, st, ShiftInit{slab.p, slab.nstride, plane, (int)slab.jstride, bb, set_canon, set_canon, (int)HPS_C_ION_RHOMJZ});
             const int dep[6] = {HPS_C_JX, HPS_C_JY, -1, d.deposit_rho ? HPS_C_RHO : -1, HPS_C_CHI, HPS_C_RHOMJZ};
             if ((e = advance_deposit_tiled(slab, el.pl, gm, comp, dep, el.charge, el.mass, d.order, d.n_subcycles, d.max_qsa, d_nqsa, el.tiling, d_nfallback, st))) return e;
             ahead_for = islice - 1;
@@ -1843,9 +1863,10 @@
     if (moving && nbeam > 0) { if ((e = beam_push_moving(*this, islice))) return e; }
     if (!coll.empty()) { if ((e = collide_slice(islice))) return e; }
     mark();
-    if (ahead_for != islice - 1) {
+    if (pend_rode) { pend_rode = false; alt_live = !alt_live; init_done = true; ++slices_rode; }
+    else if (ahead_for != islice - 1) {
         if (lazy_shift && islice > 0 && !salame_now()) shift_pending = true;
-        else hipLaunchKernelGGL(k_shift_slices, gplane, b256, 0, st, slab.p, slab.nstride, plane, (int)slab.jstride, bb);
+        else hipLaunchKernelGGL(k_shift_slices, gplane, b256, 0, st, slab.p, slab.nstride, plane, (int)slab.jstride, bb, live().njxb, live().njyb);
     }
     mark();
     HPS_HIP_CHECK(hipGetLastError());
@@ -2028,7 +2049,19 @@
     if (np) *np = E->el.pl.n;
     return HPS_OK;
 }
-extern "C" hps_slab hps_engine_slab (void* h) { Engine* E = static_cast<Engine*>(h); E->flush_shift(); return E->slab; }
+extern "C" hps_slab hps_engine_slab (void* h)
+{
+    Engine* E = static_cast<Engine*>(h);
+    E->flush_shift();
+    hps_slab s = E->slab; s.ncomp -= E->n_alt;
+    return s;
+}
+extern "C" int hps_engine_early_init_slices (void* h, long* n)
+{
+    HPS_REQUIRE(h && n, "hps_engine_early_init_slices: null argument");
+    *n = static_cast<Engine*>(h)->slices_rode;
+    return HPS_OK;
+}
 extern "C" hps_plasma hps_engine_plasma (void* h) { return static_cast<Engine*>(h)->el.pl; }
 extern "C" int hps_engine_tiling (void* h, void** tiling)
 {
diff --git a/hipace_amd/csrc/multigrid.hip b/hipace_amd/csrc/multigrid.hip
--- a/hipace_amd/csrc/multigrid.hip
+++ b/hipace_amd/csrc/multigrid.hip
@@ -944,11 +944,17 @@
     }
 }
 
+__device__ __forceinline__ void lower_v_guest (const ShiftInit& a, int guest, int nguests)
+{
+    for (long s = (long)guest*1024 + threadIdx.x; s < a.plane; s += (long)nguests*1024) shift_init_cell(a, s);
+}
+
 __global__ __launch_bounds__(1024)
 void k_lower_v3 (const Low2* __restrict__ dp, const double* __restrict__ acf_g, const double* __restrict__ cinv_g,
                  const double* __restrict__ res_g, double* __restrict__ cor_g, double* __restrict__ coef_g, int nxA, int nyA, int ctot,
-                 double facx0, double facy0, int nsweeps_bottom, StopRule sr)
-{
+                 double facx0, double facy0, int nsweeps_bottom, StopRule sr, ShiftInit guest)
+{
+    if (blockIdx.x >= 2) { lower_v_guest(guest, (int)blockIdx.x - 2, (int)gridDim.x - 2); return; }
     extern __shared__ __attribute__((aligned(16))) double lds_raw[];
     lds_double* base = (lds_double*)lds_raw;
     const int t = threadIdx.x;
@@ -1271,6 +1277,7 @@
     SolveRun run{};
     bool defer_post = false; bool deferred_valid = false; MgPost deferred{};
     bool use_low3 = false; Low2 low3{}; Low2* d_low3 = nullptr; size_t low3_lds = 0;
+    bool ride_on = false; ShiftInit ride{}; int ride_guests = 0;
     double* cinvA = nullptr;
     double* coef_img = nullptr;
     double* tmp0 = nullptr;
@@ -1369,6 +1376,10 @@
             HPS_HIP_CHECK(hipMalloc(&M->d_low3, sizeof(Low2)));
             HPS_HIP_CHECK(hipMemcpy(M->d_low3, &e, sizeof(Low2), hipMemcpyHostToDevice));
             HPS_HIP_CHECK(hipMalloc(&M->cinvA, (size_t)e.nx[0]*e.ny[0]*sizeof(double)));
+            int dev = 0, ncu = 0;
+            HPS_HIP_CHECK(hipGetDevice(&dev));
+            HPS_HIP_CHECK(hipDeviceGetAttribute(&ncu, hipDeviceAttributeMultiprocessorCount, dev));
+            M->ride_guests = std::max(ncu - 2, 1);
             break;
         }
     }
@@ -1478,10 +1489,12 @@
             const dim3 grid(ceil_div(bb.vhx - bb.vlx + 1, 64), bb.vhy - bb.vly + 1);
             for (int is = -1; is < nsweeps; ++is)
                 hipLaunchKernelGGL(k_bottom_sweep<CC>, grid, dim3(64), 0, st, bb, cor, rhs, acf, 1.0/(ldx*ldx), 1.0/(ldy*ldy), is, sr);
-        } else if (M->use_low3)
-            hipLaunchKernelGGL(k_lower_v3, dim3(2), dim3(1024), M->low3_lds, st, M->d_low3, M->L[lb].acf, M->cinvA, M->L[lb].res, M->L[lb].cor,
-                               M->coef_img, M->low3.nx[0], M->low3.ny[0], M->low3.ctot, 1.0/(ldx*ldx), 1.0/(ldy*ldy), nsweeps, sr);
-        else
+        } else if (M->use_low3) {
+            const int guests = (k == 0 && M->ride_on) ? M->ride_guests : 0;
+            M->ride_on = false;
+            hipLaunchKernelGGL(k_lower_v3, dim3(2 + guests), dim3(1024), M->low3_lds, st, M->d_low3, M->L[lb].acf, M->cinvA, M->L[lb].res, M->L[lb].cor,
+                               M->coef_img, M->low3.nx[0], M->low3.ny[0], M->low3.ctot, 1.0/(ldx*ldx), 1.0/(ldy*ldy), nsweeps, sr, M->ride);
+        } else
             hipLaunchKernelGGL(k_lower_v<CC>, dim3(CC ? 1 : 2), dim3(1024), M->low_lds, st, M->d_low, nl - lb, M->L[lb].acf, M->L[lb].res,
                                M->L[lb].cor, 1.0/(ldx*ldx), 1.0/(ldy*ldy), nsweeps, sr, M->pulls(lb) ? M->lv(lb-1, M->L[lb-1].rescor) : FView{});
     }
@@ -1715,7 +1728,12 @@
     *done = true;
     return HPS_OK;
 }
-void mg_solve1_forget_hierarchy (void* handle) { if (handle) static_cast<Multigrid*>(handle)->hierarchy_ready = false; }
+void mg_solve1_forget_hierarchy (void* handle)
+{
+    if (!handle) return;
+    Multigrid* M = static_cast<Multigrid*>(handle);
+    M->hierarchy_ready = false; M->ride_on = false;
+}
 void mg_defer_post (void* handle) { Multigrid* M = static_cast<Multigrid*>(handle); M->defer_post = true; M->deferred_valid = false; }
 bool mg_take_deferred_post (void* handle, MgPost* out)
 {
@@ -1723,6 +1741,13 @@
     M->defer_post = false;
     if (!M->deferred_valid) return false;
     M->deferred_valid = false; *out = M->deferred;
+    return true;
+}
+bool mg_ride_shift_init (void* handle, const ShiftInit& pass)
+{
+    Multigrid* M = static_cast<Multigrid*>(handle);
+    if (!M->cc || !M->use_low3 || M->bottom) return false;
+    M->ride = pass; M->ride_on = true;
     return true;
 }
 const int* mg_gate_after_enqueued (void* handle)
diff --git a/hipace_amd/csrc/slab_ops.h b/hipace_amd/csrc/slab_ops.h
--- a/hipace_amd/csrc/slab_ops.h
+++ b/hipace_amd/csrc/slab_ops.h
@@ -33,5 +33,26 @@
     f.p[a.cSx*f.ns + o] = -a.mu0*(-dx_jzb + dz_jxb);
 }
 
+struct InitSet { int chi, rhomjz, rho, jzb, njxb, njyb; };
+struct ShiftInit { double* p; long ns, plane; int js; CellBox bb; InitSet live, next; int c_ion; };
+
+__device__ __forceinline__ void shift_init_cell (const ShiftInit& a, long s)
+{
+    double* p = a.p; const long ns = a.ns;
+    const int j = (int)((unsigned)s / (unsigned)a.js), i = (int)s - j*a.js;
+    double njx = 0.0, njy = 0.0;
+    if (i >= a.bb.ilo && i <= a.bb.ihi && j >= a.bb.jlo && j <= a.bb.jhi) {
+        const double tjx = p[HPS_C_JXB*ns + s], tjy = p[HPS_C_JYB*ns + s];
+        njx = p[a.live.njxb*ns + s]; njy = p[a.live.njyb*ns + s];
+        p[HPS_C_P_JXB*ns + s] = tjx; p[HPS_C_P_JYB*ns + s] = tjy;
+        p[HPS_C_JXB*ns + s] = njx;   p[HPS_C_JYB*ns + s] = njy;
+        p[a.next.njxb*ns + s] = 0.0; p[a.next.njyb*ns + s] = 0.0; p[a.next.jzb*ns + s] = 0.0;
+    }
+    p[HPS_C_JX*ns + s] = njx; p[HPS_C_JY*ns + s] = njy;
+    const double ion = a.c_ion >= 0 ? p[a.c_ion*ns + s] : 0.0;
+    p[a.next.chi*ns + s] = 0.0; p[a.next.rhomjz*ns + s] = ion;
+    if (a.next.rho >= 0) p[a.next.rho*ns + s] = ion;
+}
+
 }
 #endif
diff --git a/include/hpslice.h b/include/hpslice.h
--- a/include/hpslice.h
+++ b/include/hpslice.h
@@ -200,6 +200,7 @@
 hps_stream hps_engine_stream (void* handle);
 int hps_engine_checksums (void* handle, double* out_host);
 int hps_engine_stats (void* handle, long* total_vcycles, long* slices_done);
+int hps_engine_early_init_slices (void* handle, long* n_slices);
 int hps_engine_pc_stats (void* handle, long* iterations, double* error_sum);
 int hps_engine_pc_zero_b_slices (void* handle, long* slices);
 int hps_engine_laser_info (void* handle, int* aabs_comp, double* envelope_abs_sum_host);
```

After: 1724, median of 6. 1.1% higher.
